# audeering/opensmile

Hardware: AMD Instinct MI355X
Metric: MFCC frames/sec (16kHz, 25ms/10ms) (higher is better)
Workload: dtype f32

## Files before the change

### include/smilehip.h

```cpp
#ifndef SMILEHIP_H
#define SMILEHIP_H

#include <stdint.h>

#ifdef __cplusplus
extern "C" {
#endif

#define SMILEHIP_VERSION 0x000100

typedef enum smilehip_status {
  SMILEHIP_OK = 0,
  SMILEHIP_ERR_INVALID = -1,
  SMILEHIP_ERR_NO_DEVICE = -2,
  SMILEHIP_ERR_HIP = -3,
  SMILEHIP_ERR_NOMEM = -4
} smilehip_status;

typedef enum smilehip_winfunc {
  SMILEHIP_WIN_RECT = 0, SMILEHIP_WIN_HANN = 1, SMILEHIP_WIN_HAMM = 2,
  SMILEHIP_WIN_GAUSS = 3, SMILEHIP_WIN_SINE = 4, SMILEHIP_WIN_TRI = 5,
  SMILEHIP_WIN_BARTLETT = 6, SMILEHIP_WIN_LANCZOS = 7
} smilehip_winfunc;

typedef struct smilehip_lld_config {
  uint32_t struct_size;
  double sample_rate;
  double frame_size_sec;
  double frame_step_sec;
  int32_t preemph;
  float   preemph_k;
  int32_t preemph_de;
  int32_t win_func;
  double  win_sigma;
  double  win_gain;
  double  win_offset;
  int32_t zero_pad_symmetric;
  int32_t n_bands;
  float   lofreq;
  float   hifreq;
  int32_t use_power;
  int32_t mel_htk_compatible;
  int32_t first_mfcc;
  int32_t last_mfcc;
  float   cep_lifter;
  int32_t mfcc_htk_compatible;
  float   melfloor;
  int32_t n_delta;
  int32_t delta_win;
  int32_t  chain_kind;
  int32_t  plp_lp_order;
  float    plp_compression;
  double   pitch_max;
  double   voicing_cutoff;
  int32_t  sma_win;
  int64_t  force_frame_size;
  double   force_fft_frame_size_sec;
  uint32_t stage_mask;
  double   pitch_min;
  int32_t  shs_n_harmonics;
  float    shs_compression;
  float    f0_min_energy;
  int32_t  append_log_energy;
  int32_t  cms;
  int32_t  jitter_broken_thresh;
  int32_t  vit_buffer_len;
  double   jitter_search_range;
  double   formant_max_freq;
  double   specscale_min_f;
  int32_t  shs_n_candidates;
  int32_t  shs_old_peak_algo;
  int32_t  spectral_band_lo[2], spectral_band_hi[2];
  int32_t  specscale_off;
} smilehip_lld_config;

#define SMILEHIP_CHAIN_MFCC 0
#define SMILEHIP_CHAIN_IS09 1
#define SMILEHIP_CHAIN_COMPARE_AB 2
#define SMILEHIP_CHAIN_PLP 3
#define SMILEHIP_CHAIN_COMPARE_F0 4
#define SMILEHIP_CHAIN_COMPARE 5
#define SMILEHIP_CHAIN_EGEMAPS 6

#define SMILEHIP_STAGE_WINDOW 1u
#define SMILEHIP_STAGE_FFT    2u
#define SMILEHIP_STAGE_MEL    4u
#define SMILEHIP_STAGE_MFCC   8u
#define SMILEHIP_STAGE_ALL    15u
#define SMILEHIP_STAGE_SPECTRAL 16u

typedef struct smilehip_geometry {
  int64_t frame_size;
  int64_t frame_step;
  int64_t fft_size;
  int64_t n_bins;
  int32_t n_static;
  int32_t n_out;
  double  frame_period;
  double  fft_frame_size_sec;
} smilehip_geometry;

typedef struct smilehip_context smilehip_context;
typedef struct smilehip_plan smilehip_plan;
typedef struct smilehip_batch smilehip_batch;

int  smilehip_version(void);
const char *smilehip_last_error(void);
int  smilehip_init(int device, smilehip_context **ctx);
void smilehip_shutdown(smilehip_context *ctx);
int  smilehip_device_name(smilehip_context *ctx, char *buf, int buflen);

void smilehip_config_is09_lld(smilehip_lld_config *c);

void smilehip_config_plp_0_d_a(smilehip_lld_config *c);
void smilehip_config_compare16_ab(smilehip_lld_config *c);
int smilehip_config_htk_variant(smilehip_lld_config *c, const char *name);
void smilehip_config_compare16_f0(smilehip_lld_config *c);
void smilehip_config_compare16(smilehip_lld_config *c);
void smilehip_config_is13_compare(smilehip_lld_config *c);

void smilehip_config_egemapsv02(smilehip_lld_config *c);
void smilehip_config_egemapsv01a(smilehip_lld_config *c);

int smilehip_specscale_frames(smilehip_plan *plan, const float *d_mag, int64_t ld_src, float *d_dst, int64_t ld_dst,
                              int64_t n_frames, void *stream);
int smilehip_pitchshs_frames(smilehip_plan *plan, const float *d_hps, int64_t ld_src, float *d_dst, int64_t ld_dst,
                             int64_t n_frames, void *stream);

int smilehip_batch_f0_taps(smilehip_batch *b, float *d_hps_dst, const float **d_shs, const float **d_e60);
int smilehip_batch_f0_pending(smilehip_batch *b, const int32_t **d_pending);

#define SMILEHIP_FUNC_MAX          (1u << 0)
#define SMILEHIP_FUNC_MIN          (1u << 1)
#define SMILEHIP_FUNC_RANGE        (1u << 2)
#define SMILEHIP_FUNC_MAXPOS       (1u << 3)
#define SMILEHIP_FUNC_MINPOS       (1u << 4)
#define SMILEHIP_FUNC_AMEAN        (1u << 5)
#define SMILEHIP_FUNC_MAXAMEANDIST (1u << 6)
#define SMILEHIP_FUNC_MINAMEANDIST (1u << 7)
#define SMILEHIP_FUNC_LINREGC1     (1u << 8)
#define SMILEHIP_FUNC_LINREGC2     (1u << 9)
#define SMILEHIP_FUNC_LINREGERRA   (1u << 10)
#define SMILEHIP_FUNC_LINREGERRQ   (1u << 11)
#define SMILEHIP_FUNC_VARIANCE     (1u << 12)
#define SMILEHIP_FUNC_STDDEV       (1u << 13)
#define SMILEHIP_FUNC_SKEWNESS     (1u << 14)
#define SMILEHIP_FUNC_KURTOSIS     (1u << 15)
#define SMILEHIP_FUNC_AMEAN_M      (1u << 16)
#define SMILEHIP_FUNC_ALL          0x1ffffu
uint32_t smilehip_functionals_is09_mask(void);
int smilehip_functionals_count(uint32_t mask);
int smilehip_batch_func_rows(const smilehip_batch *batch, int64_t *rows);
int smilehip_batch_functionals(smilehip_plan *plan, smilehip_batch *batch, const float *d_lld, int64_t ld_lld,
                               uint32_t mask, float *d_func, int64_t ld_func, void *stream);

int smilehip_functionals_matrix(smilehip_context *ctx, const float *d_x, int64_t ld_x, int64_t rows, int32_t cols,
                                uint32_t mask, float *d_out, void *stream);

enum {
  SMILEHIP_FAM_EXTREMES = 0, SMILEHIP_FAM_MEANS, SMILEHIP_FAM_MOMENTS, SMILEHIP_FAM_REGRESSION, SMILEHIP_FAM_PERCENTILES,
  SMILEHIP_FAM_TIMES, SMILEHIP_FAM_SEGMENTS, SMILEHIP_FAM_LPC, SMILEHIP_FAM_PEAKS2, SMILEHIP_FAM_ONSET, SMILEHIP_FAM_PEAKS, SMILEHIP_FAM_CROSSINGS, SMILEHIP_FAM_DCT,
  SMILEHIP_FAM_SAMPLES, SMILEHIP_FAM_MODULATION, SMILEHIP_FAM_COUNT
};
enum { SMILEHIP_NORM_SEGMENT = 0, SMILEHIP_NORM_SECOND = 1, SMILEHIP_NORM_FRAME = 2 };
enum { SMILEHIP_SEG_RELTH = 0, SMILEHIP_SEG_NONX = 1, SMILEHIP_SEG_EQX = 2, SMILEHIP_SEG_MRELTH = 3, SMILEHIP_SEG_ABSTH = 4,
       SMILEHIP_SEG_NARELTH = 5, SMILEHIP_SEG_NAMRELTH = 6, SMILEHIP_SEG_NAABSTH = 7, SMILEHIP_SEG_DELTA = 8,
       SMILEHIP_SEG_DELTA2 = 9, SMILEHIP_SEG_CHX = 10 };

typedef struct smilehip_func_spec {
  int32_t n_fam;
  int32_t fam[12];
  int32_t non_zero_functs;
  int32_t reserved0;
  double period;
  uint32_t ext_mask; int32_t ext_norm;
  uint32_t means_mask; int32_t means_norm;
  uint32_t mom_mask; int32_t mom_stddev_norm; int32_t mom_ratio_limit; int32_t reserved1;
  uint32_t reg_mask; int32_t reg_centroid_norm, reg_norm_coeff, reg_norm_inputs, reg_centroid_abs,
      reg_centroid_limit, reg_ratio_limit, reg_old_buggy_qerr;
  uint32_t pct_mask; int32_t pct_interp, n_pctl, n_range;
  double pctl[8]; int32_t range_a[8], range_b[8];
  uint32_t times_mask; int32_t times_norm, times_buggy_sec_norm, reserved2;
  uint32_t seg_mask; int32_t seg_norm, seg_algo, seg_max_num, seg_min_lng, seg_auto_min_lng, seg_pause_min_lng,
      seg_x_is_rel, seg_n_thresholds, seg_ravg_lng;
  float seg_x; float seg_thresholds[8]; float seg_range_rel_threshold;
  int32_t lpc_gain, lpc_coeffs, lpc_first, lpc_order;
  uint32_t pk_mask; int32_t pk_norm, pk_ratio_limit, pk_dyn_rel, pk_use_abs, reserved5;
  float pk_rel_thresh, pk_abs_thresh;
  uint32_t ons_mask; int32_t ons_norm, ons_use_abs, reserved6;
  float ons_thr_on, ons_thr_off;
  uint32_t pko_mask; int32_t pko_norm;
  uint32_t crs_mask; int32_t dct_first, dct_last, n_samples;
  double sample_pos[8];
  int32_t n_quot, quot_a[8], quot_b[8];
  int32_t n_ul, n_dl, reserved7;
  double ul[8], dl[8];
  int32_t mod_win_frames, mod_step_frames, mod_n_bins, mod_win_func, mod_remove_nz_mean, reserved8;
  double mod_min_freq, mod_max_freq;
} smilehip_func_spec;

int smilehip_funcspec_count(const smilehip_func_spec *spec);
int smilehip_funcspec_compare16(const char *instance, smilehip_func_spec *spec);
int smilehip_funcspec_is13_compare(const char *instance, smilehip_func_spec *spec);
int smilehip_funcspec_matrix(smilehip_context *ctx, const smilehip_func_spec *spec, const float *d_x, int64_t ld_x,
                             int64_t rows, int32_t cols, float *d_out, void *stream);
int smilehip_batch_funcspec(smilehip_plan *plan, smilehip_batch *batch, const smilehip_func_spec *spec,
                            const float *d_lld, int64_t ld_lld, int32_t col_first, int32_t n_cols, int32_t rows_cut,
                            const float *d_extra, int64_t ld_extra, float *d_func, int64_t ld_func, void *stream);

int smilehip_functionals_compare16_count(void);
int smilehip_batch_functionals_compare16(smilehip_plan *plan, smilehip_batch *batch, const float *d_lld, int64_t ld_lld,
                                         float *d_func, int64_t ld_func, void *stream);
int smilehip_batch_functionals_is13_compare(smilehip_plan *plan, smilehip_batch *batch, const float *d_lld, int64_t ld_lld,
                                            float *d_func, int64_t ld_func, void *stream);
int smilehip_batch_compare_b_extra(smilehip_batch *batch, const float **d_extra);

int smilehip_funcspec_egemaps(const char *instance, smilehip_func_spec *spec);
int smilehip_functionals_egemaps_count(void);
int smilehip_batch_functionals_egemaps(smilehip_plan *plan, smilehip_batch *batch, float *d_func, int64_t ld_func, void *stream);
int smilehip_batch_egemaps_taps(smilehip_batch *batch, const float **d_raw20, const float **d_lpc, const float **d_formants,
                                const float **d_pitch3, const float **d_jit4, const float **d_shim_db, const float **d_harm6,
                                const float **d_func_in, const int32_t **d_pending, int64_t *h_frame_off60);

int  smilehip_alloc(smilehip_context *ctx, uint64_t bytes, void **d_ptr);
int  smilehip_free(smilehip_context *ctx, void *d_ptr);
int  smilehip_copy_to_device(smilehip_context *ctx, void *d_dst, const void *h_src, uint64_t bytes, void *stream);
int  smilehip_copy_to_host(smilehip_context *ctx, void *h_dst, const void *d_src, uint64_t bytes, void *stream);
int  smilehip_stream_synchronize(smilehip_context *ctx, void *stream);
int  smilehip_alloc_cache(smilehip_context *ctx, uint64_t bytes);
int  smilehip_stream_create(smilehip_context *ctx, void **stream);
int  smilehip_stream_destroy(smilehip_context *ctx, void *stream);
int  smilehip_event_create(smilehip_context *ctx, void **event);
int  smilehip_event_destroy(smilehip_context *ctx, void *event);
int  smilehip_event_record(smilehip_context *ctx, void *event, void *stream);
int  smilehip_stream_wait_event(smilehip_context *ctx, void *stream, void *event);
int  smilehip_copy_to_device_2d(smilehip_context *ctx, void *d_dst, uint64_t d_pitch, const void *h_src, uint64_t h_pitch,
                                uint64_t width_bytes, uint64_t rows, void *stream);
int  smilehip_copy_to_host_2d(smilehip_context *ctx, void *h_dst, uint64_t h_pitch, const void *d_src, uint64_t d_pitch,
                              uint64_t width_bytes, uint64_t rows, void *stream);
int  smilehip_alloc_host(smilehip_context *ctx, uint64_t bytes, void **h_ptr);
int  smilehip_free_host(smilehip_context *ctx, void *h_ptr);
int  smilehip_host_register(smilehip_context *ctx, void *h_ptr, uint64_t bytes);
int  smilehip_host_unregister(smilehip_context *ctx, void *h_ptr);
int  smilehip_htk_rows_be(smilehip_context *ctx, const float *d_src, int64_t n, void *d_dst, void *stream);

void smilehip_config_mfcc12_0_d_a(smilehip_lld_config *c);

int  smilehip_plan_create(smilehip_context *ctx, const smilehip_lld_config *cfg, smilehip_plan **plan);
int  smilehip_plan_create_host_only(const smilehip_lld_config *cfg, smilehip_plan **plan);
void smilehip_plan_destroy(smilehip_plan *plan);
int  smilehip_plan_geometry(const smilehip_plan *plan, smilehip_geometry *g);
int64_t smilehip_num_frames(const smilehip_plan *plan, int64_t n_samples);
double  smilehip_frame_time(const smilehip_plan *plan, int64_t t);
double  smilehip_row_time(const smilehip_plan *plan, int64_t n_frames, int64_t row);
int64_t smilehip_plan_get_window(const smilehip_plan *plan, float *out, int64_t cap);
int64_t smilehip_plan_get_mel_weights(const smilehip_plan *plan, float *out, int64_t cap);
int64_t smilehip_plan_get_mel_chanmap(const smilehip_plan *plan, int32_t *out, int64_t cap);
int64_t smilehip_plan_get_dct(const smilehip_plan *plan, float *out, int64_t cap);
int64_t smilehip_plan_get_lifter(const smilehip_plan *plan, float *out, int64_t cap);

int  smilehip_batch_create(smilehip_plan *plan, const int64_t *h_sample_offsets, int32_t n_utt,
                           smilehip_batch **batch);
void smilehip_batch_destroy(smilehip_batch *batch);
int64_t smilehip_batch_total_frames(const smilehip_batch *batch);
int64_t smilehip_batch_total_rows(const smilehip_batch *batch);
int  smilehip_batch_delta_fused(const smilehip_batch *batch);
int  smilehip_batch_frame_offsets(const smilehip_batch *batch, int64_t *h_row_offsets);

int  smilehip_mfcc_run(smilehip_plan *plan, smilehip_batch *batch, const int16_t *d_pcm,
                       float *d_out, int64_t ld_out, void *stream);

int  smilehip_lld_run(smilehip_plan *plan, smilehip_batch *batch, const int16_t *d_pcm,
                      float *d_out, int64_t ld_out, void *stream);
int  smilehip_lld_run_f32(smilehip_plan *plan, smilehip_batch *batch, const float *d_pcm_f32,
                          float *d_out, int64_t ld_out, void *stream);
int  smilehip_lld_run_host(smilehip_plan *plan, smilehip_batch *batch, const int16_t *h_pcm,
                           int64_t n_samples, float *h_out);

int  smilehip_mfcc_run_host(smilehip_plan *plan, smilehip_batch *batch, const int16_t *h_pcm,
                            int64_t n_samples, float *h_out);

int  smilehip_plan_set_timing(smilehip_plan *plan, int enable);
int  smilehip_plan_last_timing(smilehip_plan *plan, float *ms_main, float *ms_delta);
int  smilehip_kernel_timing(int enable);
int64_t smilehip_kernel_timing_report(char *buf, int64_t buflen);


int smilehip_pcm16_to_float(smilehip_context *ctx, const int16_t *d_pcm, int64_t n, float *d_out, void *stream);
int smilehip_pcm_convert(smilehip_context *ctx, const void *d_raw, int n_bps, int n_bits, int n_chan, int mono_mixdown,
                         int64_t n, float *d_out, void *stream);
int smilehip_pcm_convert_float(smilehip_context *ctx, const float *d_raw, int n_chan, int mono_mixdown, int64_t n, float *d_out,
                               void *stream);
int smilehip_irfft_frames(smilehip_plan *plan, const float *d_src, int64_t ld_src, float *d_dst, int64_t ld_dst, int64_t n_frames,
                          void *stream);
#define SMILEHIP_MAGPHASE_MAGNITUDE 1
#define SMILEHIP_MAGPHASE_PHASE 2
#define SMILEHIP_MAGPHASE_NORMALISE 4
#define SMILEHIP_MAGPHASE_POWER 8
#define SMILEHIP_MAGPHASE_DBPSD 16
int smilehip_fftmagphase_frames(smilehip_context *ctx, const float *d_src, int64_t ld_src, int64_t nfft, int32_t flags, float dbp_norm,
                                float min_dbp, float *d_dst, int64_t ld_dst, int64_t n_frames, void *stream);
int smilehip_melspec_table_frames(smilehip_context *ctx, const float *d_src, int64_t ld_src, int64_t K, int32_t n_bands, int32_t dense,
                                  const float *d_coef, const int32_t *d_chanmap, int32_t n_lo, int32_t n_hi, int32_t use_power,
                                  float htk_scale, float *d_dst, int64_t ld_dst, int64_t n_frames, void *stream);
int smilehip_melspec_inverse_table_frames(smilehip_context *ctx, const float *d_src, int64_t ld_src, int32_t n_src, int64_t K,
                                          const float *d_coef, const int32_t *d_chanmap, int32_t n_lo, int32_t n_hi, int32_t use_power,
                                          float htk_div, float *d_dst, int64_t ld_dst, int64_t n_frames, void *stream);
int smilehip_pitchacf_zcr_frames(smilehip_context *ctx, const float *d_src, int64_t ld_src, int64_t n, int64_t n_frames, double fs_sec,
                                 double max_pitch, double *d_zcr, void *stream);
#define SMILEHIP_MZCR_ZCR 1
#define SMILEHIP_MZCR_MCR 2
#define SMILEHIP_MZCR_AMAX 4
#define SMILEHIP_MZCR_MAXMIN 8
#define SMILEHIP_MZCR_DC 16
int smilehip_mzcr_frames(smilehip_context *ctx, const float *d_src, int64_t ld_src, int64_t N, int64_t n_frames, int32_t flags,
                         float *d_dst, int64_t ld_dst, void *stream);
int smilehip_frame_rows(smilehip_context *ctx, const float *d_samples, int64_t frame_size, int64_t frame_step, int64_t n_frames,
                        float *d_dst, int64_t ld_dst, void *stream);
int smilehip_preemphasis_frames(smilehip_context *ctx, const float *d_src, int64_t ld_src, float *d_dst,
                                int64_t ld_dst, int64_t n_frames, int64_t N, float k, int de, void *stream);
int smilehip_window_frames(smilehip_plan *plan, const float *d_src, int64_t ld_src, float *d_dst,
                           int64_t ld_dst, int64_t n_frames, void *stream);
int smilehip_rfft_frames(smilehip_plan *plan, const float *d_src, int64_t ld_src, float *d_dst,
                         int64_t ld_dst, int64_t n_frames, void *stream);
int smilehip_fftmag_frames(smilehip_plan *plan, const float *d_src, int64_t ld_src, float *d_dst,
                           int64_t ld_dst, int64_t n_frames, void *stream);
int smilehip_melspec_frames(smilehip_plan *plan, const float *d_src, int64_t ld_src, float *d_dst,
                            int64_t ld_dst, int64_t n_frames, void *stream);
int smilehip_mfcc_frames(smilehip_plan *plan, const float *d_src, int64_t ld_src, float *d_dst,
                         int64_t ld_dst, int64_t n_frames, void *stream);
int  smilehip_mfcc_inverse_frames(smilehip_plan *plan, const float *d_src, int64_t ld_src, float *d_dst, int64_t ld_dst,
                                  int64_t n_frames, int do_log, void *stream);
int smilehip_sumsq_frames(smilehip_context *ctx, const float *d_src, int64_t ld_src, int64_t N, int64_t n_frames,
                          double *d_out, void *stream);
int smilehip_zcr_count_frames(smilehip_context *ctx, const float *d_src, int64_t ld_src, int64_t N, int64_t n_frames,
                              int32_t *d_out, void *stream);
int smilehip_acf_frames(smilehip_plan *plan, const float *d_src, int64_t ld_src, float *d_dst, int64_t ld_dst, int64_t n_out,
                        int64_t n_frames, int use_power, int cepstrum, int norm_output, int abs_cepstrum, void *stream);
int smilehip_pitchacf_frames(smilehip_context *ctx, const float *d_src, int64_t ld_src, int64_t n, int64_t n_frames,
                             double fs_sec, double max_pitch, double *d_voicing, int32_t *d_max_idx, void *stream);
int smilehip_pitchacf_contour_step(smilehip_context *ctx, const double *d_voicing, const int32_t *d_max_idx, double t_samp,
                                   double voicing_cutoff, float *d_state, float *d_out4, void *stream);
int smilehip_pitchacf_contour_frames(smilehip_context *ctx, const double *d_voicing, const int32_t *d_max_idx, double t_samp,
                                     double voicing_cutoff, float *d_state, float *d_out4, int64_t n_frames, void *stream);
int smilehip_spectral_frames(smilehip_plan *plan, const float *d_mag, int64_t ld_src, float *d_state, int first,
                             float *d_dst, int64_t ld_dst, int64_t n_frames, void *stream);
typedef struct smilehip_spectral_opts {
  int32_t n_bands;
  int32_t band_lo[16], band_hi[16];
  int32_t n_rolloff;
  double  rolloff[16];
  int32_t flux, centroid, max_pos, min_pos, entropy, variance, skewness, kurtosis, slope, sharpness, harmonicity;
  int32_t flatness, log_flatness;
  int32_t spec_diff, spec_pos_diff, flux_centroid, flux_at_flux_centroid, standard_deviation;
  int32_t n_slopes;
  int32_t slope_lo[16], slope_hi[16];
} smilehip_spectral_opts;
typedef struct smilehip_spectral_op smilehip_spectral_op;
int smilehip_spectral_opts_count(const smilehip_spectral_opts *opts);
int smilehip_spectral_op_create(smilehip_context *ctx, const smilehip_spectral_opts *opts, int64_t K, double frame_size_sec,
                                smilehip_spectral_op **op);
int smilehip_spectral_op_n_out(const smilehip_spectral_op *op);
int smilehip_spectral_op_frames(smilehip_spectral_op *op, const float *d_mag, int64_t ld_src, float *d_state, int first,
                                float *d_dst, int64_t ld_dst, int64_t n_frames, void *stream);
int smilehip_spectral_op_destroy(smilehip_spectral_op *op);
int smilehip_plp_audspec_frames(smilehip_context *ctx, const float *d_mel, int64_t ld_src, int n_bands, const float *d_eql,
                                float melfloor, float compression, int new_rasta, const float *rasta_coef, float *d_state,
                                float *d_dst, int64_t ld_dst, int64_t n_frames, void *stream);
int smilehip_plp_cc_frames(smilehip_context *ctx, const float *d_mel, int64_t ld_src, int n_bands, const float *d_eql,
                           float melfloor, float compression, int lp_order, const float *d_cos, const float *d_sin,
                           float *d_dst, int64_t ld_dst, int64_t n_frames, void *stream);
int smilehip_plp_stage_frames(smilehip_context *ctx, const float *d_mel, int64_t ld_src, int n_bands, const float *d_eql,
                              float melfloor, float compression, int lp_order, const float *d_cos, int out_stage,
                              float *d_dst, int64_t ld_dst, int64_t n_frames, void *stream);
int smilehip_window_op_row(smilehip_context *ctx, const float *d_x, float *d_y, int64_t n_t, int kind, int W, void *stream);
int smilehip_window_op_row_ex(smilehip_context *ctx, const float *d_x, float *d_y, int64_t n_t, int kind, int W, float *d_norm_io,
                              void *stream);
#define SMILEHIP_DELTA_RELATIVE 1
#define SMILEHIP_DELTA_HALFWAVE 2
#define SMILEHIP_DELTA_ABS 4
#define SMILEHIP_DELTA_SEGMENTS 8
int smilehip_delta_op_row(smilehip_context *ctx, const float *d_x, float *d_y, int64_t n_t, int W, int flags, float *d_norm_io,
                          void *stream);
int smilehip_window_op_block(smilehip_context *ctx, const float *d_x, int64_t ld_x, float *d_y, int64_t ld_y, int64_t n_t,
                             int32_t n_cols, int op, int W, int delta_flags, void *stream);
int smilehip_delta_segments_block(smilehip_context *ctx, const float *d_x, int64_t ld_x, float *d_y, int64_t ld_y, int64_t n_ticks,
                                  int32_t tick_frames, int32_t n_cols, int W, int delta_flags, float *d_norm_io, void *stream);
int smilehip_spectral_gemaps_frames(smilehip_plan *plan, const float *d_mag, int64_t ld_src, float *d_state, int first,
                                    float *d_dst, int64_t ld_dst, int64_t n_frames, void *stream);
int smilehip_specresample_frames(smilehip_plan *plan, const float *d_spec, int64_t ld_src, float *d_dst, int64_t ld_dst,
                                 int64_t n_frames, void *stream);
int smilehip_lpc_frames(smilehip_plan *plan, const float *d_x, int64_t ld_src, float *d_lpc, int64_t ld_dst, int64_t n_frames,
                        void *stream);
int smilehip_specresample_geometry(int64_t n_in, double fs_sec, double last_fs_sec, double base_period, double target_fs,
                                   int64_t *n_out, int64_t *k_max, double *nd);
int smilehip_specresample_tables(int64_t n_in, int64_t n_out, int64_t k_max, double nd, float *cos_table, float *sin_table);
int smilehip_specresample_table_frames(smilehip_context *ctx, const float *d_src, int64_t ld_src, int64_t n_in, int64_t n_out,
                                       int64_t k_max, const float *d_cos, const float *d_sin, float *d_dst, int64_t ld_dst,
                                       int64_t n_frames, void *stream);
int smilehip_lpc_acf_frames(smilehip_context *ctx, const float *d_x, int64_t ld_src, int64_t n, int32_t p, float *d_lpc,
                            int64_t ld_dst, int64_t n_frames, void *stream);
int smilehip_lsp_frames(smilehip_context *ctx, const float *d_lpc, int64_t ld_src, int32_t p, float *d_dst, int64_t ld_dst,
                        int64_t n_frames, void *stream);
int smilehip_intensity_frames(smilehip_context *ctx, const float *d_src, int64_t ld_src, int64_t N, int32_t flags, float *d_dst,
                              int64_t ld_dst, int64_t n_frames, void *stream);
enum { SMILEHIP_VOP_ADD = 0, SMILEHIP_VOP_MUL, SMILEHIP_VOP_LOG, SMILEHIP_VOP_LOGA, SMILEHIP_VOP_SQRT, SMILEHIP_VOP_E, SMILEHIP_VOP_ABS,
       SMILEHIP_VOP_DB_POW, SMILEHIP_VOP_DB_MAG, SMILEHIP_VOP_X_SUM, SMILEHIP_VOP_X_SUMSQ, SMILEHIP_VOP_X_L1, SMILEHIP_VOP_X_L2 };
int smilehip_vecop_frames(smilehip_context *ctx, int32_t op, float param1, float logfloor, const float *d_src, int64_t ld_src,
                          int32_t n_cols, float *d_dst, int64_t ld_dst, int64_t n_frames, void *stream);
int smilehip_pitch_smoother_rows(smilehip_context *ctx, int32_t n_cand, float voicing_cutoff, int32_t octave_correction,
                                 int32_t post_simple, int32_t flags, const float *d_src, int64_t ld_src, const int64_t *d_row_off,
                                 int32_t n_streams, int64_t n_rows_single, void *d_state, int32_t resume, float *d_dst, int64_t ld_dst,
                                 int64_t *d_written, void *stream);
int smilehip_formantlpc_frames(smilehip_plan *plan, const float *d_lpc, int64_t ld_src, float *d_dst, int64_t ld_dst,
                               int64_t n_frames, void *stream);
#define SMILEHIP_FORMANT_STATE_BYTES 176
int smilehip_formantlpc_rows(smilehip_plan *plan, const float *d_lpc, int64_t ld_src, float *d_dst, int64_t ld_dst,
                             int64_t n_frames, void *d_state, int32_t resume, void *stream);
int smilehip_harmonics_frames(smilehip_plan *plan, const float *d_f0, const float *d_formants, int64_t ld_formants,
                              const float *d_mag, int64_t ld_mag, float *d_dst, int64_t ld_dst, int64_t n_frames, void *stream);

int smilehip_delta_chain(smilehip_plan *plan, smilehip_batch *batch, float *d_io, int64_t ld,
                         int32_t D, int32_t W, int32_t n_orders, void *stream);

int smilehip_valbased_select_frames(smilehip_context *ctx, const float *d_src, int64_t ld_src, int64_t N, int64_t n_frames,
                                    int32_t idx, float threshold, int32_t invert, int32_t allow_equal, int32_t zero_vec,
                                    int32_t remove_idx, float output_val, float *d_dst, int64_t ld_dst, int32_t *d_keep, void *stream);

typedef struct smilehip_viterbi_stream smilehip_viterbi_stream;
int smilehip_viterbi_stream_create(smilehip_context *ctx, int32_t buffer_len, float voicing_cutoff, const double *weights6,
                                   smilehip_viterbi_stream **out);
int smilehip_viterbi_stream_set_candidates(smilehip_viterbi_stream *s, int32_t n_candidates);
int smilehip_viterbi_stream_push(smilehip_viterbi_stream *s, const float *cand_f0, const float *cand_voicing,
                                 int32_t *n_decided, int32_t *frames, int32_t *states, int32_t cap);
int smilehip_viterbi_stream_push_frames(smilehip_viterbi_stream *s, const float *cand_f0, const float *cand_voicing, int64_t ld,
                                        int32_t n_frames, int32_t *n_decided, int32_t *frames, int32_t *states, int32_t cap);
int smilehip_viterbi_stream_flush(smilehip_viterbi_stream *s, int32_t *n_decided, int32_t *frames, int32_t *states, int32_t cap);
int smilehip_viterbi_stream_destroy(smilehip_viterbi_stream *s);

typedef struct smilehip_jitter_stream smilehip_jitter_stream;
int smilehip_jitter_stream_create(smilehip_context *ctx, double sample_period, int64_t frame_size, int64_t frame_step,
                                  double frame_step_sec, double search_range_rel, int32_t broken_jitter_thresh,
                                  smilehip_jitter_stream **out);
int smilehip_jitter_stream_set_time_offset(smilehip_jitter_stream *s, int64_t frames);
int smilehip_jitter_stream_push(smilehip_jitter_stream *s, float f0, const int16_t *h_pcm, int64_t pcm_start, int64_t n_pcm,
                                float *out5, int64_t *last_idx, int64_t *last_mis);
int smilehip_jitter_stream_push_frames(smilehip_jitter_stream *s, const float *f0, int32_t n_frames, const int16_t *h_pcm,
                                       int64_t pcm_start, int64_t n_pcm, float *out5, int64_t *last_idx, int64_t *last_mis);
int smilehip_jitter_stream_destroy(smilehip_jitter_stream *s);

#define SMILEHIP_SPECSCALE_LINEAR 0
#define SMILEHIP_SPECSCALE_LOG 1
#define SMILEHIP_SPECSCALE_BARK 2
#define SMILEHIP_SPECSCALE_MEL 3
#define SMILEHIP_SPECSCALE_SEMITONE 4
#define SMILEHIP_SPECSCALE_BARK_OLD 7
typedef struct smilehip_specscale_opts {
  int32_t scale;
  double  param;
  double  min_f, max_f;
  int32_t n_points_target;
  int32_t spec_enhance, spec_smooth, auditory_weighting;
} smilehip_specscale_opts;
typedef struct smilehip_specscale_op smilehip_specscale_op;
int smilehip_specscale_op_create(smilehip_context *ctx, const smilehip_specscale_opts *opts, int64_t n_src, double frame_size_sec,
                                 smilehip_specscale_op **out);
int smilehip_specscale_op_n_out(const smilehip_specscale_op *op);
int smilehip_specscale_op_frames(smilehip_specscale_op *op, const float *d_src, int64_t ld_src, float *d_dst, int64_t ld_dst,
                                 int64_t n_frames, void *stream);
int smilehip_specscale_op_destroy(smilehip_specscale_op *op);
int smilehip_specscale_tables(const smilehip_specscale_opts *opts, int64_t n_src, double frame_size_sec, double *f_t, double *spline,
                              int32_t *k, double *rec);

#ifdef __cplusplus
}
#endif
#endif
```

### opensmile_amd/capi.py

```python
import ctypes as C
import os

import numpy as np

HERE = os.path.dirname(os.path.abspath(__file__))
LIB_PATH = os.path.join(HERE, "libsmilehip.so")

WINFUNC = {"rec": 0, "rect": 0, "han": 1, "hann": 1, "ham": 2, "hamming": 2, "gau": 3,
           "gauss": 3, "sin": 4, "sine": 4, "tri": 5, "bar": 6, "bartlett": 6, "lac": 7}


class SmileHipError(RuntimeError):
    pass


class LldConfig(C.Structure):
    _fields_ = [
        ("struct_size", C.c_uint32),
        ("sample_rate", C.c_double), ("frame_size_sec", C.c_double), ("frame_step_sec", C.c_double),
        ("preemph", C.c_int32), ("preemph_k", C.c_float), ("preemph_de", C.c_int32),
        ("win_func", C.c_int32), ("win_sigma", C.c_double), ("win_gain", C.c_double),
        ("win_offset", C.c_double),
        ("zero_pad_symmetric", C.c_int32),
        ("n_bands", C.c_int32), ("lofreq", C.c_float), ("hifreq", C.c_float),
        ("use_power", C.c_int32), ("mel_htk_compatible", C.c_int32),
        ("first_mfcc", C.c_int32), ("last_mfcc", C.c_int32), ("cep_lifter", C.c_float),
        ("mfcc_htk_compatible", C.c_int32), ("melfloor", C.c_float),
        ("n_delta", C.c_int32), ("delta_win", C.c_int32),
        ("chain_kind", C.c_int32), ("plp_lp_order", C.c_int32), ("plp_compression", C.c_float), ("pitch_max", C.c_double), ("voicing_cutoff", C.c_double),
        ("sma_win", C.c_int32),
        ("force_frame_size", C.c_int64), ("force_fft_frame_size_sec", C.c_double),
        ("stage_mask", C.c_uint32),
        ("pitch_min", C.c_double), ("shs_n_harmonics", C.c_int32), ("shs_compression", C.c_float),
        ("f0_min_energy", C.c_float), ("append_log_energy", C.c_int32), ("cms", C.c_int32), ("jitter_broken_thresh", C.c_int32),
        ("vit_buffer_len", C.c_int32), ("jitter_search_range", C.c_double), ("formant_max_freq", C.c_double), ("specscale_min_f", C.c_double), ("shs_n_candidates", C.c_int32), ("shs_old_peak_algo", C.c_int32),
        ("spectral_band_lo", C.c_int32 * 2), ("spectral_band_hi", C.c_int32 * 2), ("specscale_off", C.c_int32),
    ]


STAGE_WINDOW, STAGE_FFT, STAGE_MEL, STAGE_MFCC, STAGE_ALL = 1, 2, 4, 8, 15


class FuncSpec(C.Structure):
    _fields_ = [
        ("n_fam", C.c_int32), ("fam", C.c_int32 * 12), ("non_zero_functs", C.c_int32), ("reserved0", C.c_int32),
        ("period", C.c_double),
        ("ext_mask", C.c_uint32), ("ext_norm", C.c_int32),
        ("means_mask", C.c_uint32), ("means_norm", C.c_int32),
        ("mom_mask", C.c_uint32), ("mom_stddev_norm", C.c_int32), ("mom_ratio_limit", C.c_int32), ("reserved1", C.c_int32),
        ("reg_mask", C.c_uint32), ("reg_centroid_norm", C.c_int32), ("reg_norm_coeff", C.c_int32),
        ("reg_norm_inputs", C.c_int32), ("reg_centroid_abs", C.c_int32), ("reg_centroid_limit", C.c_int32),
        ("reg_ratio_limit", C.c_int32), ("reg_old_buggy_qerr", C.c_int32),
        ("pct_mask", C.c_uint32), ("pct_interp", C.c_int32), ("n_pctl", C.c_int32), ("n_range", C.c_int32),
        ("pctl", C.c_double * 8), ("range_a", C.c_int32 * 8), ("range_b", C.c_int32 * 8),
        ("times_mask", C.c_uint32), ("times_norm", C.c_int32), ("times_buggy_sec_norm", C.c_int32), ("reserved2", C.c_int32),
        ("seg_mask", C.c_uint32), ("seg_norm", C.c_int32), ("seg_algo", C.c_int32), ("seg_max_num", C.c_int32),
        ("seg_min_lng", C.c_int32), ("seg_auto_min_lng", C.c_int32), ("seg_pause_min_lng", C.c_int32),
        ("seg_x_is_rel", C.c_int32), ("seg_n_thresholds", C.c_int32), ("seg_ravg_lng", C.c_int32),
        ("seg_x", C.c_float), ("seg_thresholds", C.c_float * 8), ("seg_range_rel_threshold", C.c_float),
        ("lpc_gain", C.c_int32), ("lpc_coeffs", C.c_int32), ("lpc_first", C.c_int32), ("lpc_order", C.c_int32),
        ("pk_mask", C.c_uint32), ("pk_norm", C.c_int32), ("pk_ratio_limit", C.c_int32), ("pk_dyn_rel", C.c_int32),
        ("pk_use_abs", C.c_int32), ("reserved5", C.c_int32),
        ("pk_rel_thresh", C.c_float), ("pk_abs_thresh", C.c_float),
        ("ons_mask", C.c_uint32), ("ons_norm", C.c_int32), ("ons_use_abs", C.c_int32), ("reserved6", C.c_int32),
        ("ons_thr_on", C.c_float), ("ons_thr_off", C.c_float),
        ("pko_mask", C.c_uint32), ("pko_norm", C.c_int32),
        ("crs_mask", C.c_uint32), ("dct_first", C.c_int32), ("dct_last", C.c_int32), ("n_samples", C.c_int32),
        ("sample_pos", C.c_double * 8),
        ("n_quot", C.c_int32), ("quot_a", C.c_int32 * 8), ("quot_b", C.c_int32 * 8),
        ("n_ul", C.c_int32), ("n_dl", C.c_int32), ("reserved7", C.c_int32),
        ("ul", C.c_double * 8), ("dl", C.c_double * 8),
        ("mod_win_frames", C.c_int32), ("mod_step_frames", C.c_int32), ("mod_n_bins", C.c_int32), ("mod_win_func", C.c_int32),
        ("mod_remove_nz_mean", C.c_int32), ("reserved8", C.c_int32),
        ("mod_min_freq", C.c_double), ("mod_max_freq", C.c_double),
    ]


class SpectralOpts(C.Structure):
    _fields_ = [("n_bands", C.c_int32), ("band_lo", C.c_int32 * 16), ("band_hi", C.c_int32 * 16), ("n_rolloff", C.c_int32),
                ("rolloff", C.c_double * 16)] + [(k, C.c_int32) for k in ("flux", "centroid", "max_pos", "min_pos", "entropy", "variance",
                                                                          "skewness", "kurtosis", "slope", "sharpness", "harmonicity", "flatness",
                                                                          "log_flatness", "spec_diff", "spec_pos_diff", "flux_centroid",
                                                                          "flux_at_flux_centroid", "standard_deviation", "n_slopes")] + [
                   ("slope_lo", C.c_int32 * 16), ("slope_hi", C.c_int32 * 16)]


def spectral_opts(bands, rolloff=(0.25, 0.5, 0.75, 0.9), slopes=(), **flags):
    o = SpectralOpts()
    o.n_slopes = len(slopes)
    for i, (a, b) in enumerate(slopes):
        o.slope_lo[i], o.slope_hi[i] = a, b
    o.n_bands = len(bands)
    for i, (a, b) in enumerate(bands):
        o.band_lo[i], o.band_hi[i] = a, b
    o.n_rolloff = len(rolloff)
    for i, r in enumerate(rolloff):
        o.rolloff[i] = r
    for k, v in flags.items():
        setattr(o, k, int(v))
    return o


class SpecScaleOpts(C.Structure):
    _fields_ = [("scale", C.c_int32), ("param", C.c_double), ("min_f", C.c_double), ("max_f", C.c_double), ("n_points_target", C.c_int32),
                ("spec_enhance", C.c_int32), ("spec_smooth", C.c_int32), ("auditory_weighting", C.c_int32)]


SPECSCALE = {"lin": 0, "log": 1, "bark": 2, "mel": 3, "sem": 4, "bao": 7}


def specscale_opts(scale, param=0.0, min_f=25.0, max_f=-1.0, n_points_target=0, spec_enhance=0, spec_smooth=0, auditory_weighting=0):
    o = SpecScaleOpts()
    o.scale = SPECSCALE[scale] if isinstance(scale, str) else int(scale)
    o.param, o.min_f, o.max_f, o.n_points_target = float(param), float(min_f), float(max_f), int(n_points_target)
    o.spec_enhance, o.spec_smooth, o.auditory_weighting = int(spec_enhance), int(spec_smooth), int(auditory_weighting)
    return o


class Geometry(C.Structure):
    _fields_ = [("frame_size", C.c_int64), ("frame_step", C.c_int64), ("fft_size", C.c_int64),
                ("n_bins", C.c_int64), ("n_static", C.c_int32), ("n_out", C.c_int32),
                ("frame_period", C.c_double), ("fft_frame_size_sec", C.c_double)]


_vp, _i32, _i64, _f32, _dbl = C.c_void_p, C.c_int32, C.c_int64, C.c_float, C.c_double
SYMBOLS = {
    "smilehip_version": (C.c_int, []),
    "smilehip_last_error": (C.c_char_p, []),
    "smilehip_init": (C.c_int, [C.c_int, C.POINTER(_vp)]),
    "smilehip_shutdown": (None, [_vp]),
    "smilehip_device_name": (C.c_int, [_vp, C.c_char_p, C.c_int]),
    "smilehip_config_is09_lld": (None, [C.POINTER(LldConfig)]),
    "smilehip_config_compare16_ab": (None, [C.POINTER(LldConfig)]),
    "smilehip_config_compare16_f0": (None, [C.POINTER(LldConfig)]),
    "smilehip_config_htk_variant": (C.c_int, [C.POINTER(LldConfig), C.c_char_p]),
    "smilehip_config_compare16": (None, [C.POINTER(LldConfig)]),
    "smilehip_specscale_frames": (C.c_int, [_vp, _vp, _i64, _vp, _i64, _i64, _vp]),
    "smilehip_pitchshs_frames": (C.c_int, [_vp, _vp, _i64, _vp, _i64, _i64, _vp]),
    "smilehip_batch_f0_taps": (C.c_int, [_vp, _vp, C.POINTER(_vp), C.POINTER(_vp)]),
    "smilehip_config_plp_0_d_a": (None, [C.POINTER(LldConfig)]),
    "smilehip_batch_total_rows": (_i64, [_vp]),
    "smilehip_batch_delta_fused": (C.c_int, [_vp]),
    "smilehip_functionals_is09_mask": (C.c_uint32, []),
    "smilehip_functionals_count": (C.c_int, [C.c_uint32]),
    "smilehip_functionals_matrix": (C.c_int, [_vp, _vp, _i64, _i64, C.c_int32, C.c_uint32, _vp, _vp]),
    "smilehip_batch_func_rows": (C.c_int, [_vp, _vp]),
    "smilehip_batch_functionals": (C.c_int, [_vp, _vp, _vp, _i64, C.c_uint32, _vp, _i64, _vp]),
    "smilehip_functionals_compare16_count": (C.c_int, []),
    "smilehip_batch_functionals_compare16": (C.c_int, [_vp, _vp, _vp, _i64, _vp, _i64, _vp]),
    "smilehip_batch_compare_b_extra": (C.c_int, [_vp, _vp]),
    "smilehip_funcspec_count": (C.c_int, [_vp]),
    "smilehip_funcspec_compare16": (C.c_int, [C.c_char_p, _vp]),
    "smilehip_funcspec_is13_compare": (C.c_int, [C.c_char_p, _vp]),
    "smilehip_batch_functionals_is13_compare": (C.c_int, [_vp, _vp, _vp, _i64, _vp, _i64, _vp]),
    "smilehip_config_is13_compare": (None, [_vp]),
    "smilehip_config_egemapsv02": (None, [C.POINTER(LldConfig)]),
    "smilehip_config_egemapsv01a": (None, [C.POINTER(LldConfig)]),
    "smilehip_funcspec_egemaps": (C.c_int, [C.c_char_p, _vp]),
    "smilehip_functionals_egemaps_count": (C.c_int, []),
    "smilehip_batch_functionals_egemaps": (C.c_int, [_vp, _vp, _vp, _i64, _vp]),
    "smilehip_batch_egemaps_taps": (C.c_int, [_vp] + [C.POINTER(_vp)] * 9 + [_vp]),
    "smilehip_spectral_gemaps_frames": (C.c_int, [_vp, _vp, _i64, _vp, C.c_int, _vp, _i64, _i64, _vp]),
    "smilehip_specresample_frames": (C.c_int, [_vp, _vp, _i64, _vp, _i64, _i64, _vp]),
    "smilehip_lpc_frames": (C.c_int, [_vp, _vp, _i64, _vp, _i64, _i64, _vp]),
    "smilehip_formantlpc_frames": (C.c_int, [_vp, _vp, _i64, _vp, _i64, _i64, _vp]),
    "smilehip_formantlpc_rows": (C.c_int, [_vp, _vp, _i64, _vp, _i64, _i64, _vp, _i32, _vp]),
    "smilehip_harmonics_frames": (C.c_int, [_vp, _vp, _vp, _i64, _vp, _i64, _vp, _i64, _i64, _vp]),
    "smilehip_valbased_select_frames": (C.c_int, [_vp, _vp, _i64, _i64, _i64, _i32, _f32, _i32, _i32, _i32, _i32, _f32, _vp, _i64, _vp, _vp]),
    "smilehip_jitter_stream_create": (C.c_int, [_vp, _dbl, _i64, _i64, _dbl, _dbl, _i32, C.POINTER(_vp)]),
    "smilehip_jitter_stream_push": (C.c_int, [_vp, _f32, _vp, _i64, _i64, _vp, _vp, _vp]),
    "smilehip_jitter_stream_set_time_offset": (C.c_int, [_vp, _i64]),
    "smilehip_jitter_stream_destroy": (C.c_int, [_vp]),
    "smilehip_viterbi_stream_create": (C.c_int, [_vp, _i32, _f32, _vp, C.POINTER(_vp)]),
    "smilehip_viterbi_stream_push": (C.c_int, [_vp, _vp, _vp, _vp, _vp, _vp, _i32]),
    "smilehip_viterbi_stream_set_candidates": (C.c_int, [_vp, _i32]),
    "smilehip_viterbi_stream_flush": (C.c_int, [_vp, _vp, _vp, _vp, _i32]),
    "smilehip_viterbi_stream_destroy": (C.c_int, [_vp]),
    "smilehip_funcspec_matrix": (C.c_int, [_vp, _vp, _vp, _i64, _i64, C.c_int32, _vp, _vp]),
    "smilehip_batch_funcspec": (C.c_int, [_vp, _vp, _vp, _vp, _i64, C.c_int32, C.c_int32, C.c_int32, _vp, _i64, _vp, _i64, _vp]),
    "smilehip_lld_run": (C.c_int, [_vp, _vp, _vp, _vp, _i64, _vp]),
    "smilehip_lld_run_f32": (C.c_int, [_vp, _vp, _vp, _vp, _i64, _vp]),
    "smilehip_lld_run_host": (C.c_int, [_vp, _vp, _vp, _i64, _vp]),
    "smilehip_alloc": (C.c_int, [_vp, C.c_uint64, C.POINTER(_vp)]),
    "smilehip_free": (C.c_int, [_vp, _vp]),
    "smilehip_alloc_host": (C.c_int, [_vp, C.c_uint64, C.POINTER(_vp)]),
    "smilehip_free_host": (C.c_int, [_vp, _vp]),
    "smilehip_htk_rows_be": (C.c_int, [_vp, _vp, _i64, _vp, _vp]),
    "smilehip_copy_to_device": (C.c_int, [_vp, _vp, _vp, C.c_uint64, _vp]),
    "smilehip_copy_to_host": (C.c_int, [_vp, _vp, _vp, C.c_uint64, _vp]),
    "smilehip_alloc_cache": (C.c_int, [_vp, C.c_uint64]),
    "smilehip_stream_create": (C.c_int, [_vp, C.POINTER(_vp)]),
    "smilehip_stream_destroy": (C.c_int, [_vp, _vp]),
    "smilehip_event_create": (C.c_int, [_vp, C.POINTER(_vp)]),
    "smilehip_event_destroy": (C.c_int, [_vp, _vp]),
    "smilehip_event_record": (C.c_int, [_vp, _vp, _vp]),
    "smilehip_stream_wait_event": (C.c_int, [_vp, _vp, _vp]),
    "smilehip_kernel_timing": (C.c_int, [C.c_int]),
    "smilehip_kernel_timing_report": (C.c_int64, [_vp, _i64]),
    "smilehip_copy_to_device_2d": (C.c_int, [_vp, _vp, C.c_uint64, _vp, C.c_uint64, C.c_uint64, C.c_uint64, _vp]),
    "smilehip_copy_to_host_2d": (C.c_int, [_vp, _vp, C.c_uint64, _vp, C.c_uint64, C.c_uint64, C.c_uint64, _vp]),
    "smilehip_host_register": (C.c_int, [_vp, _vp, C.c_uint64]),
    "smilehip_host_unregister": (C.c_int, [_vp, _vp]),
    "smilehip_frame_rows": (C.c_int, [_vp, _vp, _i64, _i64, _i64, _vp, _i64, _vp]),
    "smilehip_window_op_block": (C.c_int, [_vp, _vp, _i64, _vp, _i64, _i64, _i32, C.c_int, C.c_int, C.c_int, _vp]),
    "smilehip_delta_segments_block": (C.c_int, [_vp, _vp, _i64, _vp, _i64, _i64, _i32, _i32, C.c_int, C.c_int, _vp, _vp]),
    "smilehip_pitchacf_contour_frames": (C.c_int, [_vp, _vp, _vp, _dbl, _dbl, _vp, _vp, _i64, _vp]),
    "smilehip_viterbi_stream_push_frames": (C.c_int, [_vp, _vp, _vp, _i64, _i32, _vp, _vp, _vp, _i32]),
    "smilehip_jitter_stream_push_frames": (C.c_int, [_vp, _vp, _i32, _vp, _i64, _i64, _vp, _vp, _vp]),
    "smilehip_stream_synchronize": (C.c_int, [_vp, _vp]),
    "smilehip_config_mfcc12_0_d_a": (None, [C.POINTER(LldConfig)]),
    "smilehip_plan_create": (C.c_int, [_vp, C.POINTER(LldConfig), C.POINTER(_vp)]),
    "smilehip_plan_create_host_only": (C.c_int, [C.POINTER(LldConfig), C.POINTER(_vp)]),
    "smilehip_plan_destroy": (None, [_vp]),
    "smilehip_plan_geometry": (C.c_int, [_vp, C.POINTER(Geometry)]),
    "smilehip_num_frames": (_i64, [_vp, _i64]),
    "smilehip_frame_time": (_dbl, [_vp, _i64]),
    "smilehip_row_time": (_dbl, [_vp, _i64, _i64]),
    "smilehip_plan_get_window": (_i64, [_vp, _vp, _i64]),
    "smilehip_plan_get_mel_weights": (_i64, [_vp, _vp, _i64]),
    "smilehip_plan_get_mel_chanmap": (_i64, [_vp, _vp, _i64]),
    "smilehip_plan_get_dct": (_i64, [_vp, _vp, _i64]),
    "smilehip_plan_get_lifter": (_i64, [_vp, _vp, _i64]),
    "smilehip_batch_f0_pending": (C.c_int, [_vp, _vp]),
    "smilehip_batch_create": (C.c_int, [_vp, _vp, _i32, C.POINTER(_vp)]),
    "smilehip_batch_destroy": (None, [_vp]),
    "smilehip_batch_total_frames": (_i64, [_vp]),
    "smilehip_batch_frame_offsets": (C.c_int, [_vp, _vp]),
    "smilehip_mfcc_run": (C.c_int, [_vp, _vp, _vp, _vp, _i64, _vp]),
    "smilehip_mfcc_run_host": (C.c_int, [_vp, _vp, _vp, _i64, _vp]),
    "smilehip_plan_set_timing": (C.c_int, [_vp, C.c_int]),
    "smilehip_plan_last_timing": (C.c_int, [_vp, C.POINTER(_f32), C.POINTER(_f32)]),
    "smilehip_sumsq_frames": (C.c_int, [_vp, _vp, _i64, _i64, _i64, _vp, _vp]),
    "smilehip_zcr_count_frames": (C.c_int, [_vp, _vp, _i64, _i64, _i64, _vp, _vp]),
    "smilehip_acf_frames": (C.c_int, [_vp, _vp, _i64, _vp, _i64, _i64, _i64, C.c_int, C.c_int, C.c_int, C.c_int, _vp]),
    "smilehip_pitchacf_frames": (C.c_int, [_vp, _vp, _i64, _i64, _i64, _dbl, _dbl, _vp, _vp, _vp]),
    "smilehip_pitchacf_contour_step": (C.c_int, [_vp, _vp, _vp, _dbl, _dbl, _vp, _vp, _vp]),
    "smilehip_spectral_frames": (C.c_int, [_vp, _vp, _i64, _vp, C.c_int, _vp, _i64, _i64, _vp]),
    "smilehip_spectral_opts_count": (C.c_int, [_vp]),
    "smilehip_spectral_op_create": (C.c_int, [_vp, _vp, _i64, C.c_double, _vp]),
    "smilehip_spectral_op_n_out": (C.c_int, [_vp]),
    "smilehip_spectral_op_frames": (C.c_int, [_vp, _vp, _i64, _vp, C.c_int, _vp, _i64, _i64, _vp]),
    "smilehip_spectral_op_destroy": (C.c_int, [_vp]),
    "smilehip_plp_audspec_frames": (C.c_int, [_vp, _vp, _i64, C.c_int, _vp, C.c_float, C.c_float, C.c_int, _vp, _vp, _vp, _i64,
                                             _i64, _vp]),
    "smilehip_plp_cc_frames": (C.c_int, [_vp, _vp, _i64, C.c_int, _vp, C.c_float, C.c_float, C.c_int, _vp, _vp, _vp, _i64, _i64,
                                        _vp]),
    "smilehip_mfcc_inverse_frames": (C.c_int, [_vp, _vp, _i64, _vp, _i64, _i64, C.c_int, _vp]),
    "smilehip_plp_stage_frames": (C.c_int, [_vp, _vp, _i64, C.c_int, _vp, C.c_float, C.c_float, C.c_int, _vp, C.c_int, _vp, _i64, _i64,
                                           _vp]),
    "smilehip_window_op_row": (C.c_int, [_vp, _vp, _vp, _i64, C.c_int, C.c_int, _vp]),
    "smilehip_window_op_row_ex": (C.c_int, [_vp, _vp, _vp, _i64, C.c_int, C.c_int, _vp, _vp]),
    "smilehip_delta_op_row": (C.c_int, [_vp, _vp, _vp, _i64, C.c_int, C.c_int, _vp, _vp]),
    "smilehip_pcm_convert": (C.c_int, [_vp, _vp, C.c_int, C.c_int, C.c_int, C.c_int, _i64, _vp, _vp]),
    "smilehip_pcm_convert_float": (C.c_int, [_vp, _vp, C.c_int, C.c_int, _i64, _vp, _vp]),
    "smilehip_pcm16_to_float": (C.c_int, [_vp, _vp, _i64, _vp, _vp]),
    "smilehip_preemphasis_frames": (C.c_int, [_vp, _vp, _i64, _vp, _i64, _i64, _i64, _f32, C.c_int, _vp]),
    "smilehip_window_frames": (C.c_int, [_vp, _vp, _i64, _vp, _i64, _i64, _vp]),
    "smilehip_rfft_frames": (C.c_int, [_vp, _vp, _i64, _vp, _i64, _i64, _vp]),
    "smilehip_fftmag_frames": (C.c_int, [_vp, _vp, _i64, _vp, _i64, _i64, _vp]),
    "smilehip_irfft_frames": (C.c_int, [_vp, _vp, _i64, _vp, _i64, _i64, _vp]),
    "smilehip_fftmagphase_frames": (C.c_int, [_vp, _vp, _i64, _i64, _i32, _f32, _f32, _vp, _i64, _i64, _vp]),
    "smilehip_melspec_table_frames": (C.c_int, [_vp, _vp, _i64, _i64, _i32, _i32, _vp, _vp, _i32, _i32, _i32, _f32, _vp, _i64, _i64, _vp]),
    "smilehip_melspec_inverse_table_frames": (C.c_int, [_vp, _vp, _i64, _i32, _i64, _vp, _vp, _i32, _i32, _i32, _f32, _vp, _i64, _i64, _vp]),
    "smilehip_pitchacf_zcr_frames": (C.c_int, [_vp, _vp, _i64, _i64, _i64, _dbl, _dbl, _vp, _vp]),
    "smilehip_mzcr_frames": (C.c_int, [_vp, _vp, _i64, _i64, _i64, _i32, _vp, _i64, _vp]),
    "smilehip_melspec_frames": (C.c_int, [_vp, _vp, _i64, _vp, _i64, _i64, _vp]),
    "smilehip_mfcc_frames": (C.c_int, [_vp, _vp, _i64, _vp, _i64, _i64, _vp]),
    "smilehip_delta_chain": (C.c_int, [_vp, _vp, _vp, _i64, _i32, _i32, _i32, _vp]),
    "smilehip_specresample_geometry": (C.c_int, [_i64, _dbl, _dbl, _dbl, _dbl, _vp, _vp, _vp]),
    "smilehip_specresample_tables": (C.c_int, [_i64, _i64, _i64, _dbl, _vp, _vp]),
    "smilehip_specresample_table_frames": (C.c_int, [_vp, _vp, _i64, _i64, _i64, _i64, _vp, _vp, _vp, _i64, _i64, _vp]),
    "smilehip_lpc_acf_frames": (C.c_int, [_vp, _vp, _i64, _i64, _i32, _vp, _i64, _i64, _vp]),
    "smilehip_lsp_frames": (C.c_int, [_vp, _vp, _i64, _i32, _vp, _i64, _i64, _vp]),
    "smilehip_intensity_frames": (C.c_int, [_vp, _vp, _i64, _i64, _i32, _vp, _i64, _i64, _vp]),
    "smilehip_vecop_frames": (C.c_int, [_vp, _i32, _f32, _f32, _vp, _i64, _i32, _vp, _i64, _i64, _vp]),
    "smilehip_pitch_smoother_rows": (C.c_int, [_vp, _i32, _f32, _i32, _i32, _i32, _vp, _i64, _vp, _i32, _i64, _vp, _i32, _vp, _i64, _vp, _vp]),
    "smilehip_specscale_op_create": (C.c_int, [_vp, _vp, _i64, _dbl, _vp]),
    "smilehip_specscale_op_n_out": (C.c_int, [_vp]),
    "smilehip_specscale_op_frames": (C.c_int, [_vp, _vp, _i64, _vp, _i64, _i64, _vp]),
    "smilehip_specscale_op_destroy": (C.c_int, [_vp]),
    "smilehip_specscale_tables": (C.c_int, [_vp, _i64, _dbl, _vp, _vp, _vp, _vp]),
}

_lib = None


def load():
    global _lib
    if _lib is None:
        path = os.environ.get("SMILEHIP_LIB", LIB_PATH)
        if not os.path.exists(path):
            raise SmileHipError(
                f"{LIB_PATH} not found: build it with `python -c 'import __graft_entry__ as g; g.build()'` "
                "(make -C opensmile_amd/csrc). libsmilehip has no CPU fallback.")
        L = C.CDLL(path)
        for name, (res, args) in SYMBOLS.items():
            fn = getattr(L, name)
            fn.restype = res
            fn.argtypes = args
        _lib = L
    return _lib


def _check(rc):
    if rc != 0:
        raise SmileHipError(f"smilehip error {rc}: {load().smilehip_last_error().decode()}")


def plp_0_d_a_config():
    c = LldConfig()
    load().smilehip_config_plp_0_d_a(C.byref(c))
    return c


def compare16_ab_config():
    c = LldConfig()
    load().smilehip_config_compare16_ab(C.byref(c))
    return c


def htk_variant_config(name):
    c = LldConfig()
    _check(load().smilehip_config_htk_variant(C.byref(c), name.encode()))
    return c


def compare16_config():
    c = LldConfig()
    load().smilehip_config_compare16(C.byref(c))
    return c


def is13_compare_config():
    c = LldConfig()
    load().smilehip_config_is13_compare(C.byref(c))
    return c


def egemapsv02_config():
    c = LldConfig()
    load().smilehip_config_egemapsv02(C.byref(c))
    return c


def egemapsv01a_config():
    c = LldConfig()
    load().smilehip_config_egemapsv01a(C.byref(c))
    return c


def funcspec_egemaps(instance):
    s = FuncSpec()
    _check(load().smilehip_funcspec_egemaps(instance.encode(), C.byref(s)))
    return s


def rows_op_host(ctx, fn, handle, inputs, out_cols, pre=(), post=()):
    L = load()
    inputs = [np.ascontiguousarray(a, dtype=np.float32) for a in inputs]
    n = inputs[0].shape[0]
    out = np.zeros((n, out_cols), np.float32)
    ptrs = []
    d_out = _vp()
    try:
        for a in inputs:
            d = _vp()
            _check(L.smilehip_alloc(ctx._h, max(a.nbytes, 4), C.byref(d)))
            ptrs.append(d)
            if a.nbytes:
                _check(L.smilehip_copy_to_device(ctx._h, d, a.ctypes.data, a.nbytes, None))
        _check(L.smilehip_alloc(ctx._h, max(out.nbytes, 4), C.byref(d_out)))
        args = [handle] + list(pre)
        for a, d in zip(inputs, ptrs):
            args += [d] + ([a.shape[1]] if a.ndim == 2 else [])
        args += [d_out, out_cols, n] + list(post) + [None]
        _check(fn(*args))
        _check(L.smilehip_stream_synchronize(ctx._h, None))
        if out.nbytes:
            _check(L.smilehip_copy_to_host(ctx._h, out.ctypes.data, d_out, out.nbytes, None))
    finally:
        for d in ptrs:
            L.smilehip_free(ctx._h, d)
        L.smilehip_free(ctx._h, d_out)
    return out


def specresample_host(plan, spec):
    return rows_op_host(plan.ctx, load().smilehip_specresample_frames, plan._h, [spec], 220)


def lpc_host(plan, x):
    return rows_op_host(plan.ctx, load().smilehip_lpc_frames, plan._h, [x], 11)


FORMANT_STATE_BYTES = 176


def formantlpc_host(plan, lpc, cuts=None):
    if cuts is None:
        return rows_op_host(plan.ctx, load().smilehip_formantlpc_frames, plan._h, [lpc], 10)
    L = load()
    ctx = plan.ctx
    lpc = np.ascontiguousarray(lpc, dtype=np.float32)
    n = lpc.shape[0]
    out = np.zeros((n, 10), np.float32)
    bounds = [0] + sorted(int(c) for c in cuts) + [n]
    d_in, d_out, d_st = _vp(), _vp(), _vp()
    _check(L.smilehip_alloc(ctx._h, max(lpc.nbytes, 4), C.byref(d_in)))
    _check(L.smilehip_alloc(ctx._h, max(out.nbytes, 4), C.byref(d_out)))
    _check(L.smilehip_alloc(ctx._h, FORMANT_STATE_BYTES, C.byref(d_st)))
    try:
        if lpc.nbytes:
            _check(L.smilehip_copy_to_device(ctx._h, d_in, lpc.ctypes.data, lpc.nbytes, None))
        for k in range(len(bounds) - 1):
            a, b = bounds[k], bounds[k + 1]
            _check(L.smilehip_formantlpc_rows(plan._h, d_in.value + a * lpc.shape[1] * 4, lpc.shape[1], d_out.value + a * 40, 10,
                                              b - a, d_st, 1 if a > 0 else 0, None))
        _check(L.smilehip_stream_synchronize(ctx._h, None))
        if out.nbytes:
            _check(L.smilehip_copy_to_host(ctx._h, out.ctypes.data, d_out, out.nbytes, None))
    finally:
        for d in (d_in, d_out, d_st):
            L.smilehip_free(ctx._h, d)
    return out


def harmonics_host(plan, f0, formants, mag):
    f0 = np.ascontiguousarray(f0, dtype=np.float32).reshape(-1)
    return rows_op_host(plan.ctx, load().smilehip_harmonics_frames, plan._h, [f0, formants, mag], 6)


def spectral_gemaps_host(plan, mag):
    L = load()
    mag = np.ascontiguousarray(mag, dtype=np.float32)
    n, K = mag.shape
    out = np.zeros((n, 5), np.float32)
    d_in, d_out, d_st = _vp(), _vp(), _vp()
    ctx = plan.ctx
    _check(L.smilehip_alloc(ctx._h, max(mag.nbytes, 4), C.byref(d_in)))
    _check(L.smilehip_alloc(ctx._h, max(out.nbytes, 4), C.byref(d_out)))
    _check(L.smilehip_alloc(ctx._h, K * 4, C.byref(d_st)))
    try:
        if mag.nbytes:
            _check(L.smilehip_copy_to_device(ctx._h, d_in, mag.ctypes.data, mag.nbytes, None))
        half = n // 2
        _check(L.smilehip_spectral_gemaps_frames(plan._h, d_in, K, d_st, 1, d_out, 5, half, None))
        _check(L.smilehip_spectral_gemaps_frames(plan._h, d_in.value + half * K * 4, K, d_st, 1 if half == 0 else 0,
                                                 d_out.value + half * 5 * 4, 5, n - half, None))
        _check(L.smilehip_stream_synchronize(ctx._h, None))
        if out.nbytes:
            _check(L.smilehip_copy_to_host(ctx._h, out.ctypes.data, d_out, out.nbytes, None))
    finally:
        L.smilehip_free(ctx._h, d_in)
        L.smilehip_free(ctx._h, d_out)
        L.smilehip_free(ctx._h, d_st)
    return out


def funcspec_is13_compare(instance):
    s = FuncSpec()
    _check(load().smilehip_funcspec_is13_compare(instance.encode(), C.byref(s)))
    return s


def compare16_f0_config():
    c = LldConfig()
    load().smilehip_config_compare16_f0(C.byref(c))
    return c


def funcspec_compare16(instance):
    s = FuncSpec()
    _check(load().smilehip_funcspec_compare16(instance.encode(), C.byref(s)))
    return s


def funcspec_count(spec):
    n = load().smilehip_funcspec_count(C.byref(spec))
    if n < 0:
        _check(n)
    return n


def funcspec_matrix_host(ctx, spec, x):
    L = load()
    x = np.ascontiguousarray(x, dtype=np.float32)
    rows, cols = x.shape
    per = funcspec_count(spec)
    out = np.zeros((cols, per), np.float32)
    d_x, d_out = _vp(), _vp()
    _check(L.smilehip_alloc(ctx._h, max(x.nbytes, 4), C.byref(d_x)))
    _check(L.smilehip_alloc(ctx._h, max(out.nbytes, 4), C.byref(d_out)))
    try:
        _check(L.smilehip_copy_to_device(ctx._h, d_x, x.ctypes.data, x.nbytes, None))
        _check(L.smilehip_funcspec_matrix(ctx._h, C.byref(spec), d_x, cols, rows, cols, d_out, None))
        _check(L.smilehip_stream_synchronize(ctx._h, None))
        _check(L.smilehip_copy_to_host(ctx._h, out.ctypes.data, d_out, out.nbytes, None))
    finally:
        L.smilehip_free(ctx._h, d_x)
        L.smilehip_free(ctx._h, d_out)
    return out


def is09_lld_config():
    c = LldConfig()
    load().smilehip_config_is09_lld(C.byref(c))
    return c


def mfcc12_0_d_a_config():
    c = LldConfig()
    load().smilehip_config_mfcc12_0_d_a(C.byref(c))
    return c


class Context:
    def __init__(self, device=0):
        self._h = _vp()
        _check(load().smilehip_init(device, C.byref(self._h)))

    def name(self):
        buf = C.create_string_buffer(256)
        _check(load().smilehip_device_name(self._h, buf, 256))
        return buf.value.decode()

    def close(self):
        if self._h:
            load().smilehip_shutdown(self._h)
            self._h = _vp()

    def __del__(self):
        try:
            self.close()
        except Exception:
            pass


class Plan:

    def __init__(self, ctx, cfg=None):
        self.ctx = ctx
        self.cfg = cfg if cfg is not None else mfcc12_0_d_a_config()
        self._h = _vp()
        if ctx is None:
            _check(load().smilehip_plan_create_host_only(C.byref(self.cfg), C.byref(self._h)))
        else:
            _check(load().smilehip_plan_create(ctx._h, C.byref(self.cfg), C.byref(self._h)))
        g = Geometry()
        _check(load().smilehip_plan_geometry(self._h, C.byref(g)))
        self.geometry = g

    def num_frames(self, n_samples):
        return int(load().smilehip_num_frames(self._h, n_samples))

    def frame_time(self, t):
        return float(load().smilehip_frame_time(self._h, t))

    def _table(self, fn, dtype):
        n = fn(self._h, None, 0)
        a = np.zeros(n, dtype)
        fn(self._h, a.ctypes.data, n)
        return a

    def window(self):
        return self._table(load().smilehip_plan_get_window, np.float32)

    def mel_weights(self):
        return self._table(load().smilehip_plan_get_mel_weights, np.float32)

    def mel_chanmap(self):
        return self._table(load().smilehip_plan_get_mel_chanmap, np.int32)

    def dct(self):
        g = self.geometry
        return self._table(load().smilehip_plan_get_dct, np.float32).reshape(g.n_static, self.cfg.n_bands)

    def lifter(self):
        return self._table(load().smilehip_plan_get_lifter, np.float32)

    def set_timing(self, on=True):
        _check(load().smilehip_plan_set_timing(self._h, 1 if on else 0))

    def last_timing(self):
        a, b = _f32(), _f32()
        _check(load().smilehip_plan_last_timing(self._h, C.byref(a), C.byref(b)))
        return a.value, b.value

    def close(self):
        if self._h:
            load().smilehip_plan_destroy(self._h)
            self._h = _vp()

    def __del__(self):
        try:
            self.close()
        except Exception:
            pass


class Batch:

    def __init__(self, plan, sample_offsets):
        self.plan = plan
        off = np.ascontiguousarray(sample_offsets, dtype=np.int64)
        assert off.ndim == 1 and len(off) >= 1
        self.n_utt = len(off) - 1
        self.sample_offsets = off
        self._h = _vp()
        _check(load().smilehip_batch_create(plan._h, off.ctypes.data, self.n_utt, C.byref(self._h)))
        self.total_frames = int(load().smilehip_batch_total_frames(self._h))
        self.total_rows = int(load().smilehip_batch_total_rows(self._h))
        self.delta_fused = bool(load().smilehip_batch_delta_fused(self._h))
        fo = np.zeros(self.n_utt + 1, np.int64)
        _check(load().smilehip_batch_frame_offsets(self._h, fo.ctypes.data))
        self.frame_offsets = fo

    def run_device(self, d_pcm_ptr, d_out_ptr, ld_out, stream=None):
        _check(load().smilehip_lld_run(self.plan._h, self._h, d_pcm_ptr, d_out_ptr, ld_out, stream))

    def run_device_f32(self, d_pcm_f32_ptr, d_out_ptr, ld_out, stream=None):
        _check(load().smilehip_lld_run_f32(self.plan._h, self._h, d_pcm_f32_ptr, d_out_ptr, ld_out, stream))

    def run_host(self, pcm):
        pcm = np.ascontiguousarray(pcm, dtype=np.int16)
        out = np.zeros((self.total_rows, self.plan.geometry.n_out), np.float32)
        _check(load().smilehip_lld_run_host(self.plan._h, self._h, pcm.ctypes.data, len(pcm),
                                            out.ctypes.data))
        return out

    def f0_run_host_taps(self, pcm):
        L = load()
        ctx = self.plan.ctx._h
        pcm = np.ascontiguousarray(pcm, dtype=np.int16)
        K = self.plan.geometry.n_bins
        nf = self.total_frames
        out = np.zeros((self.total_rows, self.plan.geometry.n_out), np.float32)
        taps = {"hps": np.zeros((nf, K), np.float32), "shs": np.zeros((nf, 21), np.float32), "e60": np.zeros((nf, 1), np.float32)}
        d_pcm, d_out, d_hps = _vp(), _vp(), _vp()
        _check(L.smilehip_alloc(ctx, max(pcm.nbytes, 4), C.byref(d_pcm)))
        _check(L.smilehip_alloc(ctx, max(out.nbytes, 4), C.byref(d_out)))
        _check(L.smilehip_alloc(ctx, max(taps["hps"].nbytes, 4), C.byref(d_hps)))
        try:
            if pcm.nbytes:
                _check(L.smilehip_copy_to_device(ctx, d_pcm, pcm.ctypes.data, pcm.nbytes, None))
            d_shs, d_e60 = _vp(), _vp()
            _check(L.smilehip_batch_f0_taps(self._h, d_hps, C.byref(d_shs), C.byref(d_e60)))
            _check(L.smilehip_lld_run(self.plan._h, self._h, d_pcm, d_out, self.plan.geometry.n_out, None))
            _check(L.smilehip_stream_synchronize(ctx, None))
            if out.nbytes:
                _check(L.smilehip_copy_to_host(ctx, out.ctypes.data, d_out, out.nbytes, None))
            if nf:
                _check(L.smilehip_copy_to_host(ctx, taps["hps"].ctypes.data, d_hps, taps["hps"].nbytes, None))
                _check(L.smilehip_copy_to_host(ctx, taps["shs"].ctypes.data, d_shs, taps["shs"].nbytes, None))
                _check(L.smilehip_copy_to_host(ctx, taps["e60"].ctypes.data, d_e60, taps["e60"].nbytes, None))
            _check(L.smilehip_batch_f0_taps(self._h, None, None, None))
        finally:
            L.smilehip_free(ctx, d_pcm)
            L.smilehip_free(ctx, d_out)
            L.smilehip_free(ctx, d_hps)
        return out, taps

    def func_rows(self):
        r = np.zeros(self.n_utt, np.int64)
        _check(load().smilehip_batch_func_rows(self._h, r.ctypes.data))
        return r

    def functionals_device(self, d_lld_ptr, ld_lld, d_func_ptr, ld_func, mask=None, stream=None):
        L = load()
        mask = L.smilehip_functionals_is09_mask() if mask is None else mask
        _check(L.smilehip_batch_functionals(self.plan._h, self._h, d_lld_ptr, ld_lld, mask, d_func_ptr, ld_func, stream))

    def functionals_host(self, lld, mask=None):
        L = load()
        mask = L.smilehip_functionals_is09_mask() if mask is None else mask
        per = L.smilehip_functionals_count(mask)
        n_out = self.plan.geometry.n_out
        lld = np.ascontiguousarray(lld, dtype=np.float32)
        assert lld.shape == (self.total_rows, n_out)
        out = np.zeros((self.n_utt, n_out * per), np.float32)
        ctx = self.plan.ctx._h
        d_lld, d_out = _vp(), _vp()
        _check(L.smilehip_alloc(ctx, max(lld.nbytes, 4), C.byref(d_lld)))
        _check(L.smilehip_alloc(ctx, max(out.nbytes, 4), C.byref(d_out)))
        try:
            if lld.nbytes:
                _check(L.smilehip_copy_to_device(ctx, d_lld, lld.ctypes.data, lld.nbytes, None))
            _check(L.smilehip_batch_functionals(self.plan._h, self._h, d_lld, n_out, mask, d_out, n_out * per, None))
            _check(L.smilehip_stream_synchronize(ctx, None))
            if out.nbytes:
                _check(L.smilehip_copy_to_host(ctx, out.ctypes.data, d_out, out.nbytes, None))
        finally:
            L.smilehip_free(ctx, d_lld)
            L.smilehip_free(ctx, d_out)
        return out

    def run_host_with_functionals16(self, pcm):
        L = load()
        pcm = np.ascontiguousarray(pcm, dtype=np.int16)
        n_out = self.plan.geometry.n_out
        nf = L.smilehip_functionals_compare16_count()
        lld = np.zeros((self.total_rows, n_out), np.float32)
        func = np.zeros((self.n_utt, nf), np.float32)
        ex = np.zeros((self.n_utt, 110), np.float32)
        ctx = self.plan.ctx._h
        d_pcm, d_lld, d_func = _vp(), _vp(), _vp()
        _check(L.smilehip_alloc(ctx, max(pcm.nbytes, 4), C.byref(d_pcm)))
        _check(L.smilehip_alloc(ctx, max(lld.nbytes, 4), C.byref(d_lld)))
        _check(L.smilehip_alloc(ctx, max(func.nbytes, 4), C.byref(d_func)))
        try:
            if pcm.nbytes:
                _check(L.smilehip_copy_to_device(ctx, d_pcm, pcm.ctypes.data, pcm.nbytes, None))
            _check(L.smilehip_lld_run(self.plan._h, self._h, d_pcm, d_lld, n_out, None))
            fn = L.smilehip_batch_functionals_is13_compare if self.plan.cfg.jitter_broken_thresh else L.smilehip_batch_functionals_compare16
            _check(fn(self.plan._h, self._h, d_lld, n_out, d_func, nf, None))
            _check(L.smilehip_stream_synchronize(ctx, None))
            if lld.nbytes:
                _check(L.smilehip_copy_to_host(ctx, lld.ctypes.data, d_lld, lld.nbytes, None))
            if func.nbytes:
                _check(L.smilehip_copy_to_host(ctx, func.ctypes.data, d_func, func.nbytes, None))
            d_ex = _vp()
            _check(L.smilehip_batch_compare_b_extra(self._h, C.byref(d_ex)))
            if ex.nbytes:
                _check(L.smilehip_copy_to_host(ctx, ex.ctypes.data, d_ex, ex.nbytes, None))
        finally:
            L.smilehip_free(ctx, d_pcm)
            L.smilehip_free(ctx, d_lld)
            L.smilehip_free(ctx, d_func)
        return lld, func, ex

    def run_host_egemaps(self, pcm, functionals=True, taps=False):
        L = load()
        pcm = np.ascontiguousarray(pcm, dtype=np.int16)
        n_out = self.plan.geometry.n_out
        lld = np.zeros((self.total_rows, n_out), np.float32)
        func = np.zeros((self.n_utt, 88), np.float32) if functionals else None
        ctx = self.plan.ctx._h
        d_pcm, d_lld, d_func = _vp(), _vp(), _vp()
        _check(L.smilehip_alloc(ctx, max(pcm.nbytes, 4), C.byref(d_pcm)))
        _check(L.smilehip_alloc(ctx, max(lld.nbytes, 4), C.byref(d_lld)))
        _check(L.smilehip_alloc(ctx, max(self.n_utt * 88 * 4, 4), C.byref(d_func)))
        out_taps = {}
        try:
            if pcm.nbytes:
                _check(L.smilehip_copy_to_device(ctx, d_pcm, pcm.ctypes.data, pcm.nbytes, None))
            _check(L.smilehip_lld_run(self.plan._h, self._h, d_pcm, d_lld, n_out, None))
            if functionals:
                _check(L.smilehip_batch_functionals_egemaps(self.plan._h, self._h, d_func, 88, None))
            _check(L.smilehip_stream_synchronize(ctx, None))
            if lld.nbytes:
                _check(L.smilehip_copy_to_host(ctx, lld.ctypes.data, d_lld, lld.nbytes, None))
            if functionals and func.nbytes:
                _check(L.smilehip_copy_to_host(ctx, func.ctypes.data, d_func, func.nbytes, None))
            if taps:
                ptrs = [_vp() for _ in range(9)]
                fo60 = np.zeros(self.n_utt + 1, np.int64)
                _check(L.smilehip_batch_egemaps_taps(self._h, *[C.byref(q) for q in ptrs], fo60.ctypes.data))
                nf, nf60 = self.total_frames, int(fo60[-1])
                T20 = np.diff(self.frame_offsets_frames())
                T60 = np.diff(fo60)
                nfin = int(np.where(T60 >= 1, T20 + 1, 0).sum())
                shapes = [("raw20", (nf, 12)), ("lpc", (nf, 12)), ("formants", (nf, 10)), ("pitch3", (nf60, 3)), ("jit4", (nf60, 4)),
                          ("shim_db", (nf60, 1)), ("harm6", (nf60, 6)), ("func_in", (nfin, 36))]
                for (name, shp), q in zip(shapes, ptrs):
                    a = np.zeros(shp, np.float32)
                    if a.nbytes:
                        _check(L.smilehip_copy_to_host(ctx, a.ctypes.data, q, a.nbytes, None))
                    out_taps[name] = a
                pend = np.zeros(self.n_utt, np.int32)
                if pend.nbytes:
                    _check(L.smilehip_copy_to_host(ctx, pend.ctypes.data, ptrs[8], pend.nbytes, None))
                out_taps["pending"] = pend
                out_taps["frame_off60"] = fo60
                out_taps["fin_off"] = np.concatenate([[0], np.cumsum(np.where(T60 >= 1, T20 + 1, 0))]).astype(np.int64)
        finally:
            L.smilehip_free(ctx, d_pcm)
            L.smilehip_free(ctx, d_lld)
            L.smilehip_free(ctx, d_func)
        return (lld, func, out_taps) if taps else (lld, func)

    def frame_offsets_frames(self):
        T = [self.plan.num_frames(int(self.sample_offsets[u + 1] - self.sample_offsets[u])) for u in range(self.n_utt)]
        return np.concatenate([[0], np.cumsum(T)]).astype(np.int64)

    def funcspec_host(self, lld, spec, col_first, n_cols, rows_cut, extra=None):
        L = load()
        per = funcspec_count(spec)
        lld = np.ascontiguousarray(lld, dtype=np.float32)
        ld = lld.shape[1]
        assert lld.shape[0] == self.total_rows
        out = np.zeros((self.n_utt, n_cols * per), np.float32)
        ctx = self.plan.ctx._h
        d_lld, d_out, d_ex = _vp(), _vp(), _vp()
        _check(L.smilehip_alloc(ctx, max(lld.nbytes, 4), C.byref(d_lld)))
        _check(L.smilehip_alloc(ctx, max(out.nbytes, 4), C.byref(d_out)))
        try:
            if extra is not None:
                extra = np.ascontiguousarray(extra, dtype=np.float32)
                assert extra.shape == (self.n_utt, n_cols)
                _check(L.smilehip_alloc(ctx, max(extra.nbytes, 4), C.byref(d_ex)))
                _check(L.smilehip_copy_to_device(ctx, d_ex, extra.ctypes.data, extra.nbytes, None))
            if lld.nbytes:
                _check(L.smilehip_copy_to_device(ctx, d_lld, lld.ctypes.data, lld.nbytes, None))
            _check(L.smilehip_batch_funcspec(self.plan._h, self._h, C.byref(spec), d_lld, ld, col_first, n_cols, rows_cut,
                                             d_ex if extra is not None else None, n_cols, d_out, n_cols * per, None))
            _check(L.smilehip_stream_synchronize(ctx, None))
            if out.nbytes:
                _check(L.smilehip_copy_to_host(ctx, out.ctypes.data, d_out, out.nbytes, None))
        finally:
            L.smilehip_free(ctx, d_lld)
            L.smilehip_free(ctx, d_out)
            if extra is not None:
                L.smilehip_free(ctx, d_ex)
        return out

    def close(self):
        if self._h:
            load().smilehip_batch_destroy(self._h)
            self._h = _vp()

    def __del__(self):
        try:
            self.close()
        except Exception:
            pass


def extract_mfcc(pcm_list, cfg=None, device=0):
    ctx = Context(device)
    plan = Plan(ctx, cfg)
    lens = [len(p) for p in pcm_list]
    off = np.concatenate([[0], np.cumsum(lens)]).astype(np.int64)
    pcm = np.concatenate([np.asarray(p, np.int16) for p in pcm_list]) if pcm_list else np.zeros(0, np.int16)
    b = Batch(plan, off)
    out = b.run_host(pcm)
    res = [out[b.frame_offsets[i]:b.frame_offsets[i + 1]] for i in range(len(pcm_list))]
    b.close()
    plan.close()
    ctx.close()
    return res


def pcm_convert_host(ctx, raw, n_bps, n_bits, n_chan, mixdown=True):
    L = load()
    raw = np.ascontiguousarray(np.frombuffer(bytes(raw), dtype=np.uint8))
    n = len(raw) // (n_bps * n_chan)
    out = np.zeros(n if mixdown else (n, n_chan), np.float32)
    d_in, d_out = _vp(), _vp()
    _check(L.smilehip_alloc(ctx._h, max(raw.nbytes, 4), C.byref(d_in)))
    _check(L.smilehip_alloc(ctx._h, max(out.nbytes, 4), C.byref(d_out)))
    try:
        if raw.nbytes:
            _check(L.smilehip_copy_to_device(ctx._h, d_in, raw.ctypes.data, raw.nbytes, None))
        _check(L.smilehip_pcm_convert(ctx._h, d_in, n_bps, n_bits, n_chan, int(mixdown), n, d_out, None))
        _check(L.smilehip_stream_synchronize(ctx._h, None))
        if out.nbytes:
            _check(L.smilehip_copy_to_host(ctx._h, out.ctypes.data, d_out, out.nbytes, None))
    finally:
        L.smilehip_free(ctx._h, d_in)
        L.smilehip_free(ctx._h, d_out)
    return out


def kernel_timing(enable=True):
    _check(load().smilehip_kernel_timing(1 if enable else 0))


def kernel_timing_report():
    L = load()
    n = 1 << 16
    while True:
        buf = C.create_string_buffer(n)
        got = L.smilehip_kernel_timing_report(buf, n)
        if got >= 0:
            break
        n = -got + 1
    out = {}
    for line in buf.value.decode().splitlines():
        name, launches, ms = line.split("\t")
        name = name.split("<")[0].strip()
        a = out.get(name, (0, 0.0))
        out[name] = (a[0] + int(launches), a[1] + float(ms))
    return out


def pcm16_to_float(ctx, d_pcm, n, d_out, stream=None):
    _check(load().smilehip_pcm16_to_float(ctx._h, d_pcm, n, d_out, stream))


def preemphasis_frames(ctx, d_src, ld_src, d_dst, ld_dst, n_frames, N, k, de=0, stream=None):
    _check(load().smilehip_preemphasis_frames(ctx._h, d_src, ld_src, d_dst, ld_dst, n_frames, N, k, de, stream))


def window_frames(plan, d_src, ld_src, d_dst, ld_dst, n_frames, stream=None):
    _check(load().smilehip_window_frames(plan._h, d_src, ld_src, d_dst, ld_dst, n_frames, stream))


def rfft_frames(plan, d_src, ld_src, d_dst, ld_dst, n_frames, stream=None):
    _check(load().smilehip_rfft_frames(plan._h, d_src, ld_src, d_dst, ld_dst, n_frames, stream))


def fftmag_frames(plan, d_src, ld_src, d_dst, ld_dst, n_frames, stream=None):
    _check(load().smilehip_fftmag_frames(plan._h, d_src, ld_src, d_dst, ld_dst, n_frames, stream))


def melspec_frames(plan, d_src, ld_src, d_dst, ld_dst, n_frames, stream=None):
    _check(load().smilehip_melspec_frames(plan._h, d_src, ld_src, d_dst, ld_dst, n_frames, stream))


def mfcc_frames(plan, d_src, ld_src, d_dst, ld_dst, n_frames, stream=None):
    _check(load().smilehip_mfcc_frames(plan._h, d_src, ld_src, d_dst, ld_dst, n_frames, stream))


# ... 32 lines not shown
```

### opensmile_amd/csrc/batch_layout.hpp

```cpp
#pragma once
#include <algorithm>
#include <cmath>
#include <cstdint>
#include <map>
#include <vector>

#include "../../include/smilehip.h"
#include "lld_tile_rec.hpp"

namespace smilehip {

struct BatchLayoutSpec {
  int chain_kind = SMILEHIP_CHAIN_MFCC;
  int64_t N = 0, H = 0;
  double period = 0.0;
  int row_extra = 0;
  bool fused_delta_eligible = false;
  int64_t fast_slots = 8;
  int64_t tile_frames = 0;
  int64_t dtile_rows = 0;
  int short_T = 0;
  int jitter_chunk = 0;
  int run_frames_override = 0;
};

struct BatchLayout {
  std::vector<int64_t> samp_off, frame_off, row_off;
  std::vector<int64_t> fin_off;
  std::vector<int32_t> short_utts;
  bool all_even = true;
  int64_t total_frames = 0, total_rows = 0;
  std::vector<int32_t> tile_utt, tile_t0, dtile_utt, dtile_t0;
  std::vector<TileRec> tile_rec;
  std::vector<int32_t> run_utt, run_t0;
  int32_t run_frames = 8;
  std::vector<FTileRec> ftiles;
  std::vector<int32_t> jit_utt, jit_t0;
  std::vector<int32_t> frame_utt;
};

constexpr int kRunFramesMin = 8;

inline int compare_run_frames(int64_t total_frames) {
  int L = kRunFramesMin;
  while (L < 64 && total_frames / (2 * L) >= 65536) L *= 2;
  return L;
}

inline int64_t layout_num_frames(int64_t len, int64_t N, int64_t H) { return len < N ? 0 : (len - N) / H + 1; }
inline int64_t samples_60ms(double period) { return std::lround(0.060 / period); }

inline int64_t layout_rows(const BatchLayoutSpec &s, int64_t len, int64_t T) {
  const bool compare = s.chain_kind == SMILEHIP_CHAIN_COMPARE_AB || s.chain_kind == SMILEHIP_CHAIN_COMPARE;
  if (!compare && s.chain_kind != SMILEHIP_CHAIN_EGEMAPS) return T > 0 ? T + s.row_extra : 0;
  const int64_t T60 = layout_num_frames(len, samples_60ms(s.period), s.H);
  return T60 >= (compare ? 4 : 1) ? T60 + 1 : 0;
}

inline void layout_fused_tiles(const BatchLayoutSpec &s, const int64_t *h_off, int32_t n_utt, BatchLayout &out) {
  const auto parts_of = [&](int64_t T, int64_t L) { return (T + L - 1) / L; };
  int64_t bestL = 32;
  double best = 1e300;
  std::map<int64_t, int64_t> hist;
  for (int32_t u = 0; u < n_utt; ++u) {
    const int64_t T = out.frame_off[u + 1] - out.frame_off[u];
    if (T > 0) hist[T]++;
  }
  for (int64_t L = 32; L <= 2048; L += 4) {
    int64_t n = 0;
    for (const auto &h : hist) n += h.second * ((h.first <= s.short_T) ? 1 : parts_of(h.first, L));
    const double cost = double((n + s.fast_slots - 1) / s.fast_slots) * double(L / 4 + 2);
    if (cost <= best) { best = cost; bestL = L; }
  }
  for (int32_t u = 0; u < n_utt; ++u) {
    const int64_t T = out.frame_off[u + 1] - out.frame_off[u];
    if (T <= 0) continue;
    const int64_t parts = (T <= s.short_T) ? 1 : parts_of(T, bestL);
    const int64_t len = (((T + parts - 1) / parts) + 3) & ~int64_t(3);
    for (int64_t t0 = 0; t0 < T; t0 += len) {
      const int64_t t1 = std::min<int64_t>(T, t0 + len), p0 = t0 > 0 ? t0 - 4 : 0;
      FTileRec r;
      r.samp0 = h_off[u] + p0 * s.H;
      r.row0 = out.frame_off[u] + p0;
      const int64_t last = (t1 + 3) & ~int64_t(3);
      r.n_frames = (int32_t)(last - p0 + 4);
      r.live_n = (int32_t)(T - p0);
      r.e0 = (int32_t)(t0 - p0);
      r.e1 = (int32_t)(t1 - p0);
      r.lo = (int32_t)(-p0);
      r.delta_on = T > s.short_T;
      out.ftiles.push_back(r);
    }
  }
  std::stable_sort(out.ftiles.begin(), out.ftiles.end(), [](const FTileRec &a, const FTileRec &c) { return a.n_frames > c.n_frames; });
}

inline int batch_layout(const BatchLayoutSpec &s, const int64_t *h_off, int32_t n_utt, BatchLayout &out) {
  out = BatchLayout();
  out.samp_off.assign(h_off, h_off + (n_utt ? n_utt + 1 : 0));
  if (n_utt == 0) out.samp_off.assign(1, 0);
  out.frame_off.assign(size_t(n_utt) + 1, 0);
  out.row_off.assign(size_t(n_utt) + 1, 0);
  const bool compare = s.chain_kind == SMILEHIP_CHAIN_COMPARE_AB || s.chain_kind == SMILEHIP_CHAIN_COMPARE;
  const bool egemaps = s.chain_kind == SMILEHIP_CHAIN_EGEMAPS;
  if (egemaps) out.fin_off.assign(size_t(n_utt) + 1, 0);
  {
    int64_t total_T = 0;
    for (int32_t u = 0; u < n_utt; ++u) total_T += layout_num_frames(h_off[u + 1] - h_off[u], s.N, s.H);
    out.run_frames = s.run_frames_override >= 1 ? s.run_frames_override : compare_run_frames(total_T);
  }
  for (int32_t u = 0; u < n_utt; ++u) {
    const int64_t len = h_off[u + 1] - h_off[u];
    if (len < 0) return u + 1;
    const int64_t T = layout_num_frames(len, s.N, s.H);
    const int64_t rows = layout_rows(s, len, T);
    if (compare || egemaps)
      for (int64_t t0 = 0; t0 < T; t0 += out.run_frames) {
        out.run_utt.push_back(u);
        out.run_t0.push_back((int32_t)t0);
      }
    if (egemaps) out.fin_off[u + 1] = out.fin_off[u] + (rows > 0 ? T + 1 : 0);
    out.frame_off[u + 1] = out.frame_off[u] + T;
    out.row_off[u + 1] = out.row_off[u] + rows;
    if (T > 0 && T <= s.short_T) out.short_utts.push_back(u);
    if (T > 0 && (h_off[u] & 1)) out.all_even = false;
    for (int64_t t0 = 0; t0 < T; t0 += s.tile_frames) {
      out.tile_utt.push_back(u);
      out.tile_t0.push_back((int32_t)t0);
      TileRec r;
      r.samp0 = h_off[u] + t0 * s.H;
      r.row0 = out.frame_off[u] + t0;
      r.n_frames = (int32_t)std::min<int64_t>(s.tile_frames, T - t0);
      r.pad = 0;
      out.tile_rec.push_back(r);
    }
    for (int64_t t0 = 0; t0 < rows; t0 += s.dtile_rows) {
      out.dtile_utt.push_back(u);
      out.dtile_t0.push_back((int32_t)t0);
    }
  }
  out.total_frames = out.frame_off[n_utt];
  out.total_rows = out.row_off[n_utt];
  if (s.chain_kind == SMILEHIP_CHAIN_IS09 && out.total_frames > 0) {
    out.frame_utt.resize((size_t)out.total_frames);
    for (int32_t u = 0; u < n_utt; ++u) std::fill(out.frame_utt.begin() + out.frame_off[u], out.frame_utt.begin() + out.frame_off[u + 1], u);
  }
  if (s.fused_delta_eligible && out.total_frames > 0 && out.all_even)
    layout_fused_tiles(s, h_off, n_utt, out);
  if (s.chain_kind == SMILEHIP_CHAIN_COMPARE_F0) {
    int64_t maxT = 0;
    for (int32_t u = 0; u < n_utt; ++u) maxT = std::max(maxT, out.frame_off[u + 1] - out.frame_off[u]);
    for (int64_t t0 = 0; t0 < maxT; t0 += s.jitter_chunk)
      for (int32_t u = 0; u < n_utt; ++u)
        if (t0 < out.frame_off[u + 1] - out.frame_off[u]) { out.jit_utt.push_back(u); out.jit_t0.push_back((int32_t)t0); }
  }
  return 0;
}

}
```

### opensmile_amd/csrc/lld_mfcc512.hip

```cpp
#include <hip/hip_runtime.h>
#include "kernel_timing.hpp"

#include <algorithm>
#include <cmath>
#include <cstdio>
#include <cstdlib>
#include <cstring>
#include <type_traits>
#include <vector>

#include "lld_device.hpp"
#include "lld_launch.hpp"
#include "lld_params.hpp"
#include "tables.hpp"

namespace smilehip {

namespace {

constexpr int kWavesPerBlock = 8;
constexpr int kTileFrames = 32;
constexpr int kTB2Row = 65;
constexpr int kTB2Floats = 2 * (15 * kTB2Row + 3 * 16 + 16);
constexpr int kLmelFloats = 64;
constexpr int kOctetFloats = 12;
constexpr int kPbFloats = 448;
constexpr int kWaveFloats = 2080;

static_assert(kWaveFloats >= kTB2Floats && kWaveFloats >= 4 * (kLmelFloats + kPbFloats) && kWaveFloats % 4 == 0, "per-wave LDS region");
static_assert(kPbFloats % 64 == 0 && kPbFloats >= 33 * kOctetFloats, "power buffer");

constexpr float C1 = 0.92387953251128673848f;
constexpr float S1 = 0.38268343236508978178f;
constexpr float R2 = 0.70710678118654752440f;

__device__ __forceinline__ void wave_lds_fence() {
  __builtin_amdgcn_fence(__ATOMIC_ACQ_REL, "wavefront");
  __builtin_amdgcn_wave_barrier();
}

__host__ __device__ constexpr int pb_pos(int k) { return k + (kOctetFloats - 8) * (k >> 3); }

__device__ __forceinline__ void dft4(float &r0, float &i0, float &r1, float &i1, float &r2, float &i2,
                                     float &r3, float &i3) {
  const float t0r = r0 + r2, t0i = i0 + i2;
  const float t1r = r0 - r2, t1i = i0 - i2;
  const float t2r = r1 + r3, t2i = i1 + i3;
  const float t3r = r1 - r3, t3i = i1 - i3;
  r0 = t0r + t2r; i0 = t0i + t2i;
  r2 = t0r - t2r; i2 = t0i - t2i;
  r1 = t1r + t3i; i1 = t1i - t3r;
  r3 = t1r - t3i; i3 = t1i + t3r;
}

__device__ __forceinline__ void cmul(float &r, float &i, float c, float s) {
  const float nr = fmaf(r, c, -i * s);
  const float ni = fmaf(r, s, i * c);
  r = nr; i = ni;
}
__device__ __forceinline__ void cmul_ns(float &r, float &i, float c, float s, float ns) {
  const float nr = fmaf(r, c, i * ns);
  const float ni = fmaf(r, s, i * c);
  r = nr; i = ni;
}

struct Dft16K {
  float c1, s1, r2, nc1, ns1, nr2;
  __device__ __forceinline__ Dft16K() : c1(C1), s1(S1), r2(R2), nc1(-C1), ns1(-S1), nr2(-R2) {
    asm volatile("" : "+s"(c1), "+s"(s1), "+s"(r2), "+s"(nc1), "+s"(ns1), "+s"(nr2));
  }
};

__device__ __forceinline__ void dft16_first(float (&re)[16], float (&im)[16], int m0) {
  dft4(re[m0], im[m0], re[m0 + 4], im[m0 + 4], re[m0 + 8], im[m0 + 8], re[m0 + 12], im[m0 + 12]);
}
__device__ __forceinline__ void dft16_twiddles(float (&re)[16], float (&im)[16], const Dft16K &K) {
  cmul_ns(re[1 + 4], im[1 + 4], K.c1, K.ns1, K.s1);
  { const float a = re[1 + 8], b = im[1 + 8]; re[1 + 8] = K.r2 * (a + b); im[1 + 8] = K.r2 * (b - a); }
  cmul_ns(re[1 + 12], im[1 + 12], K.s1, K.nc1, K.c1);
  { const float a = re[2 + 4], b = im[2 + 4]; re[2 + 4] = K.r2 * (a + b); im[2 + 4] = K.r2 * (b - a); }
  { const float a = re[2 + 8], b = im[2 + 8]; re[2 + 8] = b; im[2 + 8] = -a; }
  { const float a = re[2 + 12], b = im[2 + 12]; re[2 + 12] = K.r2 * (b - a); im[2 + 12] = K.nr2 * (a + b); }
  cmul_ns(re[3 + 4], im[3 + 4], K.s1, K.nc1, K.c1);
  { const float a = re[3 + 8], b = im[3 + 8]; re[3 + 8] = K.r2 * (b - a); im[3 + 8] = K.nr2 * (a + b); }
  cmul_ns(re[3 + 12], im[3 + 12], K.nc1, K.s1, K.ns1);
}
__device__ __forceinline__ void dft16_last(float (&re)[16], float (&im)[16], int q) {
  dft4(re[4 * q], im[4 * q], re[4 * q + 1], im[4 * q + 1], re[4 * q + 2], im[4 * q + 2], re[4 * q + 3], im[4 * q + 3]);
}
__device__ __forceinline__ void dft16_rename(float (&re)[16], float (&im)[16]) {
  float tr[16], ti[16];
#pragma unroll
  for (int q = 0; q < 4; ++q)
#pragma unroll
    for (int p = 0; p < 4; ++p) { tr[q + 4 * p] = re[4 * q + p]; ti[q + 4 * p] = im[4 * q + p]; }
#pragma unroll
  for (int k = 0; k < 16; ++k) { re[k] = tr[k]; im[k] = ti[k]; }
}
__device__ __forceinline__ void dft16(float (&re)[16], float (&im)[16], const Dft16K &K) {
#pragma unroll
  for (int m0 = 0; m0 < 4; ++m0) dft16_first(re, im, m0);
  dft16_twiddles(re, im, K);
#pragma unroll
  for (int q = 0; q < 4; ++q) dft16_last(re, im, q);
  dft16_rename(re, im);
}

template <int CTRL>
__device__ __forceinline__ float dpp_f(float v) {
  return __int_as_float(__builtin_amdgcn_update_dpp(0, __float_as_int(v), CTRL, 0xf, 0xf, true));
}

}

#ifdef SMILEHIP_MFCC512_PRED_LOADS
#ifdef SMILEHIP_MFCC512_GLOBAL_LOADS
#error "SMILEHIP_MFCC512_GLOBAL_LOADS loads no predecessor samples"
#endif
constexpr bool kPredLoads = true;
#else
constexpr bool kPredLoads = false;
#endif
#ifdef SMILEHIP_MFCC512_B16_SAMPLES
#ifdef SMILEHIP_MFCC512_GLOBAL_LOADS
#error "SMILEHIP_MFCC512_GLOBAL_LOADS loads dwords for aligned input: it cannot be combined with SMILEHIP_MFCC512_B16_SAMPLES"
#endif
constexpr bool kB16Samples = true;
#else
constexpr bool kB16Samples = false;
#endif
#ifdef SMILEHIP_MFCC512_WRITES_IN_ONE_BLOCK
constexpr bool kWritesEarly = false;
#else
constexpr bool kWritesEarly = true;
#endif
#ifdef SMILEHIP_MFCC512_READS_IN_DFT_ORDER
constexpr bool kReadsInDftOrder = true;
#else
constexpr bool kReadsInDftOrder = false;
#endif
#ifdef SMILEHIP_MFCC512_MIRROR_OPERAND
constexpr bool kMirrorOperand = true;
#else
constexpr bool kMirrorOperand = false;
#endif
#ifdef SMILEHIP_MFCC512_BPERMUTE_PARTNER
constexpr bool kMirrorAtUse = false;
#else
constexpr bool kMirrorAtUse = kMirrorOperand;
#endif
template <int MP, bool ALIGNED, bool PREEMPH>
struct FrameRegs {
  uint32_t v[ALIGNED && !kB16Samples ? MP : 2 * MP];
  uint32_t p[PREEMPH && kPredLoads ? MP : 1];
};

template <int MP, bool ALIGNED, bool PREEMPH>
__device__ __forceinline__ void pcm_prefetch(const int16_t *pcm, int64_t pcm_total, int64_t base, int H, int lane,
                                             FrameRegs<MP, ALIGNED, PREEMPH> &R) {
#ifndef SMILEHIP_MFCC512_GLOBAL_LOADS
  const int64_t b0 = base < 0 ? 0 : base;
  int64_t left = (pcm_total - b0) * 2;
  left = left < 0 ? 0 : (left > 0xfffffffcLL ? 0xfffffffcLL : left);
  const __amdgpu_buffer_rsrc_t rsrc = __builtin_amdgcn_make_buffer_rsrc(const_cast<int16_t *>(pcm + b0), 0, (int)(uint32_t)left, 0x00020000);
  uint32_t lo = ((uint32_t)(lane >> 4) * (uint32_t)H + 2u * (uint32_t)(lane & 15)) * 2u + (uint32_t)((base - b0) * 2);
  asm volatile("" : "+v"(lo));
  uint32_t lo_p = lo - 2u;
  if (PREEMPH && kPredLoads) asm volatile("" : "+v"(lo_p));
#pragma unroll
  for (int m = 0; m < MP; ++m) {
    if (PREEMPH && kPredLoads)
      R.p[m] = (uint32_t)(int32_t)(int16_t)__builtin_amdgcn_raw_buffer_load_b16(rsrc, m == 0 ? (int)lo_p : (int)lo + 64 * m - 2, 0, 0);
    if (ALIGNED && !kB16Samples) {
      R.v[m] = (uint32_t)__builtin_amdgcn_raw_buffer_load_b32(rsrc, (int)lo + 64 * m, 0, 0);
    } else {
      R.v[2 * m] = (uint32_t)(int32_t)(int16_t)__builtin_amdgcn_raw_buffer_load_b16(rsrc, (int)lo + 64 * m, 0, 0);
      R.v[2 * m + 1] = (uint32_t)(int32_t)(int16_t)__builtin_amdgcn_raw_buffer_load_b16(rsrc, (int)lo + 64 * m + 2, 0, 0);
    }
  }
#else
#ifdef SMILEHIP_DEBUG_SAME_SPAN
  base &= 0xfffff;
#endif
  uint32_t lo = ((uint32_t)(lane >> 4) * (uint32_t)H + 2u * (uint32_t)(lane & 15)) * 2u;
  asm volatile("" : "+v"(lo));
#ifdef SMILEHIP_DEBUG_NO_LOADS
  for (int m = 0; m < (ALIGNED ? MP : 2 * MP); ++m) R.v[m] = lo * (m + 3);
  return;
#endif
  const unsigned char *span = reinterpret_cast<const unsigned char *>(pcm + base);
  const int64_t room = pcm_total - base;
  if (base >= 0 && room >= (int64_t)(3 * H + 32 * MP)) {
#pragma unroll
    for (int m = 0; m < MP; ++m) {
      const unsigned char *q = span + 64 * m + lo;
      if (ALIGNED) {
        R.v[m] = *reinterpret_cast<const uint32_t *>(q);
      } else {
        R.v[2 * m] = (uint32_t)(int32_t) reinterpret_cast<const int16_t *>(q)[0];
        R.v[2 * m + 1] = (uint32_t)(int32_t) reinterpret_cast<const int16_t *>(q)[1];
      }
    }
  } else {
    const int64_t last = ALIGNED ? ((pcm_total >> 1) - 1) * 2 : pcm_total - 2;
    const int32_t lim_lo = base < 0 ? (int32_t)(-base) * 2 : 0;
    int64_t hi64 = (last - base) * 2;
    hi64 = hi64 > (1 << 24) ? (1 << 24) : hi64;
    const int32_t lim_hi = hi64 < lim_lo ? lim_lo : (int32_t)hi64;
#pragma unroll
    for (int m = 0; m < MP; ++m) {
      int32_t off = (int32_t)lo + 64 * m;
      off = off < lim_lo ? lim_lo : (off > lim_hi ? lim_hi : off);
      const unsigned char *q = span + off;
      if (ALIGNED) {
        R.v[m] = *reinterpret_cast<const uint32_t *>(q);
      } else {
        R.v[2 * m] = (uint32_t)(int32_t) reinterpret_cast<const int16_t *>(q)[0];
        R.v[2 * m + 1] = (uint32_t)(int32_t) reinterpret_cast<const int16_t *>(q)[1];
      }
    }
  }
#endif
}

#ifdef SMILEHIP_PHASE_TIMING
__device__ unsigned long long g_phase[16];
#define PHASE_DECL unsigned long long ph_acc[12] = {0}; unsigned long long ph_last = __builtin_amdgcn_s_memtime();
#define PHASE(i) do { const unsigned long long t_ = __builtin_amdgcn_s_memtime(); ph_acc[i] += t_ - ph_last; ph_last = t_; } while (0)
#define PHASE_FLUSH do { if (lane == 0) for (int i_ = 0; i_ < 12; ++i_) atomicAdd(&g_phase[i_], ph_acc[i_]); } while (0)
#else
#define PHASE_DECL
#define PHASE(i)
#define PHASE_FLUSH
#endif

template <int MP, bool PREEMPH, bool USE_POWER, bool ALIGNED, bool PLP, int UC, bool DELTA, bool PAD0>
__device__ __forceinline__ void lld_mfcc512_body(const LldParams &P, const Fast512Tables &F) {
  extern __shared__ __attribute__((aligned(16))) float smem[];
  const int lane = threadIdx.x & 63;
  const int wave = __builtin_amdgcn_readfirstlane(threadIdx.x >> 6);
  const int g = lane >> 4;
  const int j = lane & 15;

  float2 *s_tw512 = reinterpret_cast<float2 *>(smem);
  float2 *s_win = s_tw512 + 256;
  float2 *s_tw256 = s_win + MP * 16;
  float4 *s_melw0 = reinterpret_cast<float4 *>(s_tw256 + 256);
  float4 *s_melw1 = s_melw0 + UC * 16;
  float *s_dct = reinterpret_cast<float *>(s_melw1 + UC * 16);
  float *s_plp = s_dct + 16 * 28;
  constexpr int shared_floats = 256 * 2 + MP * 16 * 2 + 256 * 2 + UC * 16 * 8 + 16 * 28 + 48;
  float *wbase = smem + shared_floats + wave * kWaveFloats;
  float *s_lmel = wbase + g * kLmelFloats;
  float *s_cep = s_lmel + 48;
  float *s_pb = wbase + 4 * kLmelFloats + g * kPbFloats;

  for (int i = threadIdx.x; i < 256; i += blockDim.x) { s_tw512[i] = F.tw512[i]; s_tw256[i] = F.tw256[i]; }
  for (int i = threadIdx.x; i < MP * 16; i += blockDim.x) s_win[i] = F.win[i];
  for (int i = threadIdx.x; i < UC * 16; i += blockDim.x) { s_melw0[i] = F.melw[2 * i]; s_melw1[i] = F.melw[2 * i + 1]; }
  for (int i = threadIdx.x; i < 16 * 28; i += blockDim.x) s_dct[i] = F.dct28[i];
  if (PLP) {
    for (int i = threadIdx.x; i < 32; i += blockDim.x) s_plp[i] = F.plp_eql[i];
    for (int i = threadIdx.x; i < 16; i += blockDim.x) s_plp[32 + i] = F.plp_sin[i];
  }
  __syncthreads();

  uint32_t mo[UC];
#pragma unroll
  for (int i = 0; i < UC; ++i) mo[i] = F.melo[i * 16 + j];
  const uint32_t lane_bands = (uint32_t)F.lane_bands[j];
  const int band0 = (int)((lane_bands >> 8) & 0xffu), band1 = (int)((lane_bands >> 16) & 0xffu);
  float uf0[UC], uf1[UC];
#pragma unroll
  for (int i = 0; i < UC; ++i) { uf0[i] = ((lane_bands >> i) & 1u) ? 1.0f : 0.0f; uf1[i] = 1.0f - uf0[i]; }
  const uint32_t out_off = (uint32_t)(g * (int)P.ld_out + j) * 4u;
  const uint32_t out_off_d = out_off + (uint32_t)P.n_mfcc * 4u;
  const uint32_t out_off_dd = out_off + (uint32_t)P.n_mfcc * 8u;
  const float nkpre = P.de ? P.k : -P.k;
  const int m0 = P.pad_left >> 5, j0 = (P.pad_left >> 1) & 15;
  float *pb_k = s_pb + pb_pos(j);
  float *pb_m = s_pb + pb_pos(256 - j);

  const Dft16K dk;
  PHASE_DECL
  const int tile_stride = __builtin_amdgcn_readfirstlane((int)gridDim.x) * kWavesPerBlock;
  int tile = blockIdx.x * kWavesPerBlock + wave;
  const int n_tiles = DELTA ? P.n_ftiles : P.n_tiles;
  if (tile >= n_tiles) return;
  typedef typename std::conditional<DELTA, FTileRec, TileRec>::type Rec;
  typedef const __attribute__((address_space(4))) Rec *ConstRecPtr;
  const ConstRecPtr recs = DELTA ? (ConstRecPtr)(uintptr_t)P.ftile_rec : (ConstRecPtr)(uintptr_t)P.tile_rec;
  int64_t cur_samp0 = recs[tile].samp0, cur_row0 = recs[tile].row0;
  int cur_n = recs[tile].n_frames;
  int cur_live = 0, cur_e0 = 0, cur_e1 = 0, cur_lo = 0, cur_don = 0;
  if constexpr (DELTA) {
    cur_live = recs[tile].live_n; cur_e0 = recs[tile].e0; cur_e1 = recs[tile].e1; cur_lo = recs[tile].lo; cur_don = recs[tile].delta_on;
  }
  bool has_next = tile + tile_stride < n_tiles;
  int64_t nxt_samp0 = cur_samp0;
  if (has_next) nxt_samp0 = recs[tile + tile_stride].samp0;
  int tp = 0;
  FrameRegs<MP, ALIGNED, PREEMPH> R;
  pcm_prefetch<MP, ALIGNED, PREEMPH>(P.pcm, P.pcm_total, cur_samp0 - P.pad_left, P.H, lane, R);
  unsigned char *pend_row = nullptr;
  float pend_val = 0.0f;
  bool pend_live = false;
  float s_prev = 0.0f, d_cur = 0.0f;
  int b_tp = 0, b_lo = 0, b_live = 0, b_e0 = 0, b_e1 = 0, b_don = 0;
  const auto from_group = [&](int grp, float v) {
    return __int_as_float(__builtin_amdgcn_ds_bpermute(4 * ((grp << 4) | j), __float_as_int(v)));
  };
  const auto regress = [](float vm2, float vm1, float vp1, float vp2) {
    float num = 0.0f;
    num += 1.0f * (vp1 - vm1);
    num += 2.0f * (vp2 - vm2);
    return num;
  };
  const auto div10 = [](float a, bool &plain) {
    const float y = 0.1f, b = 10.0f;
    plain |= div_needs_division(a);
    return div_markstein(a, b, y);
  };
  const auto delta_fast = [&](float s_cur, float dp, float &dn, float &ddn, float &drow, bool &plain) {
    const float s1 = from_group((g + 1) & 3, g == 0 ? s_cur : s_prev);
    const float s3 = from_group((g + 3) & 3, g == 3 ? s_prev : s_cur);
    dn = div10(regress(s_prev, s1, s3, s_cur), plain);
    const float d1 = from_group((g + 1) & 3, g == 0 ? dn : dp);
    const float d3 = from_group((g + 3) & 3, g == 3 ? dp : dn);
    ddn = div10(regress(dp, d1, d3, dn), plain);
    drow = from_group((g + 2) & 3, g >= 2 ? dp : dn);
  };
  const auto delta_exact = [&](float s_cur, float dp, int btp, int lo, int live_n, float &dn, float &ddn, float &drow) {
    const auto fetch = [&](int x, int hi_c, int base, float cur, float prev) {
      x = x < lo ? lo : (x > hi_c ? hi_c : x);
      const int dd = x - base;
      const float c = from_group(dd & 3, cur), p = from_group(dd & 3, prev);
      return dd >= 0 ? c : p;
    };
    const float norm = 10.0f;
    const int fd = btp - 2 + g, fdd = btp - 4 + g, hi0 = live_n - 1, hi1 = live_n + 1;
    dn = regress(fetch(fd - 2, hi0, btp, s_cur, s_prev), fetch(fd - 1, hi0, btp, s_cur, s_prev), fetch(fd + 1, hi0, btp, s_cur, s_prev),
                 fetch(fd + 2, hi0, btp, s_cur, s_prev)) / norm;
    ddn = regress(fetch(fdd - 2, hi1, btp - 2, dn, dp), fetch(fdd - 1, hi1, btp - 2, dn, dp), fetch(fdd + 1, hi1, btp - 2, dn, dp),
                  fetch(fdd + 2, hi1, btp - 2, dn, dp)) / norm;
    drow = from_group((g + 2) & 3, g >= 2 ? dp : dn);
  };

  for (;;) {
    const bool live = tp + g < (DELTA ? cur_live : cur_n);
    PHASE(0);
    if constexpr (!DELTA) {
      if (pend_row != nullptr && pend_live) {
        uint32_t oo = out_off;
        asm volatile("" : "+v"(oo));
        *reinterpret_cast<float *>(pend_row + oo) = pend_val;
      }
    }
    float st_dn = 0.0f, st_ddn = 0.0f, st_drow = 0.0f;
    bool st_plain = false;
    if constexpr (DELTA) delta_fast(pend_val, d_cur, st_dn, st_ddn, st_drow, st_plain);
    float re[16], im[16];
    {
      float tprev = 0.0f;
      (void)tprev;
#pragma unroll
      for (int m = 0; m < 16; ++m) {
        if (m < MP) {
          float a, b;
          if constexpr (ALIGNED && !kB16Samples) {
            a = (float)(int16_t)(R.v[m] & 0xffffu);
            b = (float)(int16_t)(R.v[m] >> 16);
          } else {
            a = (float)(int32_t)R.v[2 * m];
            b = (float)(int32_t)R.v[2 * m + 1];
          }
          float ya = a, yb = b;
          if (PREEMPH) {
            float pa;
            if constexpr (kPredLoads) {
              pa = (float)(int32_t)R.p[m];
            } else {
              const float t = dpp_f<0x121>(b);
              pa = (j == 0) ? tprev : t;
              tprev = t;
            }
#ifndef SMILEHIP_MFCC512_PREEMPH_TWO_ROUNDINGS
            yb = fmaf(nkpre, a, b);
            ya = fmaf(nkpre, pa, a);
#else
            yb = b + nkpre * a;
            ya = a + nkpre * pa;
#endif
            if (PAD0 ? (m == 0 && j == 0) : (m == m0 && j == j0)) ya = P.one_minus_k * a;
          }
          const float2 w = s_win[m * 16 + j];
          re[m] = ya * w.x;
          im[m] = yb * w.y;
        } else {
          re[m] = 0.0f; im[m] = 0.0f;
        }
      }
    }
    PHASE(1);
    if constexpr (DELTA) {
      const bool clamped = !(b_tp - 6 >= b_lo && b_tp + 3 <= b_live - 1);
      if (clamped || __builtin_amdgcn_ballot_w64(st_plain && j < P.n_mfcc) != 0) delta_exact(pend_val, d_cur, b_tp, b_lo, b_live, st_dn, st_ddn, st_drow);
      const int fdd = b_tp - 4 + g;
      const bool row_live = pend_row != nullptr && j < P.n_mfcc && fdd >= b_e0 && fdd < b_e1;
      if (row_live) {
        uint32_t oo = out_off;
        asm volatile("" : "+v"(oo));
        *reinterpret_cast<float *>(pend_row + oo) = s_prev;
      }
      if (row_live && b_don) {
        uint32_t oo = out_off_d;
        asm volatile("" : "+v"(oo));
        *reinterpret_cast<float *>(pend_row + oo) = st_drow;
        oo = out_off_dd;
        asm volatile("" : "+v"(oo));
        *reinterpret_cast<float *>(pend_row + oo) = st_ddn;
      }
      s_prev = pend_val;
      d_cur = st_dn;
    }

    float2 *tbw = reinterpret_cast<float2 *>(wbase) + g * 16 + j;
    const float2 *tbr = reinterpret_cast<const float2 *>(wbase) + g * 16 + j * kTB2Row;
    if constexpr (kWritesEarly) {
      float2 w[4], wn[4];
#pragma unroll
      for (int p = 1; p < 4; ++p) w[p] = s_tw256[(4 * p) * 16 + j];
      w[0] = make_float2(1.0f, 0.0f);
#pragma unroll
      for (int m0 = 0; m0 < 4; ++m0) dft16_first(re, im, m0);
      dft16_twiddles(re, im, dk);
#pragma unroll
      for (int q = 0; q < 4; ++q) {
        if (q < 3) {
#pragma unroll
          for (int p = 0; p < 4; ++p) wn[p] = s_tw256[(q + 1 + 4 * p) * 16 + j];
        }
        dft16_last(re, im, q);
#pragma unroll
        for (int p = 0; p < 4; ++p) {
          const int k1 = q + 4 * p;
          if (k1 > 0) cmul(re[4 * q + p], im[4 * q + p], w[p].x, w[p].y);
          tbw[k1 * kTB2Row] = make_float2(re[4 * q + p], im[4 * q + p]);
        }
#pragma unroll
        for (int p = 0; p < 4; ++p) w[p] = wn[p];
      }
    } else {
      dft16(re, im, dk);
#pragma unroll
      for (int k1 = 1; k1 < 16; ++k1) {
        const float2 w = s_tw256[k1 * 16 + j];
        cmul(re[k1], im[k1], w.x, w.y);
      }
#pragma unroll
      for (int k1 = 0; k1 < 16; ++k1) tbw[k1 * kTB2Row] = make_float2(re[k1], im[k1]);
    }
    PHASE(3);
    {
      wave_lds_fence();
#pragma unroll
      for (int i = 0; i < 16; ++i) {
        const int jj = kReadsInDftOrder ? (i >> 2) + 4 * (i & 3) : i;
        typedef const volatile __attribute__((address_space(3))) unsigned long long *LdsU64;
        const unsigned long long v = ((LdsU64)tbr)[jj];
        re[jj] = __int_as_float((int)(uint32_t)v); im[jj] = __int_as_float((int)(uint32_t)(v >> 32));
      }
      wave_lds_fence();
    }
    PHASE(4);
#ifndef SMILEHIP_DEBUG_SKIP_DFT2
    dft16(re, im, dk);
#endif
    PHASE(5);

    float zr[8], zi[8];
#ifdef SMILEHIP_MFCC512_BPERMUTE_PARTNER
    {
      const int paddr = 4 * ((lane & 48) | ((16 - j) & 15));
#pragma unroll
      for (int q = 0; q < 8; ++q) {
        float c = __int_as_float(__builtin_amdgcn_ds_bpermute(paddr, __float_as_int(re[15 - q])));
        float d = __int_as_float(__builtin_amdgcn_ds_bpermute(paddr, __float_as_int(im[15 - q])));
        if (q > 0) { c = (j == 0) ? re[16 - q] : c; d = (j == 0) ? im[16 - q] : d; }
        zr[q] = c; zi[q] = d;
      }
    }
#else
#pragma unroll
    for (int q = 0; q < 8; ++q) {
      const float pr = q > 0 ? dpp_f<0x12f>(re[(16 - q) & 15]) : re[15];
      const float pi = q > 0 ? dpp_f<0x12f>(im[(16 - q) & 15]) : im[15];
      const float tr = __int_as_float(__builtin_amdgcn_update_dpp(__float_as_int(pr), __float_as_int(re[15 - q]), 0x101, 0xf, 0xf, false));
      const float ti = __int_as_float(__builtin_amdgcn_update_dpp(__float_as_int(pi), __float_as_int(im[15 - q]), 0x101, 0xf, 0xf, false));
      zr[q] = kMirrorOperand ? tr : dpp_f<0x140>(tr);
      zi[q] = kMirrorOperand ? ti : dpp_f<0x140>(ti);
    }
#endif
    float2 tw5[8];
#pragma unroll
    for (int q = 0; q < 8; ++q) tw5[q] = s_tw512[j + 16 * q];
#pragma unroll
    for (int q = 0; q < 8; ++q) {
      const float2 w = tw5[q];
      const float a = re[q], b = im[q];
      const float c = kMirrorAtUse ? dpp_f<0x140>(zr[q]) : zr[q], d = kMirrorAtUse ? dpp_f<0x140>(zi[q]) : zi[q];
      const float sr = a + c, si = b - d, dr = a - c, di = b + d;
      const float ur = fmaf(w.x, dr, -w.y * di);
      const float ui = fmaf(w.x, di, w.y * dr);
      const float xr = sr + ui, xi = si - ur;
      const float yr = sr - ui, yi = si + ur;
      float pk = fmaf(xi, xi, xr * xr);
      float pm = fmaf(yi, yi, yr * yr);
      if (q == 0 && j == 0) {
        const float v0 = 2.0f * (a + b), v1 = 2.0f * (a - b);
        pk = v0 * v0; pm = v1 * v1;
      }
      if (!USE_POWER) { pk = sqrtf(pk); pm = sqrtf(pm); }
      pb_k[(2 * kOctetFloats) * q] = pk;
      pb_m[-(2 * kOctetFloats) * q] = pm;
    }
    if (j == 0) {
      const float a = re[8], b = im[8];
      const float s = 4.0f * fmaf(b, b, a * a);
      s_pb[pb_pos(128)] = USE_POWER ? s : sqrtf(s);
    } else if (j < 8) {
      s_pb[pb_pos(256) + j] = 0.0f;
    }
    wave_lds_fence();

    PHASE(6);
    int ntp = tp + 4;
    const bool advance = ntp >= cur_n;
    const bool more = !advance || has_next;
    if (advance) ntp = 0;
    if (more)
      pcm_prefetch<MP, ALIGNED, PREEMPH>(P.pcm, P.pcm_total, (advance ? nxt_samp0 : cur_samp0) + (int64_t)ntp * P.H - P.pad_left, P.H, lane, R);

    PHASE(7);
    {
      float a0 = 0.0f, a1 = 0.0f;
#pragma unroll
      for (int i = 0; i < UC; ++i) {
        const float4 *pp = reinterpret_cast<const float4 *>(reinterpret_cast<const unsigned char *>(s_pb) + mo[i]);
        const float4 p0 = pp[0], p1 = pp[1];
        const float4 w0 = s_melw0[i * 16 + j], w1 = s_melw1[i * 16 + j];
        float acc = p0.x * w0.x;
        acc = fmaf(p0.y, w0.y, acc); acc = fmaf(p0.z, w0.z, acc); acc = fmaf(p0.w, w0.w, acc);
        acc = fmaf(p1.x, w1.x, acc); acc = fmaf(p1.y, w1.y, acc); acc = fmaf(p1.z, w1.z, acc); acc = fmaf(p1.w, w1.w, acc);
        a0 = fmaf(acc, uf0[i], a0);
        a1 = fmaf(acc, uf1[i], a1);
      }
      PHASE(8);
#pragma unroll
      for (int h = 0; h < 2; ++h) {
        const int b = h ? band1 : band0;
        const float acc = h ? a1 : a0;
        if (b != 0xff) {
          if (PLP) {
            float v = acc * F.mel_scale;
            v = v < P.melfloor ? P.melfloor : v;
            s_lmel[b] = __expf(P.plp_compression * __logf(v * s_plp[b]));
          } else {
            s_lmel[b] = log_mel_fast(acc * F.mel_scale, P.melfloor, P.log_floor);
          }
        }
      }
      if (j + 16 >= P.n_bands) s_lmel[j + 16] = 0.0f;
      if (j >= P.n_bands) s_lmel[j] = 0.0f;
    }
    wave_lds_fence();

    PHASE(9);
    if (PLP) {
      float *s_acf = s_lmel + 32;
      if (j <= P.plp_order) s_acf[j] = plp_acf_lag(s_lmel, s_dct + j * 28, P.n_bands);
      wave_lds_fence();
      if (j == 0) plp_cc_serial(s_acf, P.plp_order, s_plp + 32, s_cep);
      wave_lds_fence();
      if (j < P.n_mfcc) pend_val = s_cep[j];
    } else
    if (j < P.n_mfcc) {
      const float4 *row_c = reinterpret_cast<const float4 *>(s_dct + j * 28);
      const float4 *lm = reinterpret_cast<const float4 *>(s_lmel);
      float acc = 0.0f, dgain = 0.0f;
#pragma unroll
      for (int q = 0; q < 7; ++q) {
        const float4 l = lm[q], c = row_c[q];
        acc = fmaf(l.x, c.x, acc); acc = fmaf(l.y, c.y, acc); acc = fmaf(l.z, c.z, acc);
        if (q < 6) acc = fmaf(l.w, c.w, acc); else dgain = c.w;
      }
      pend_val = acc * dgain;
    }
    pend_live = live && j < P.n_mfcc;
    pend_row = reinterpret_cast<unsigned char *>(P.out + (cur_row0 + tp - (DELTA ? 4 : 0)) * P.ld_out);
    if constexpr (DELTA) { b_tp = tp; b_lo = cur_lo; b_live = cur_live; b_e0 = cur_e0; b_e1 = cur_e1; b_don = cur_don; }
    wave_lds_fence();
    PHASE(10);
    if (!more) break;
    if (advance) {
      tile += tile_stride;
      cur_samp0 = nxt_samp0; cur_row0 = recs[tile].row0; cur_n = recs[tile].n_frames;
      if constexpr (DELTA) {
        cur_live = recs[tile].live_n; cur_e0 = recs[tile].e0; cur_e1 = recs[tile].e1; cur_lo = recs[tile].lo; cur_don = recs[tile].delta_on;
      }
      has_next = tile + tile_stride < n_tiles;
      if (has_next) nxt_samp0 = recs[tile + tile_stride].samp0;
    }
    tp = ntp;
  }
  if constexpr (DELTA) {
    float dn, ddn, drow;
    delta_exact(pend_val, d_cur, b_tp, b_lo, b_live, dn, ddn, drow);
    const int fdd = b_tp - 4 + g;
    if (j < P.n_mfcc && fdd >= b_e0 && fdd < b_e1) {
      *reinterpret_cast<float *>(pend_row + out_off) = s_prev;
      if (b_don) {
        *reinterpret_cast<float *>(pend_row + out_off_d) = drow;
        *reinterpret_cast<float *>(pend_row + out_off_dd) = ddn;
      }
    }
  } else if (pend_live) {
    uint32_t oo = out_off;
    asm volatile("" : "+v"(oo));
    *reinterpret_cast<float *>(pend_row + oo) = pend_val;
  }
  PHASE_FLUSH;
}

template <int MP, bool PREEMPH, bool USE_POWER, bool ALIGNED, bool PLP, int UC, bool DELTA = false>
__global__ void __launch_bounds__(kWavesPerBlock * 64, 4) lld_mfcc512(LldParams P, Fast512Tables F) {
  lld_mfcc512_body<MP, PREEMPH, USE_POWER, ALIGNED, PLP, UC, DELTA, true>(P, F);
}
template <int MP, bool PREEMPH, bool USE_POWER, bool ALIGNED, bool PLP, int UC, bool DELTA = false>
__global__ void __launch_bounds__(kWavesPerBlock * 64, 4) lld_mfcc512_padded(LldParams P, Fast512Tables F) {
  lld_mfcc512_body<MP, PREEMPH, USE_POWER, ALIGNED, PLP, UC, DELTA, false>(P, F);
}

#ifdef SMILEHIP_PHASE_TIMING
extern "C" int smilehip_debug_phase(unsigned long long *out16, int reset) {
  if (out16 && hipMemcpyFromSymbol(out16, HIP_SYMBOL(g_phase), sizeof(unsigned long long) * 16) != hipSuccess) return -1;
  if (reset) {
    unsigned long long z[16] = {0};
    if (hipMemcpyToSymbol(HIP_SYMBOL(g_phase), z, sizeof(z)) != hipSuccess) return -1;
  }
  return 0;
}
#endif

bool fast512_applicable(int Nfft, int N) { return Nfft == 512 && N <= 512 && N >= 2; }

int fast512_tile_frames() { return kTileFrames; }

int fast512_build_host(const smilehip_lld_config &cfg, const Geometry &geo, const std::vector<float> &window,
                       const MelBank &mel, const DctTables &dct, Fast512Host &h) {
  const int pad_left = cfg.zero_pad_symmetric ? (int)((geo.Nfft - geo.N) / 2) : 0;
  const int H = (int)geo.H, N = (int)geo.N;
  if (mel.n_bands > 27 || dct.n_mfcc > 16 || cfg.win_offset != 0.0 || (pad_left & 1) || (H & 1) || H < 2) return -1;
  h.mp = (pad_left + N) <= 13 * 32 ? 13 : 16;
  const char *fp = getenv("SMILEHIP_MFCC512_FORCE_PADDED");
  h.force_padded = fp != nullptr && fp[0] == '1';
  h.tw256.resize(256);
  for (int k1 = 0; k1 < 16; ++k1)
    for (int j = 0; j < 16; ++j) {
      const double a = -2.0 * M_PI * double(j * k1) / 256.0;
      h.tw256[k1 * 16 + j] = make_float2(float(cos(a)), float(sin(a)));
    }
  h.tw512.resize(256);
  for (int k = 0; k < 256; ++k) {
    const double a = -2.0 * M_PI * double(k) / 512.0;
    h.tw512[k] = make_float2(float(cos(a)), float(sin(a)));
  }
  h.win.assign(size_t(h.mp) * 16, make_float2(0.f, 0.f));
  for (int m = 0; m < h.mp; ++m)
    for (int j = 0; j < 16; ++j) {
      const int n = 2 * (j + 16 * m) - pad_left;
      float a = 0.f, b = 0.f;
      if (n >= 0 && n < N) a = float(double(window[n]) / 32767.0);
      if (n + 1 >= 0 && n + 1 < N) b = float(double(window[n + 1]) / 32767.0);
      h.win[size_t(m) * 16 + j] = make_float2(a, b);
    }
  struct Unit { int octet; float w[8]; };
  std::vector<Unit> units;
  const int nb = mel.n_bands;
  std::vector<int> first_unit(nb + 1, 0);
  for (int b = 0; b < nb; ++b) {
    int lo = -1, hi = -1;
    if (mel.rise_hi[b] > mel.rise_lo[b]) { lo = mel.rise_lo[b]; hi = mel.rise_hi[b]; }
    if (mel.fall_hi[b] > mel.fall_lo[b]) { if (lo < 0) lo = mel.fall_lo[b]; hi = mel.fall_hi[b]; }
    first_unit[b] = int(units.size());
    if (lo >= 0) {
      for (int o = lo / 8; o <= (hi - 1) / 8; ++o) {
        Unit un;
        un.octet = o;
        for (int e = 0; e < 8; ++e) {
          const int n = 8 * o + e;
          float w = 0.0f;
          if (n >= mel.rise_lo[b] && n < mel.rise_hi[b]) w = 1.0f - mel.coef[n];
          else if (n >= mel.fall_lo[b] && n < mel.fall_hi[b]) w = mel.coef[n];
          un.w[e] = w;
        }
        units.push_back(un);
      }
    }
  }
  first_unit[nb] = int(units.size());
  h.n_slots = int(units.size());
  std::vector<int> size(nb), order(nb);
  for (int b = 0; b < nb; ++b) { size[b] = first_unit[b + 1] - first_unit[b]; order[b] = b; }
  std::stable_sort(order.begin(), order.end(), [&](int x, int y) { return size[x] > size[y]; });
  int cap = 0;
  std::vector<std::pair<int, int>> lanes;
  for (int c : {6, 8}) {
    lanes.clear();
    std::vector<char> used(nb, 0);
    bool ok = true;
    for (int oi = 0; oi < nb && ok; ++oi) {
      const int a = order[oi];
      if (used[a]) continue;
      used[a] = 1;
      if (size[a] > c) { ok = false; break; }
      int partner = -1;
      for (int oj = oi + 1; oj < nb; ++oj)
        if (!used[order[oj]] && size[a] + size[order[oj]] <= c) { partner = order[oj]; break; }
      if (partner >= 0) used[partner] = 1;
      lanes.push_back({a, partner});
    }
    if (ok && (int)lanes.size() <= 16) { cap = c; break; }
  }
  if (cap == 0) return -1;
  h.mel_units = cap;
  std::vector<std::vector<int>> slot(16, std::vector<int>(cap, -1));
  for (size_t l = 0; l < lanes.size(); ++l) {
    int pos = 0;
    for (int which = 0; which < 2; ++which) {
      const int b = which ? lanes[l].second : lanes[l].first;
      if (b < 0) continue;
      for (int c = first_unit[b]; c < first_unit[b + 1]; ++c) slot[l][pos++] = c;
    }
  }
  auto step_cost = [&](int i, int &worst, int &coll) {
    int cnt[16] = {0};
    for (int l = 0; l < 16; ++l)
      if (slot[l][i] >= 0) ++cnt[units[slot[l][i]].octet & 15];
    worst = 1; coll = 0;
    for (int r = 0; r < 16; ++r) { worst = std::max(worst, cnt[r]); coll += std::max(0, cnt[r] - 1); }
  };
  auto total_cost = [&](long &primary, long &secondary) {
    primary = secondary = 0;
    for (int i = 0; i < cap; ++i) { int w, c; step_cost(i, w, c); primary += w; secondary += c; }
  };
  long best_p, best_s;
  total_cost(best_p, best_s);
  for (bool improved = true; improved;) {
    improved = false;
    for (int l = 0; l < 16; ++l)
      for (int a = 0; a < cap; ++a)
        for (int b = a + 1; b < cap; ++b) {
          if (slot[l][a] == slot[l][b]) continue;
          std::swap(slot[l][a], slot[l][b]);
          long p, s2;
          total_cost(p, s2);
          if (p < best_p || (p == best_p && s2 < best_s)) { best_p = p; best_s = s2; improved = true; }
          else std::swap(slot[l][a], slot[l][b]);
        }
  }
  h.mel_conflict_steps = int(best_p - cap);
  if (getenv("SMILEHIP_DEBUG_TABLES"))
    fprintf(stderr, "fast512: %d mel units on %zu lanes, %d per lane, bank model: %ld extra cycles over %d steps (%ld colliding lanes)\n",
            h.n_slots, lanes.size(), cap, best_p - cap, cap, best_s);
  h.melw.assign(size_t(cap) * 16 * 2, make_float4(0.f, 0.f, 0.f, 0.f));
  h.melo.assign(size_t(cap) * 16, 0u);
  h.lane_bands.assign(16, int32_t(0xffff00));
  for (int i = 0; i < cap; ++i) {
    bool taken[16] = {false};
    for (int l = 0; l < 16; ++l)
      if (slot[l][i] >= 0) taken[units[slot[l][i]].octet & 15] = true;
    for (int l = 0; l < 16; ++l) {
      const size_t idx = size_t(i) * 16 + l;
      if (slot[l][i] >= 0) {
        const Unit &un = units[slot[l][i]];
        h.melw[2 * idx] = make_float4(un.w[0], un.w[1], un.w[2], un.w[3]);
        h.melw[2 * idx + 1] = make_float4(un.w[4], un.w[5], un.w[6], un.w[7]);
        h.melo[idx] = uint32_t(un.octet) * uint32_t(kOctetFloats * 4);
      } else {
        int o = 0;
        for (int r = 0; r < 16; ++r)
          if (!taken[r]) { o = r; taken[r] = true; break; }
        h.melo[idx] = uint32_t(o) * uint32_t(kOctetFloats * 4);
      }
    }
  }
  for (size_t l = 0; l < lanes.size(); ++l) {
    uint32_t mask = 0;
    const int b0 = lanes[l].first;
    for (int i = 0; i < cap; ++i)
      if (slot[l][i] >= first_unit[b0] && slot[l][i] < first_unit[b0 + 1]) mask |= 1u << i;
    h.lane_bands[l] = int32_t(mask | (uint32_t(b0) << 8) | (uint32_t(lanes[l].second < 0 ? 0xff : lanes[l].second) << 16));
  }
  h.mel_scale = mel.scale * (cfg.use_power ? 0.25f : 0.5f);
  h.dct28.assign(16 * 28, 0.0f);
  for (int r = 0; r < dct.n_mfcc; ++r)
    for (int m = 0; m < mel.n_bands; ++m) h.dct28[size_t(r) * 28 + m] = dct.cos_rows[size_t(r) * mel.n_bands + m];
  for (int r = 0; r < dct.n_mfcc; ++r) h.dct28[size_t(r) * 28 + 27] = dct.gain[r];
  return 0;
}

template <int MP, bool PREEMPH, bool USE_POWER, bool ALIGNED, bool PLP, int UC, bool DELTA = false>
static hipError_t launch_mfcc512_one(bool padded, unsigned grid, size_t lds, hipStream_t s, const LldParams &P, const Fast512Tables &F) {
  if constexpr (PREEMPH) {
    if (padded) {
      hipError_t e = hipFuncSetAttribute(reinterpret_cast<const void *>(&lld_mfcc512_padded<MP, PREEMPH, USE_POWER, ALIGNED, PLP, UC, DELTA>),
                                         hipFuncAttributeMaxDynamicSharedMemorySize, (int)lds);
      if (e != hipSuccess) return e;
      SMILEHIP_KLAUNCH((lld_mfcc512_padded<MP, PREEMPH, USE_POWER, ALIGNED, PLP, UC, DELTA>), dim3(grid), dim3(kWavesPerBlock * 64), lds, s, P, F);
      return hipSuccess;
    }
  }
  hipError_t e = hipFuncSetAttribute(reinterpret_cast<const void *>(&lld_mfcc512<MP, PREEMPH, USE_POWER, ALIGNED, PLP, UC, DELTA>),
                                     hipFuncAttributeMaxDynamicSharedMemorySize, (int)lds);
  if (e != hipSuccess) return e;
  SMILEHIP_KLAUNCH((lld_mfcc512<MP, PREEMPH, USE_POWER, ALIGNED, PLP, UC, DELTA>), dim3(grid), dim3(kWavesPerBlock * 64), lds, s, P, F);
  return hipSuccess;
}

hipError_t launch_mfcc512(const LldParams &P, const Fast512Tables &F, const Fast512Host &h, bool aligned, bool fused_delta, hipStream_t s) {
  const int shared_floats = 256 * 2 + h.mp * 16 * 2 + 256 * 2 + h.mel_units * 16 * 8 + 16 * 28 + 48;
  const size_t lds = sizeof(float) * (size_t(shared_floats) + size_t(kWavesPerBlock) * kWaveFloats);
  if (fused_delta && (!aligned || !P.ftile_rec || P.n_ftiles <= 0)) return hipErrorInvalidValue;
  unsigned grid = (unsigned)(((fused_delta ? P.n_ftiles : P.n_tiles) + kWavesPerBlock - 1) / kWavesPerBlock);
  if (grid > (unsigned)h.max_blocks) grid = (unsigned)h.max_blocks;
#ifdef SMILEHIP_DEBUG_KNOBS
  if (const char *e = getenv("SMILEHIP_DEBUG_GRID")) grid = (unsigned)atoi(e);
#endif
  bool launched = false;
  const bool padded = P.pad_left != 0 || h.force_padded;
#define SMILEHIP_LAUNCH(...)                                                                                    \
  {                                                                                                             \
    hipError_t e = launch_mfcc512_one<__VA_ARGS__>(padded, grid, lds, s, P, F);                                 \
    if (e != hipSuccess) return e;                                                                              \
    launched = true;                                                                                            \
  }
#define SMILEHIP_MATCH(MPV, PE, UP, AL, PL, UCV)                                                                \
  (!launched && h.mp == MPV && (P.preemph != 0) == PE && (P.use_power != 0) == UP && aligned == AL && (P.plp != 0) == PL && h.mel_units == UCV)
#define SMILEHIP_PICK_UD(MPV, PE, UP, PL, UCV) \
  if (fused_delta && SMILEHIP_MATCH(MPV, PE, UP, true, PL, UCV)) SMILEHIP_LAUNCH(MPV, PE, UP, true, PL, UCV, true)
#define SMILEHIP_PICK_U(MPV, PE, UP, AL, PL, UCV) \
  if (!fused_delta && SMILEHIP_MATCH(MPV, PE, UP, AL, PL, UCV)) SMILEHIP_LAUNCH(MPV, PE, UP, AL, PL, UCV)
#define SMILEHIP_PICK(MPV, PE, UP, AL, PL) SMILEHIP_PICK_U(MPV, PE, UP, AL, PL, 6) SMILEHIP_PICK_U(MPV, PE, UP, AL, PL, 8)
#define SMILEHIP_PICKD(MPV, PE, UP, PL) SMILEHIP_PICK_UD(MPV, PE, UP, PL, 6) SMILEHIP_PICK_UD(MPV, PE, UP, PL, 8)
#define SMILEHIP_PICK2(MPV, PE, UP) SMILEHIP_PICK(MPV, PE, UP, true, false) SMILEHIP_PICK(MPV, PE, UP, false, false) SMILEHIP_PICKD(MPV, PE, UP, false)
#define SMILEHIP_PICK4(MPV) SMILEHIP_PICK2(MPV, true, true) SMILEHIP_PICK2(MPV, true, false) \
                            SMILEHIP_PICK2(MPV, false, true) SMILEHIP_PICK2(MPV, false, false) \
                             \
                            SMILEHIP_PICK(MPV, true, true, true, true) SMILEHIP_PICK(MPV, true, true, false, true) \
                            SMILEHIP_PICK(MPV, false, true, true, true) SMILEHIP_PICK(MPV, false, true, false, true) \
                            SMILEHIP_PICKD(MPV, true, true, true) SMILEHIP_PICKD(MPV, false, true, true)
  SMILEHIP_PICK4(13)
  SMILEHIP_PICK4(16)
#undef SMILEHIP_PICK4
#undef SMILEHIP_PICK2
#undef SMILEHIP_PICKD
#undef SMILEHIP_PICK
#undef SMILEHIP_PICK_U
#undef SMILEHIP_PICK_UD
#undef SMILEHIP_MATCH
#undef SMILEHIP_LAUNCH
  if (!launched) return hipErrorInvalidConfiguration;
  return hipGetLastError();
}

}
```

### opensmile_amd/csrc/smilehip_batch.cpp

```cpp
#include "smilehip_internal.hpp"
#include "batch_layout.hpp"

smilehip_batch::~smilehip_batch() { delete f0_batch; }

static inline bool mfcc_like(const smilehip_plan *p) {
  return p->cfg.chain_kind == SMILEHIP_CHAIN_MFCC || p->cfg.chain_kind == SMILEHIP_CHAIN_PLP;
}

static BatchLayoutSpec layout_spec(const smilehip_plan *plan) {
  const smilehip_lld_config &c = plan->cfg;
  BatchLayoutSpec s;
  s.chain_kind = c.chain_kind;
  s.N = plan->geo.N; s.H = plan->geo.H; s.period = plan->geo.period;
  s.row_extra = plan_row_extra(plan);
  s.fused_delta_eligible = plan->use_fast && mfcc_like(plan) && c.n_delta == 2 && c.delta_win == 2 && !c.append_log_energy && !c.cms &&
                           !getenv("SMILEHIP_NO_FUSED_DELTA");
  s.fast_slots = std::max<int64_t>(1, plan->fast.max_blocks) * 8;
  s.tile_frames = plan->use_fast ? fast512_tile_frames() : (c.chain_kind == SMILEHIP_CHAIN_COMPARE_F0 ? f0_tile_frames() : (int64_t(1) << 40));
  s.dtile_rows = chain_tile_rows(); s.short_T = chain_short_max(); s.jitter_chunk = jitter_chunk_frames();
  if (const char *rf = getenv("SMILEHIP_RUN_FRAMES")) { const int v = atoi(rf); if (v >= 1 && v <= 4096) s.run_frames_override = v; }
  return s;
}

static inline size_t at_least_one(int64_t n) { return size_t(n ? n : 1); }

static int alloc_mfcc_scratch(const smilehip_plan *plan, smilehip_batch *b, const BatchLayout &L) {
  b->n_ftiles = (int32_t)L.ftiles.size();
  if (b->n_ftiles) return b->d_ftile_rec.upload(L.ftiles);
  if (plan->cfg.n_delta > 0 && b->total_frames > 0 && b->d_static.alloc(size_t(b->total_frames) * size_t(plan_n_static(plan))))
    return fail(SMILEHIP_ERR_HIP, "hipMalloc of the static-block scratch failed");
  return SMILEHIP_OK;
}

static int alloc_is09_scratch(smilehip_batch *b, const BatchLayout &L) {
  int rc;
  if (b->total_frames > 0 && (rc = b->d_frame_utt.upload(L.frame_utt))) return rc;
  if (b->d_raw16.alloc(size_t(b->total_frames) * 16)) return fail(SMILEHIP_ERR_HIP, "hipMalloc of the IS09 scratch matrix failed");
  return SMILEHIP_OK;
}

static int alloc_compare_ab_scratch(smilehip_batch *b, const BatchLayout &L) {
  int rc;
  b->n_runs = (int32_t)L.run_utt.size();
  if ((rc = b->d_run_utt.upload(L.run_utt)) || (rc = b->d_run_t0.upload(L.run_t0))) return rc;
  const size_t nf = at_least_one(b->total_frames);
  if (b->d_rawA.alloc(nf * 4) || b->d_rawB.alloc(nf * 55) || b->d_mel1.alloc(nf * 26) || b->d_b_extra.alloc(at_least_one(b->n_utt) * 110))
    return fail(SMILEHIP_ERR_HIP, "hipMalloc of the ComParE scratch matrices failed");
  (void)hipMemset(b->d_rawA.p, 0, nf * 4 * sizeof(float));
  return SMILEHIP_OK;
}

static int alloc_f0_scratch(const smilehip_plan *plan, smilehip_batch *b, const BatchLayout &L) {
  const size_t nf = at_least_one(b->total_frames);
  if (b->d_shs.alloc(nf * 21) || b->d_e60.alloc(nf)) return fail(SMILEHIP_ERR_HIP, "hipMalloc of the F0 scratch matrices failed");
  const size_t nab = (size_t)std::max<int64_t>(f0_scratch_doubles(b->n_tiles, (int)plan->geo.K), 1);
  if (b->d_f0_ab.alloc(nab)) return fail(SMILEHIP_ERR_HIP, "hipMalloc of the F0 row scratch (%zu MB) failed", nab * sizeof(double) >> 20);
  static const bool pipe_on = [] { const char *e = getenv("SMILEHIP_F0_PIPE"); return e && e[0] == '1'; }();
  if (pipe_on && b->n_tiles > f0_chunk_tiles()) {
    size_t free_b = 0, total_b = 0;
    if (hipMemGetInfo(&free_b, &total_b) != hipSuccess || free_b / 4 <= nab * sizeof(double) || b->d_f0_ab2.alloc(nab))
      (void)hipGetLastError();
  }
  int rc;
  const std::vector<int32_t> zp(at_least_one(b->n_utt), 0);
  if ((rc = b->d_pending.upload(zp)) || (rc = b->d_jit_redo.upload(zp)) || (rc = b->d_jit_utt.upload(L.jit_utt)) ||
      (rc = b->d_jit_t0.upload(L.jit_t0)) || (rc = b->d_jit_ctl.upload(std::vector<int32_t>(2, 0))))
    return rc;
  return SMILEHIP_OK;
}

static int alloc_compare_scratch(smilehip_plan *plan, smilehip_batch *b, const BatchLayout &L) {
  int rc;
  if ((rc = alloc_compare_ab_scratch(b, L)) || (rc = smilehip_batch_create(plan->f0_plan, b->h_samp_off.data(), b->n_utt, &b->f0_batch)))
    return rc;
  const size_t nf = at_least_one(b->f0_batch->total_frames);
  if (b->d_pitch2.alloc(nf * 2) || b->d_jit4.alloc(nf * 4)) return fail(SMILEHIP_ERR_HIP, "hipMalloc of the F0 group's scratch matrices failed");
  return SMILEHIP_OK;
}

static void try_keep_magnitudes(const smilehip_plan *f0_plan, smilehip_batch *fb) {
  if (fb->total_frames <= 0) return;
  const int64_t ld = (f0_plan->geo.K + 3) & ~int64_t(3);
  const size_t n = size_t(fb->total_frames) * size_t(ld);
  size_t free_b = 0, total_b = 0;
  const char *env = getenv("SMILEHIP_HARM_KEEP_MAG");
  bool keep = hipMemGetInfo(&free_b, &total_b) == hipSuccess && n * sizeof(float) <= free_b / 2;
  if (env && env[0] == '0') keep = false;
  if (env && env[0] == '1') keep = true;
  if (keep && fb->d_mag_keep.alloc(n) == SMILEHIP_OK)
    fb->mag_ld = ld;
  else
    (void)hipGetLastError();
}

static int alloc_egemaps_scratch(smilehip_plan *plan, smilehip_batch *b, const BatchLayout &L) {
  int rc;
  b->n_runs = (int32_t)L.run_utt.size();
  if ((rc = b->d_run_utt.upload(L.run_utt)) || (rc = b->d_run_t0.upload(L.run_t0)) || (rc = b->d_fin_off.upload(b->h_fin_off)) ||
      (rc = smilehip_batch_create(plan->f0_plan, b->h_samp_off.data(), b->n_utt, &b->f0_batch)))
    return rc;
  const size_t nf = at_least_one(b->total_frames), nf60 = at_least_one(b->f0_batch->total_frames), nfin = at_least_one(b->h_fin_off[b->n_utt]);
  if (b->d_raw20.alloc(nf * 12) || b->d_spec220.alloc(nf * 220) || b->d_lpc.alloc(nf * 12) || b->d_formants.alloc(nf * 10) ||
      b->d_pitch3.alloc(nf60 * 3) || b->d_jit4.alloc(nf60 * 4) || b->d_shim.alloc(nf60) || b->d_harm6.alloc(nf60 * 6) ||
      b->d_func_in.alloc(nfin * 36))
    return fail(SMILEHIP_ERR_HIP, "hipMalloc of the eGeMAPS scratch matrices failed (%.1f GB needed)",
                double(nf * 254 + nf60 * 14 + nfin * 36) * 4e-9);
  if ((rc = b->d_pending_j.upload(std::vector<int32_t>(at_least_one(b->n_utt), 0))) || (rc = b->d_harm_ctl.upload(std::vector<int32_t>(2, 0))) ||
      (rc = b->d_fm_flags.upload(std::vector<uint64_t>(2 * ((nf + 63) / 64), 0))))
    return rc;
  try_keep_magnitudes(plan->f0_plan, b->f0_batch);
  return SMILEHIP_OK;
}

extern "C" int smilehip_batch_create(smilehip_plan *plan, const int64_t *h_off, int32_t n_utt, smilehip_batch **out) {
  if (!plan || !out || n_utt < 0 || (n_utt > 0 && !h_off)) return fail(SMILEHIP_ERR_INVALID, "smilehip_batch_create: bad argument");
  *out = nullptr;
  if (!plan->ctx) return fail(SMILEHIP_ERR_NO_DEVICE, "host-only plan: no device attached (tables only)");
  if (plan->stage_mask != SMILEHIP_STAGE_ALL) return fail(SMILEHIP_ERR_INVALID, "single-component plan cannot run the fused chain");
  if (int rt = require_transform(plan, "smilehip_batch_create")) return rt;
  HIP_TRY(hipSetDevice(plan->ctx->device));
  std::unique_ptr<smilehip_batch> b(new (std::nothrow) smilehip_batch());
  if (!b) return fail(SMILEHIP_ERR_NOMEM, "out of host memory");
  BatchLayout L;
  if (const int bad = batch_layout(layout_spec(plan), h_off, n_utt, L))
    return fail(SMILEHIP_ERR_INVALID, "sample offsets must be non-decreasing (utterance %d)", bad - 1);
  b->plan = plan;
  b->n_utt = n_utt;
  b->total_frames = L.total_frames; b->total_rows = L.total_rows;
  b->n_tiles = (int32_t)L.tile_utt.size(); b->n_dtiles = (int32_t)L.dtile_utt.size();
  b->run_frames = L.run_frames; b->all_even = L.all_even;
  int rc;
  if ((rc = b->d_samp_off.upload(L.samp_off)) || (rc = b->d_frame_off.upload(L.frame_off)) || (rc = b->d_row_off.upload(L.row_off)) ||
      (rc = b->d_tile_utt.upload(L.tile_utt)) || (rc = b->d_tile_t0.upload(L.tile_t0)) || (rc = b->d_tile_rec.upload(L.tile_rec)) ||
      (rc = b->d_dtile_utt.upload(L.dtile_utt)) || (rc = b->d_dtile_t0.upload(L.dtile_t0)) || (rc = b->d_short.upload(L.short_utts)))
    return rc;
  b->h_samp_off = std::move(L.samp_off);
  b->h_frame_off = std::move(L.frame_off); b->h_row_off = std::move(L.row_off);
  b->h_fin_off = std::move(L.fin_off); b->h_short = std::move(L.short_utts);
  switch (plan->cfg.chain_kind) {
    case SMILEHIP_CHAIN_IS09: rc = alloc_is09_scratch(b.get(), L); break;
    case SMILEHIP_CHAIN_COMPARE_AB: rc = alloc_compare_ab_scratch(b.get(), L); break;
    case SMILEHIP_CHAIN_COMPARE_F0: rc = alloc_f0_scratch(plan, b.get(), L); break;
    case SMILEHIP_CHAIN_COMPARE: rc = alloc_compare_scratch(plan, b.get(), L); break;
    case SMILEHIP_CHAIN_EGEMAPS: rc = alloc_egemaps_scratch(plan, b.get(), L); break;
    case SMILEHIP_CHAIN_MFCC:
    case SMILEHIP_CHAIN_PLP: rc = alloc_mfcc_scratch(plan, b.get(), L); break;
  }
  if (rc) return rc;
  *out = b.release();
  return SMILEHIP_OK;
}

extern "C" void smilehip_batch_destroy(smilehip_batch *b) { delete b; }
extern "C" int64_t smilehip_batch_total_frames(const smilehip_batch *b) { return b ? b->total_frames : 0; }
extern "C" int64_t smilehip_batch_total_rows(const smilehip_batch *b) { return b ? b->total_rows : 0; }
extern "C" int smilehip_batch_delta_fused(const smilehip_batch *b) { return b && b->n_ftiles > 0 ? 1 : 0; }
extern "C" int smilehip_batch_frame_offsets(const smilehip_batch *b, int64_t *o) {
  if (!b || !o) return fail(SMILEHIP_ERR_INVALID, "smilehip_batch_frame_offsets: null argument");
  std::memcpy(o, b->h_row_off.data(), b->h_row_off.size() * sizeof(int64_t));
  return SMILEHIP_OK;
}

static bool serial_forced() {
  static const bool v = [] { const char *e = getenv("SMILEHIP_SERIAL"); return e && e[0] != '0'; }();
  return v;
}
static bool serial_streams(int64_t total_frames) {
  static const int forced = [] { const char *e = getenv("SMILEHIP_SERIAL"); return e ? (e[0] == '0' ? 0 : 1) : -1; }();
  return forced >= 0 ? forced != 0 : total_frames >= (int64_t)4000000;
}
static void fill_params(const smilehip_plan *p, const smilehip_batch *b, const int16_t *d_pcm, float *d_out,
                        int64_t ld, LldParams &P) {
  std::memset(&P, 0, sizeof(P));
  P.pcm = d_pcm;
  P.pcm_f32 = b->run_pcm_f32;
  P.pcm_total = b->h_samp_off.back();
  P.samp_off = b->d_samp_off.p;
  P.frame_off = b->d_frame_off.p;
  P.frame_utt = b->d_frame_utt.p;
  P.tile_utt = b->d_tile_utt.p;
  P.tile_t0 = b->d_tile_t0.p;
  P.tile_rec = b->d_tile_rec.p;
  P.ftile_rec = b->d_ftile_rec.p;
  P.n_ftiles = b->n_ftiles;
  P.n_utt = b->n_utt;
  P.n_tiles = b->n_tiles;
  P.total_frames = b->total_frames;
  P.out = d_out;
  P.ld_out = ld;
  P.N = (int32_t)p->geo.N;
  P.H = (int32_t)p->geo.H;
  P.Nfft = (int32_t)p->geo.Nfft;
  P.K = (int32_t)p->geo.K;
  P.pad_left = p->cfg.zero_pad_symmetric ? (int32_t)((p->geo.Nfft - p->geo.N) / 2) : 0;
  P.preemph = p->cfg.preemph;
  P.de = p->cfg.preemph_de;
  P.k = p->cfg.preemph_k;
  P.one_minus_k = 1 - p->cfg.preemph_k;
  P.win_offset = (float)p->cfg.win_offset;
  P.window = p->d_window.p;
  P.oo = p->oo.tab();
  P.mel_coef = p->d_mel_coef.p;
  P.mel_rng = p->d_mel_rng.p;
  P.mel_scale = p->mel.scale;
  P.use_power = p->cfg.use_power;
  P.n_bands = p->mel.n_bands;
  P.dct_rows = p->d_dct_rows.p;
  P.dct_gain = p->d_dct_gain.p;
  P.n_mfcc = p->dct.n_mfcc;
  P.melfloor = p->dct.melfloor;
  P.log_floor = p->dct.log_floor;
  P.plp = p->cfg.chain_kind == SMILEHIP_CHAIN_PLP;
  P.plp_order = p->cfg.plp_lp_order;
  P.plp_compression = p->cfg.plp_compression;
  P.plp_eql = p->d_plp_eql.p;
  P.plp_cos = p->d_plp_cos.p;
  P.plp_sin = p->d_plp_sin.p;
}

static ChainParams chain_params(const smilehip_batch *b, const float *x, int64_t ld_x, int32_t D, float *out, int64_t ld_out) {
  ChainParams Q;
  std::memset(&Q, 0, sizeof(Q));
  Q.frame_off = b->d_frame_off.p;
  Q.row_off = b->d_row_off.p;
  Q.tile_utt = b->d_dtile_utt.p;
  Q.tile_t0 = b->d_dtile_t0.p;
  Q.n_tiles = b->n_dtiles;
  Q.n_utt = b->n_utt;
  Q.x = x;
  Q.ld_x = ld_x;
  Q.out = out;
  Q.ld_out = ld_out;
  Q.D = D;
  Q.short_T = chain_short_max();
  Q.short_utts = b->d_short.p;
  Q.n_short = (int32_t)b->h_short.size();
  return Q;
}

static int delta_chain_from(smilehip_plan *plan, smilehip_batch *b, const float *d_x, int64_t ld_x, int copy_col, float *d_io,
                            int64_t ld, int32_t D, int32_t W, int32_t n_orders, void *stream) {
  if (!plan || !b || !d_io) return fail(SMILEHIP_ERR_INVALID, "smilehip_delta_chain: null argument");
  if (n_orders < 1 || n_orders > 2 || W < 1 || W > 4 || D < 1 || D > 64 || ld < (int64_t)D * (1 + n_orders))
    return fail(SMILEHIP_ERR_INVALID, "smilehip_delta_chain: unsupported D=%d W=%d orders=%d ld=%lld", D, W, n_orders, (long long)ld);
  if (b->total_frames == 0) return SMILEHIP_OK;
  if (b->total_rows != b->total_frames) return fail(SMILEHIP_ERR_INVALID, "smilehip_delta_chain: batch belongs to a chain with extra rows");
  ChainParams Q = chain_params(b, d_x, ld_x, D, d_io, ld);
  Q.copy_col = copy_col;
  Q.n_stages = n_orders;
  Q.kind[0] = Q.kind[1] = 0;
  Q.W[0] = Q.W[1] = W;
  Q.out_col[0] = D;
  Q.out_col[1] = 2 * D;
  hipError_t e = launch_chain(Q, (hipStream_t)stream);
  if (e != hipSuccess) return fail(SMILEHIP_ERR_HIP, "window-chain kernel launch failed: %s", hipGetErrorString(e));
  return SMILEHIP_OK;
}

extern "C" int smilehip_delta_chain(smilehip_plan *plan, smilehip_batch *b, float *d_io, int64_t ld, int32_t D,
                                    int32_t W, int32_t n_orders, void *stream) {
  return delta_chain_from(plan, b, d_io, ld, -1, d_io, ld, D, W, n_orders, stream);
}

extern "C" int smilehip_mfcc_run(smilehip_plan *plan, smilehip_batch *b, const int16_t *d_pcm, float *d_out,
                                 int64_t ld_out, void *stream) {
  if (!plan || !b || b->plan != plan) return fail(SMILEHIP_ERR_INVALID, "smilehip_mfcc_run: plan/batch mismatch");
  if (plan->cfg.chain_kind != SMILEHIP_CHAIN_MFCC && plan->cfg.chain_kind != SMILEHIP_CHAIN_PLP)
    return fail(SMILEHIP_ERR_INVALID, "smilehip_mfcc_run: plan is not an MFCC / PLP chain (use smilehip_lld_run)");
  const int n_static = plan_n_static(plan), n_cep = plan->dct.n_mfcc;
  const int n_out = n_static * (1 + plan->cfg.n_delta);
  if (ld_out < n_out) return fail(SMILEHIP_ERR_INVALID, "ld_out %lld < n_out %d", (long long)ld_out, n_out);
  if (b->total_frames == 0) return SMILEHIP_OK;
  if (!d_pcm || !d_out) return fail(SMILEHIP_ERR_INVALID, "smilehip_mfcc_run: null device pointer");
  hipStream_t s = (hipStream_t)stream;
  LldParams P;
  fill_params(plan, b, d_pcm, d_out, ld_out, P);
  const bool aligned_in = b->all_even && ((reinterpret_cast<uintptr_t>(d_pcm) & 3) == 0);
  const bool fused_delta = plan->use_fast && !b->run_pcm_f32 && b->n_ftiles > 0 && aligned_in;
  const bool compact = !fused_delta && plan->cfg.n_delta > 0 && b->d_static.p != nullptr;
  if (compact) {
    P.out = b->d_static.p;
    P.ld_out = n_static;
  }
  hipEvent_t *ev = plan->ev[plan->n_timed % smilehip_plan::kRing];
  if (plan->timing) {
    for (int i = 0; i < 3; ++i)
      if (!ev[i]) HIP_TRY(hipEventCreate(&ev[i]));
    HIP_TRY(hipEventRecord(ev[0], s));
  }
  hipError_t e;
  if (plan->use_fast && !b->run_pcm_f32) {
    Fast512Tables F;
    F.tw256 = plan->d_tw256.p;
    F.tw512 = plan->d_tw512.p;
    F.win = plan->d_fwin.p;
    F.melw = plan->d_melw.p;
    F.melo = plan->d_melo.p;
    F.dct28 = plan->d_dct28.p;
    F.lane_bands = plan->d_lane_bands.p;
    F.mel_units = plan->fast.mel_units;
    F.mel_scale = plan->fast.mel_scale;
    F.plp_eql = plan->d_plp_eql.p;
    F.plp_sin = plan->d_plp_sin.p;
    const bool aligned = aligned_in;
    e = launch_mfcc512(P, F, plan->fast, aligned, fused_delta, s);
  } else {
    e = launch_mfcc_generic(P, s);
  }
  if (e != hipSuccess) return fail(SMILEHIP_ERR_HIP, "mfcc kernel launch failed: %s", hipGetErrorString(e));
  if (plan->cfg.append_log_energy) {
    e = launch_log_energy(P, b->d_dtile_utt.p, b->d_dtile_t0.p, b->n_dtiles, P.out, P.ld_out, n_cep, s);
    if (e != hipSuccess) return fail(SMILEHIP_ERR_HIP, "log-energy kernel launch failed: %s", hipGetErrorString(e));
  }
  if (plan->timing) HIP_TRY(hipEventRecord(ev[1], s));
  if (fused_delta) {
    if (!b->h_short.empty()) {
      ChainParams Q = chain_params(b, d_out, ld_out, n_static, d_out, ld_out);
      Q.tile_utt = Q.tile_t0 = nullptr; Q.n_tiles = 0;
      Q.copy_col = -1;
      Q.n_stages = 2;
      Q.kind[0] = Q.kind[1] = 0;
      Q.W[0] = Q.W[1] = plan->cfg.delta_win;
      Q.out_col[0] = n_static;
      Q.out_col[1] = 2 * n_static;
      e = launch_chain(Q, s);
      if (e != hipSuccess) return fail(SMILEHIP_ERR_HIP, "window-chain kernel launch failed: %s", hipGetErrorString(e));
    }
  } else if (plan->cfg.n_delta > 0) {
    int rc = compact ? delta_chain_from(plan, b, b->d_static.p, n_static, 0, d_out, ld_out, n_static,
                                        plan->cfg.delta_win, plan->cfg.n_delta, stream)
                     : smilehip_delta_chain(plan, b, d_out, ld_out, n_static, plan->cfg.delta_win, plan->cfg.n_delta, stream);
    if (rc) return rc;
  }
  if (plan->cfg.cms) {
    e = launch_cms(b->d_frame_off.p, b->n_utt, P.out, P.ld_out, d_out, ld_out, n_cep, s);
    if (e != hipSuccess) return fail(SMILEHIP_ERR_HIP, "mean-subtraction kernel launch failed: %s", hipGetErrorString(e));
  }
  if (plan->timing) {
    HIP_TRY(hipEventRecord(ev[2], s));
    plan->n_timed++;
  }
  return SMILEHIP_OK;
}

static int timing_mark(smilehip_plan *plan, int which, hipStream_t s) {
  if (!plan->timing) return SMILEHIP_OK;
  hipEvent_t *ev = plan->ev[plan->n_timed % smilehip_plan::kRing];
  if (!ev[which]) HIP_TRY(hipEventCreate(&ev[which]));
  HIP_TRY(hipEventRecord(ev[which], s));
  if (which == 2) plan->n_timed++;
  return SMILEHIP_OK;
}

static int is09_run(smilehip_plan *plan, smilehip_batch *b, const int16_t *d_pcm, float *d_out, int64_t ld_out, void *stream) {
  const int n_out = plan_n_out(plan);
  if (ld_out < n_out) return fail(SMILEHIP_ERR_INVALID, "ld_out %lld < n_out %d", (long long)ld_out, n_out);
  if (b->total_frames == 0) return SMILEHIP_OK;
  if (!d_pcm || !d_out) return fail(SMILEHIP_ERR_INVALID, "smilehip_lld_run: null device pointer");
  hipStream_t s = (hipStream_t)stream;
  LldParams P;
  fill_params(plan, b, d_pcm, d_out, ld_out, P);
  Is09Params I;
  I.raw16 = b->d_raw16.p;
  I.fsSec = (float)plan->geo.fft_frame_size_sec;
  I.maxPitch = plan->cfg.pitch_max;
  I.voicingCutoff = plan->cfg.voicing_cutoff;
  if (I.voicingCutoff > 1.0) I.voicingCutoff = 1.0;
  if (I.voicingCutoff < 0.0) I.voicingCutoff = 0.0;
  if (I.maxPitch < 0.0) I.maxPitch = 0.0;
  int trc;
  if ((trc = timing_mark(plan, 0, s))) return trc;
  hipError_t e = launch_is09(P, I, s);
  if (e != hipSuccess) return fail(SMILEHIP_ERR_HIP, "IS09 kernel launch failed: %s", hipGetErrorString(e));
  if ((trc = timing_mark(plan, 1, s))) return trc;
  ChainParams Q = chain_params(b, b->d_raw16.p, 16, 16, d_out, ld_out);
  Q.copy_col = -1;
  Q.n_stages = 2;
  Q.kind[0] = 1; Q.W[0] = plan->cfg.sma_win / 2;
  Q.kind[1] = 0; Q.W[1] = plan->cfg.delta_win;
  Q.out_col[0] = 0;
  Q.out_col[1] = 16;
  e = launch_chain(Q, s);
  if (e != hipSuccess) return fail(SMILEHIP_ERR_HIP, "window-chain kernel launch failed: %s", hipGetErrorString(e));
  return timing_mark(plan, 2, s);
}

static int compare_run(smilehip_plan *plan, smilehip_batch *b, const int16_t *d_pcm, float *d_out, int64_t ld_out, void *stream,
                       int de_col = 59) {
  const int n_out = plan_n_out(plan);
  if (ld_out < n_out) return fail(SMILEHIP_ERR_INVALID, "ld_out %lld < n_out %d", (long long)ld_out, n_out);
  if (b->total_frames == 0 || b->total_rows == 0) return SMILEHIP_OK;
  if (!d_pcm || !d_out) return fail(SMILEHIP_ERR_INVALID, "smilehip_lld_run: null device pointer");
  hipStream_t s = (hipStream_t)stream;
  LldParams P;
  fill_params(plan, b, d_pcm, d_out, ld_out, P);
  CompareParams Q;
  std::memset(&Q, 0, sizeof(Q));
  Q.run_utt = b->d_run_utt.p;
  Q.run_t0 = b->d_run_t0.p;
  Q.run_frames = b->run_frames;
  Q.rawA = b->d_rawA.p;
  Q.rawB = b->d_rawB.p;
  Q.mel1 = b->d_mel1.p;
  Q.eql = plan->d_eql.p;
  Q.eql_log = plan->d_eql_log.p;
  Q.sharp_w = plan->d_sharp.p;
  Q.plp_melfloor = 0.00000000093f;
  Q.compression = 0.33f;
  Q.rasta_iir = plan->rasta_iir;
  for (int i = 0; i < 5; ++i) Q.rasta_fir[i] = plan->rasta_fir[i];
  Q.fsSec = plan->geo.fft_frame_size_sec;
  Q.N60 = (int32_t)samples_60ms(plan->geo.period);
  Q.max_utt_samples = 0;
  for (size_t u2 = 0; u2 + 1 < b->h_samp_off.size(); ++u2) Q.max_utt_samples = std::max<int64_t>(Q.max_utt_samples, b->h_samp_off[u2 + 1] - b->h_samp_off[u2]);
  for (int i = 0; i < 2; ++i) {
    Q.band_iL[i] = plan->band_iL[i]; Q.band_iR[i] = plan->band_iR[i];
    Q.band_wL[i] = plan->band_wL[i]; Q.band_wR[i] = plan->band_wR[i];
  }
  Q.slope_Sf = plan->slope_Sf;
  Q.slope_S2f = plan->slope_S2f;
  int trc;
  if ((trc = timing_mark(plan, 0, s))) return trc;
  hipError_t e = launch_compare(P, Q, b->n_runs, b->d_row_off.p, b->total_rows, d_out, ld_out, de_col, s);
  if (e != hipSuccess) return fail(SMILEHIP_ERR_HIP, "ComParE kernel launch failed: %s", hipGetErrorString(e));
  if ((trc = timing_mark(plan, 1, s))) return trc;
  ChainParams C = chain_params(b, b->d_rawB.p, 55, 55, d_out, ld_out);
  C.copy_col = -1;
// ... 381 lines not shown
```

Before: 2.862 billion.

## Skip dead delta-tail passes, prune first FFT layer, and rebalance fused tile split

Adds a fast path for trailing passes in delta mode where only delta outputs remain, skipping the FFT, mel and DCT work. Specialises the first radix-4 FFT layer when the fourth input group is zero, and adds an optional early mel-weight load. Rewrites the fused-tile layout cost model so that halo passes are counted and each utterance is split into balanced pass counts. It also exposes a user-selectable tile length through a new API. This mixes several ideas, and the layout change may alter how work is spread across slots.

```diff
diff --git a/include/smilehip.h b/include/smilehip.h
--- a/include/smilehip.h
+++ b/include/smilehip.h
@@ -261,6 +261,8 @@
 
 int  smilehip_batch_create(smilehip_plan *plan, const int64_t *h_sample_offsets, int32_t n_utt,
                            smilehip_batch **batch);
+int  smilehip_batch_create_tiled(smilehip_plan *plan, const int64_t *h_sample_offsets, int32_t n_utt,
+                                 int32_t fused_tile_frames, smilehip_batch **batch);
 void smilehip_batch_destroy(smilehip_batch *batch);
 int64_t smilehip_batch_total_frames(const smilehip_batch *batch);
 int64_t smilehip_batch_total_rows(const smilehip_batch *batch);
diff --git a/opensmile_amd/capi.py b/opensmile_amd/capi.py
--- a/opensmile_amd/capi.py
+++ b/opensmile_amd/capi.py
@@ -223,6 +223,7 @@
     "smilehip_plan_get_lifter": (_i64, [_vp, _vp, _i64]),
     "smilehip_batch_f0_pending": (C.c_int, [_vp, _vp]),
     "smilehip_batch_create": (C.c_int, [_vp, _vp, _i32, C.POINTER(_vp)]),
+    "smilehip_batch_create_tiled": (C.c_int, [_vp, _vp, _i32, _i32, C.POINTER(_vp)]),
     "smilehip_batch_destroy": (None, [_vp]),
     "smilehip_batch_total_frames": (_i64, [_vp]),
     "smilehip_batch_frame_offsets": (C.c_int, [_vp, _vp]),
@@ -600,14 +601,14 @@
 
 class Batch:
 
-    def __init__(self, plan, sample_offsets):
+    def __init__(self, plan, sample_offsets, fused_tile_frames=0):
         self.plan = plan
         off = np.ascontiguousarray(sample_offsets, dtype=np.int64)
         assert off.ndim == 1 and len(off) >= 1
         self.n_utt = len(off) - 1
         self.sample_offsets = off
         self._h = _vp()
-        _check(load().smilehip_batch_create(plan._h, off.ctypes.data, self.n_utt, C.byref(self._h)))
+        _check(load().smilehip_batch_create_tiled(plan._h, off.ctypes.data, self.n_utt, fused_tile_frames, C.byref(self._h)))
         self.total_frames = int(load().smilehip_batch_total_frames(self._h))
         self.total_rows = int(load().smilehip_batch_total_rows(self._h))
         self.delta_fused = bool(load().smilehip_batch_delta_fused(self._h))
diff --git a/opensmile_amd/csrc/batch_layout.hpp b/opensmile_amd/csrc/batch_layout.hpp
--- a/opensmile_amd/csrc/batch_layout.hpp
+++ b/opensmile_amd/csrc/batch_layout.hpp
@@ -2,6 +2,7 @@
 #include <algorithm>
 #include <cmath>
 #include <cstdint>
+#include <functional>
 #include <map>
 #include <vector>
 
@@ -22,6 +23,7 @@
   int short_T = 0;
   int jitter_chunk = 0;
   int run_frames_override = 0;
+  int64_t fused_tile_frames = 0;
 };
 
 struct BatchLayout {
@@ -57,28 +59,50 @@
   return T60 >= (compare ? 4 : 1) ? T60 + 1 : 0;
 }
 
+inline int64_t fused_tile_passes(const FTileRec &r) { return r.n_frames / 4 - (r.e1 == r.live_n ? 1 : 0); }
+inline int64_t fused_parts(int64_t T, int64_t L) {
+  const int64_t Q = (T + 3) / 4, most = Q <= 3 ? std::min<int64_t>(Q, 2) : Q - 2;
+  return std::min((T + L - 1) / L, most);
+}
 inline void layout_fused_tiles(const BatchLayoutSpec &s, const int64_t *h_off, int32_t n_utt, BatchLayout &out) {
-  const auto parts_of = [&](int64_t T, int64_t L) { return (T + L - 1) / L; };
-  int64_t bestL = 32;
-  double best = 1e300;
-  std::map<int64_t, int64_t> hist;
-  for (int32_t u = 0; u < n_utt; ++u) {
-    const int64_t T = out.frame_off[u + 1] - out.frame_off[u];
-    if (T > 0) hist[T]++;
-  }
-  for (int64_t L = 32; L <= 2048; L += 4) {
-    int64_t n = 0;
-    for (const auto &h : hist) n += h.second * ((h.first <= s.short_T) ? 1 : parts_of(h.first, L));
-    const double cost = double((n + s.fast_slots - 1) / s.fast_slots) * double(L / 4 + 2);
-    if (cost <= best) { best = cost; bestL = L; }
+  int64_t bestL = s.fused_tile_frames >= 4 ? (s.fused_tile_frames & ~int64_t(3)) : 0;
+  if (bestL == 0) {
+    std::map<int64_t, int64_t> hist;
+    for (int32_t u = 0; u < n_utt; ++u) {
+      const int64_t T = out.frame_off[u + 1] - out.frame_off[u];
+      if (T > 0) hist[T]++;
+    }
+    double best = 1e300;
+    std::map<int64_t, int64_t, std::greater<int64_t>> by_passes;
+    for (int64_t L = 32; L <= 2048; L += 4) {
+      by_passes.clear();
+      for (const auto &h : hist) {
+        const int64_t Q = (h.first + 3) / 4, k = (h.first <= s.short_T) ? 1 : fused_parts(h.first, L), total = Q + 2 * k - 2;
+        by_passes[total / k] += h.second * (k - total % k);
+        if (total % k) by_passes[total / k + 1] += h.second * (total % k);
+      }
+      double cost = 0.0;
+      int64_t at = 0, seen = 0;
+      for (const auto &b : by_passes) {
+        seen += b.second;
+        if (at < seen) {
+          const int64_t n = (seen - at + s.fast_slots - 1) / s.fast_slots;
+          cost += double(n) * double(b.first);
+          at += n * s.fast_slots;
+        }
+      }
+      if (cost <= best) { best = cost; bestL = L; }
+    }
   }
   for (int32_t u = 0; u < n_utt; ++u) {
     const int64_t T = out.frame_off[u + 1] - out.frame_off[u];
     if (T <= 0) continue;
-    const int64_t parts = (T <= s.short_T) ? 1 : parts_of(T, bestL);
-    const int64_t len = (((T + parts - 1) / parts) + 3) & ~int64_t(3);
-    for (int64_t t0 = 0; t0 < T; t0 += len) {
-      const int64_t t1 = std::min<int64_t>(T, t0 + len), p0 = t0 > 0 ? t0 - 4 : 0;
+    const int64_t Q = (T + 3) / 4, k = (T <= s.short_T) ? 1 : fused_parts(T, bestL), total = Q + 2 * k - 2;
+    int64_t t0 = 0;
+    for (int64_t i = 0; i < k; ++i) {
+      const int64_t passes = total / k + (i < total % k ? 1 : 0);
+      const int64_t halo = (i > 0 ? 1 : 0) + (i + 1 < k ? 1 : 0);
+      const int64_t t1 = i + 1 < k ? t0 + 4 * (passes - halo) : T, p0 = t0 > 0 ? t0 - 4 : 0;
       FTileRec r;
       r.samp0 = h_off[u] + p0 * s.H;
       r.row0 = out.frame_off[u] + p0;
@@ -90,6 +114,7 @@
       r.lo = (int32_t)(-p0);
       r.delta_on = T > s.short_T;
       out.ftiles.push_back(r);
+      t0 = t1;
     }
   }
   std::stable_sort(out.ftiles.begin(), out.ftiles.end(), [](const FTileRec &a, const FTileRec &c) { return a.n_frames > c.n_frames; });
diff --git a/opensmile_amd/csrc/lld_mfcc512.hip b/opensmile_amd/csrc/lld_mfcc512.hip
--- a/opensmile_amd/csrc/lld_mfcc512.hip
+++ b/opensmile_amd/csrc/lld_mfcc512.hip
@@ -53,6 +53,16 @@
   r3 = t1r - t3i; i3 = t1i + t3r;
 }
 
+__device__ __forceinline__ void dft4_no3(float &r0, float &i0, float &r1, float &i1, float &r2, float &i2, float &r3, float &i3) {
+  const float t0r = r0 + r2, t0i = i0 + i2;
+  const float t1r = r0 - r2, t1i = i0 - i2;
+  const float t2r = r1, t2i = i1;
+  r0 = t0r + t2r; i0 = t0i + t2i;
+  r2 = t0r - t2r; i2 = t0i - t2i;
+  r1 = t1r + t2i; i1 = t1i - t2r;
+  r3 = t1r - t2i; i3 = t1i + t2r;
+}
+
 __device__ __forceinline__ void cmul(float &r, float &i, float c, float s) {
   const float nr = fmaf(r, c, -i * s);
   const float ni = fmaf(r, s, i * c);
@@ -71,8 +81,18 @@
   }
 };
 
+#ifdef SMILEHIP_MFCC512_FULL_FIRST_LAYER
+constexpr bool kPrunedFirstLayer = false;
+#else
+constexpr bool kPrunedFirstLayer = true;
+#endif
+template <int NIN = 16>
 __device__ __forceinline__ void dft16_first(float (&re)[16], float (&im)[16], int m0) {
-  dft4(re[m0], im[m0], re[m0 + 4], im[m0 + 4], re[m0 + 8], im[m0 + 8], re[m0 + 12], im[m0 + 12]);
+  static_assert(NIN >= 12 && NIN <= 16, "only the fourth input of a first-layer group can be absent");
+  if (kPrunedFirstLayer && m0 + 12 >= NIN)
+    dft4_no3(re[m0], im[m0], re[m0 + 4], im[m0 + 4], re[m0 + 8], im[m0 + 8], re[m0 + 12], im[m0 + 12]);
+  else
+    dft4(re[m0], im[m0], re[m0 + 4], im[m0 + 4], re[m0 + 8], im[m0 + 8], re[m0 + 12], im[m0 + 12]);
 }
 __device__ __forceinline__ void dft16_twiddles(float (&re)[16], float (&im)[16], const Dft16K &K) {
   cmul_ns(re[1 + 4], im[1 + 4], K.c1, K.ns1, K.s1);
@@ -97,9 +117,10 @@
 #pragma unroll
   for (int k = 0; k < 16; ++k) { re[k] = tr[k]; im[k] = ti[k]; }
 }
+template <int NIN = 16>
 __device__ __forceinline__ void dft16(float (&re)[16], float (&im)[16], const Dft16K &K) {
 #pragma unroll
-  for (int m0 = 0; m0 < 4; ++m0) dft16_first(re, im, m0);
+  for (int m0 = 0; m0 < 4; ++m0) dft16_first<NIN>(re, im, m0);
   dft16_twiddles(re, im, K);
 #pragma unroll
   for (int q = 0; q < 4; ++q) dft16_last(re, im, q);
@@ -148,6 +169,16 @@
 constexpr bool kMirrorAtUse = false;
 #else
 constexpr bool kMirrorAtUse = kMirrorOperand;
+#endif
+#ifdef SMILEHIP_MFCC512_FULL_DEAD_PASSES
+constexpr bool kSkipDeadPasses = false;
+#else
+constexpr bool kSkipDeadPasses = true;
+#endif
+#ifdef SMILEHIP_MFCC512_MELW_EARLY
+constexpr bool kMelwEarly = true;
+#else
+constexpr bool kMelwEarly = false;
 #endif
 template <int MP, bool ALIGNED, bool PREEMPH>
 struct FrameRegs {
@@ -349,252 +380,272 @@
   for (;;) {
     const bool live = tp + g < (DELTA ? cur_live : cur_n);
     PHASE(0);
-    if constexpr (!DELTA) {
-      if (pend_row != nullptr && pend_live) {
-        uint32_t oo = out_off;
-        asm volatile("" : "+v"(oo));
-        *reinterpret_cast<float *>(pend_row + oo) = pend_val;
-      }
-    }
-    float st_dn = 0.0f, st_ddn = 0.0f, st_drow = 0.0f;
-    bool st_plain = false;
-    if constexpr (DELTA) delta_fast(pend_val, d_cur, st_dn, st_ddn, st_drow, st_plain);
-    float re[16], im[16];
-    {
-      float tprev = 0.0f;
-      (void)tprev;
-#pragma unroll
-      for (int m = 0; m < 16; ++m) {
-        if (m < MP) {
-          float a, b;
-          if constexpr (ALIGNED && !kB16Samples) {
-            a = (float)(int16_t)(R.v[m] & 0xffffu);
-            b = (float)(int16_t)(R.v[m] >> 16);
+    const bool dead = DELTA && kSkipDeadPasses && MP < 16 && !PLP && tp >= cur_live;
+    if (dead) {
+      float dn, ddn, drow;
+      delta_exact(pend_val, d_cur, b_tp, b_lo, b_live, dn, ddn, drow);
+      const int fdd = b_tp - 4 + g;
+      if (pend_row != nullptr && j < P.n_mfcc && fdd >= b_e0 && fdd < b_e1) {
+        *reinterpret_cast<float *>(pend_row + out_off) = s_prev;
+        if (b_don) {
+          *reinterpret_cast<float *>(pend_row + out_off_d) = drow;
+          *reinterpret_cast<float *>(pend_row + out_off_dd) = ddn;
+        }
+      }
+      s_prev = pend_val;
+      d_cur = dn;
+    } else {
+      if constexpr (!DELTA) {
+        if (pend_row != nullptr && pend_live) {
+          uint32_t oo = out_off;
+          asm volatile("" : "+v"(oo));
+          *reinterpret_cast<float *>(pend_row + oo) = pend_val;
+        }
+      }
+      float st_dn = 0.0f, st_ddn = 0.0f, st_drow = 0.0f;
+      bool st_plain = false;
+      if constexpr (DELTA) delta_fast(pend_val, d_cur, st_dn, st_ddn, st_drow, st_plain);
+      float re[16], im[16];
+      {
+        float tprev = 0.0f;
+        (void)tprev;
+#pragma unroll
+        for (int m = 0; m < 16; ++m) {
+          if (m < MP) {
+            float a, b;
+            if constexpr (ALIGNED && !kB16Samples) {
+              a = (float)(int16_t)(R.v[m] & 0xffffu);
+              b = (float)(int16_t)(R.v[m] >> 16);
+            } else {
+              a = (float)(int32_t)R.v[2 * m];
+              b = (float)(int32_t)R.v[2 * m + 1];
+            }
+            float ya = a, yb = b;
+            if (PREEMPH) {
+              float pa;
+              if constexpr (kPredLoads) {
+                pa = (float)(int32_t)R.p[m];
+              } else {
+                const float t = dpp_f<0x121>(b);
+                pa = (j == 0) ? tprev : t;
+                tprev = t;
+              }
+#ifndef SMILEHIP_MFCC512_PREEMPH_TWO_ROUNDINGS
+              yb = fmaf(nkpre, a, b);
+              ya = fmaf(nkpre, pa, a);
+#else
+              yb = b + nkpre * a;
+              ya = a + nkpre * pa;
+#endif
+              if (PAD0 ? (m == 0 && j == 0) : (m == m0 && j == j0)) ya = P.one_minus_k * a;
+            }
+            const float2 w = s_win[m * 16 + j];
+            re[m] = ya * w.x;
+            im[m] = yb * w.y;
           } else {
-            a = (float)(int32_t)R.v[2 * m];
-            b = (float)(int32_t)R.v[2 * m + 1];
+            re[m] = 0.0f; im[m] = 0.0f;
           }
-          float ya = a, yb = b;
-          if (PREEMPH) {
-            float pa;
-            if constexpr (kPredLoads) {
-              pa = (float)(int32_t)R.p[m];
-            } else {
-              const float t = dpp_f<0x121>(b);
-              pa = (j == 0) ? tprev : t;
-              tprev = t;
-            }
-#ifndef SMILEHIP_MFCC512_PREEMPH_TWO_ROUNDINGS
-            yb = fmaf(nkpre, a, b);
-            ya = fmaf(nkpre, pa, a);
-#else
-            yb = b + nkpre * a;
-            ya = a + nkpre * pa;
-#endif
-            if (PAD0 ? (m == 0 && j == 0) : (m == m0 && j == j0)) ya = P.one_minus_k * a;
+        }
+      }
+      PHASE(1);
+      if constexpr (DELTA) {
+        const bool clamped = !(b_tp - 6 >= b_lo && b_tp + 3 <= b_live - 1);
+        if (clamped || __builtin_amdgcn_ballot_w64(st_plain && j < P.n_mfcc) != 0) delta_exact(pend_val, d_cur, b_tp, b_lo, b_live, st_dn, st_ddn, st_drow);
+        const int fdd = b_tp - 4 + g;
+        const bool row_live = pend_row != nullptr && j < P.n_mfcc && fdd >= b_e0 && fdd < b_e1;
+        if (row_live) {
+          uint32_t oo = out_off;
+          asm volatile("" : "+v"(oo));
+          *reinterpret_cast<float *>(pend_row + oo) = s_prev;
+        }
+        if (row_live && b_don) {
+          uint32_t oo = out_off_d;
+          asm volatile("" : "+v"(oo));
+          *reinterpret_cast<float *>(pend_row + oo) = st_drow;
+          oo = out_off_dd;
+          asm volatile("" : "+v"(oo));
+          *reinterpret_cast<float *>(pend_row + oo) = st_ddn;
+        }
+        s_prev = pend_val;
+        d_cur = st_dn;
+      }
+
+      float2 *tbw = reinterpret_cast<float2 *>(wbase) + g * 16 + j;
+      const float2 *tbr = reinterpret_cast<const float2 *>(wbase) + g * 16 + j * kTB2Row;
+      if constexpr (kWritesEarly) {
+        float2 w[4], wn[4];
+#pragma unroll
+        for (int p = 1; p < 4; ++p) w[p] = s_tw256[(4 * p) * 16 + j];
+        w[0] = make_float2(1.0f, 0.0f);
+#pragma unroll
+        for (int m0 = 0; m0 < 4; ++m0) dft16_first<MP>(re, im, m0);
+        dft16_twiddles(re, im, dk);
+#pragma unroll
+        for (int q = 0; q < 4; ++q) {
+          if (q < 3) {
+#pragma unroll
+            for (int p = 0; p < 4; ++p) wn[p] = s_tw256[(q + 1 + 4 * p) * 16 + j];
           }
-          const float2 w = s_win[m * 16 + j];
-          re[m] = ya * w.x;
-          im[m] = yb * w.y;
-        } else {
-          re[m] = 0.0f; im[m] = 0.0f;
-        }
-      }
-    }
-    PHASE(1);
-    if constexpr (DELTA) {
-      const bool clamped = !(b_tp - 6 >= b_lo && b_tp + 3 <= b_live - 1);
-      if (clamped || __builtin_amdgcn_ballot_w64(st_plain && j < P.n_mfcc) != 0) delta_exact(pend_val, d_cur, b_tp, b_lo, b_live, st_dn, st_ddn, st_drow);
-      const int fdd = b_tp - 4 + g;
-      const bool row_live = pend_row != nullptr && j < P.n_mfcc && fdd >= b_e0 && fdd < b_e1;
-      if (row_live) {
-        uint32_t oo = out_off;
-        asm volatile("" : "+v"(oo));
-        *reinterpret_cast<float *>(pend_row + oo) = s_prev;
-      }
-      if (row_live && b_don) {
-        uint32_t oo = out_off_d;
-        asm volatile("" : "+v"(oo));
-        *reinterpret_cast<float *>(pend_row + oo) = st_drow;
-        oo = out_off_dd;
-        asm volatile("" : "+v"(oo));
-        *reinterpret_cast<float *>(pend_row + oo) = st_ddn;
-      }
-      s_prev = pend_val;
-      d_cur = st_dn;
-    }
-
-    float2 *tbw = reinterpret_cast<float2 *>(wbase) + g * 16 + j;
-    const float2 *tbr = reinterpret_cast<const float2 *>(wbase) + g * 16 + j * kTB2Row;
-    if constexpr (kWritesEarly) {
-      float2 w[4], wn[4];
-#pragma unroll
-      for (int p = 1; p < 4; ++p) w[p] = s_tw256[(4 * p) * 16 + j];
-      w[0] = make_float2(1.0f, 0.0f);
-#pragma unroll
-      for (int m0 = 0; m0 < 4; ++m0) dft16_first(re, im, m0);
-      dft16_twiddles(re, im, dk);
-#pragma unroll
-      for (int q = 0; q < 4; ++q) {
-        if (q < 3) {
-#pragma unroll
-          for (int p = 0; p < 4; ++p) wn[p] = s_tw256[(q + 1 + 4 * p) * 16 + j];
-        }
-        dft16_last(re, im, q);
-#pragma unroll
-        for (int p = 0; p < 4; ++p) {
-          const int k1 = q + 4 * p;
-          if (k1 > 0) cmul(re[4 * q + p], im[4 * q + p], w[p].x, w[p].y);
-          tbw[k1 * kTB2Row] = make_float2(re[4 * q + p], im[4 * q + p]);
-        }
-#pragma unroll
-        for (int p = 0; p < 4; ++p) w[p] = wn[p];
-      }
-    } else {
+          dft16_last(re, im, q);
+#pragma unroll
+          for (int p = 0; p < 4; ++p) {
+            const int k1 = q + 4 * p;
+            if (k1 > 0) cmul(re[4 * q + p], im[4 * q + p], w[p].x, w[p].y);
+            tbw[k1 * kTB2Row] = make_float2(re[4 * q + p], im[4 * q + p]);
+          }
+#pragma unroll
+          for (int p = 0; p < 4; ++p) w[p] = wn[p];
+        }
+      } else {
+        dft16<MP>(re, im, dk);
+#pragma unroll
+        for (int k1 = 1; k1 < 16; ++k1) {
+          const float2 w = s_tw256[k1 * 16 + j];
+          cmul(re[k1], im[k1], w.x, w.y);
+        }
+#pragma unroll
+        for (int k1 = 0; k1 < 16; ++k1) tbw[k1 * kTB2Row] = make_float2(re[k1], im[k1]);
+      }
+      PHASE(3);
+      {
+        wave_lds_fence();
+#pragma unroll
+        for (int i = 0; i < 16; ++i) {
+          const int jj = kReadsInDftOrder ? (i >> 2) + 4 * (i & 3) : i;
+          typedef const volatile __attribute__((address_space(3))) unsigned long long *LdsU64;
+          const unsigned long long v = ((LdsU64)tbr)[jj];
+          re[jj] = __int_as_float((int)(uint32_t)v); im[jj] = __int_as_float((int)(uint32_t)(v >> 32));
+        }
+        wave_lds_fence();
+      }
+      PHASE(4);
+#ifndef SMILEHIP_DEBUG_SKIP_DFT2
       dft16(re, im, dk);
-#pragma unroll
-      for (int k1 = 1; k1 < 16; ++k1) {
-        const float2 w = s_tw256[k1 * 16 + j];
-        cmul(re[k1], im[k1], w.x, w.y);
-      }
-#pragma unroll
-      for (int k1 = 0; k1 < 16; ++k1) tbw[k1 * kTB2Row] = make_float2(re[k1], im[k1]);
-    }
-    PHASE(3);
-    {
+#endif
+      PHASE(5);
+
+      float zr[8], zi[8];
+#ifdef SMILEHIP_MFCC512_BPERMUTE_PARTNER
+      {
+        const int paddr = 4 * ((lane & 48) | ((16 - j) & 15));
+#pragma unroll
+        for (int q = 0; q < 8; ++q) {
+          float c = __int_as_float(__builtin_amdgcn_ds_bpermute(paddr, __float_as_int(re[15 - q])));
+          float d = __int_as_float(__builtin_amdgcn_ds_bpermute(paddr, __float_as_int(im[15 - q])));
+          if (q > 0) { c = (j == 0) ? re[16 - q] : c; d = (j == 0) ? im[16 - q] : d; }
+          zr[q] = c; zi[q] = d;
+        }
+      }
+#else
+#pragma unroll
+      for (int q = 0; q < 8; ++q) {
+        const float pr = q > 0 ? dpp_f<0x12f>(re[(16 - q) & 15]) : re[15];
+        const float pi = q > 0 ? dpp_f<0x12f>(im[(16 - q) & 15]) : im[15];
+        const float tr = __int_as_float(__builtin_amdgcn_update_dpp(__float_as_int(pr), __float_as_int(re[15 - q]), 0x101, 0xf, 0xf, false));
+        const float ti = __int_as_float(__builtin_amdgcn_update_dpp(__float_as_int(pi), __float_as_int(im[15 - q]), 0x101, 0xf, 0xf, false));
+        zr[q] = kMirrorOperand ? tr : dpp_f<0x140>(tr);
+        zi[q] = kMirrorOperand ? ti : dpp_f<0x140>(ti);
+      }
+#endif
+      float2 tw5[8];
+#pragma unroll
+      for (int q = 0; q < 8; ++q) tw5[q] = s_tw512[j + 16 * q];
+#pragma unroll
+      for (int q = 0; q < 8; ++q) {
+        const float2 w = tw5[q];
+        const float a = re[q], b = im[q];
+        const float c = kMirrorAtUse ? dpp_f<0x140>(zr[q]) : zr[q], d = kMirrorAtUse ? dpp_f<0x140>(zi[q]) : zi[q];
+        const float sr = a + c, si = b - d, dr = a - c, di = b + d;
+        const float ur = fmaf(w.x, dr, -w.y * di);
+        const float ui = fmaf(w.x, di, w.y * dr);
+        const float xr = sr + ui, xi = si - ur;
+        const float yr = sr - ui, yi = si + ur;
+        float pk = fmaf(xi, xi, xr * xr);
+        float pm = fmaf(yi, yi, yr * yr);
+        if (q == 0 && j == 0) {
+          const float v0 = 2.0f * (a + b), v1 = 2.0f * (a - b);
+          pk = v0 * v0; pm = v1 * v1;
+        }
+        if (!USE_POWER) { pk = sqrtf(pk); pm = sqrtf(pm); }
+        pb_k[(2 * kOctetFloats) * q] = pk;
+        pb_m[-(2 * kOctetFloats) * q] = pm;
+      }
+      if (j == 0) {
+        const float a = re[8], b = im[8];
+        const float s = 4.0f * fmaf(b, b, a * a);
+        s_pb[pb_pos(128)] = USE_POWER ? s : sqrtf(s);
+      } else if (j < 8) {
+        s_pb[pb_pos(256) + j] = 0.0f;
+      }
       wave_lds_fence();
-#pragma unroll
-      for (int i = 0; i < 16; ++i) {
-        const int jj = kReadsInDftOrder ? (i >> 2) + 4 * (i & 3) : i;
-        typedef const volatile __attribute__((address_space(3))) unsigned long long *LdsU64;
-        const unsigned long long v = ((LdsU64)tbr)[jj];
-        re[jj] = __int_as_float((int)(uint32_t)v); im[jj] = __int_as_float((int)(uint32_t)(v >> 32));
-      }
-      wave_lds_fence();
-    }
-    PHASE(4);
-#ifndef SMILEHIP_DEBUG_SKIP_DFT2
-    dft16(re, im, dk);
-#endif
-    PHASE(5);
-
-    float zr[8], zi[8];
-#ifdef SMILEHIP_MFCC512_BPERMUTE_PARTNER
-    {
-      const int paddr = 4 * ((lane & 48) | ((16 - j) & 15));
-#pragma unroll
-      for (int q = 0; q < 8; ++q) {
-        float c = __int_as_float(__builtin_amdgcn_ds_bpermute(paddr, __float_as_int(re[15 - q])));
-        float d = __int_as_float(__builtin_amdgcn_ds_bpermute(paddr, __float_as_int(im[15 - q])));
-        if (q > 0) { c = (j == 0) ? re[16 - q] : c; d = (j == 0) ? im[16 - q] : d; }
-        zr[q] = c; zi[q] = d;
-      }
-    }
-#else
-#pragma unroll
-    for (int q = 0; q < 8; ++q) {
-      const float pr = q > 0 ? dpp_f<0x12f>(re[(16 - q) & 15]) : re[15];
-      const float pi = q > 0 ? dpp_f<0x12f>(im[(16 - q) & 15]) : im[15];
-      const float tr = __int_as_float(__builtin_amdgcn_update_dpp(__float_as_int(pr), __float_as_int(re[15 - q]), 0x101, 0xf, 0xf, false));
-      const float ti = __int_as_float(__builtin_amdgcn_update_dpp(__float_as_int(pi), __float_as_int(im[15 - q]), 0x101, 0xf, 0xf, false));
-      zr[q] = kMirrorOperand ? tr : dpp_f<0x140>(tr);
-      zi[q] = kMirrorOperand ? ti : dpp_f<0x140>(ti);
-    }
-#endif
-    float2 tw5[8];
-#pragma unroll
-    for (int q = 0; q < 8; ++q) tw5[q] = s_tw512[j + 16 * q];
-#pragma unroll
-    for (int q = 0; q < 8; ++q) {
-      const float2 w = tw5[q];
-      const float a = re[q], b = im[q];
-      const float c = kMirrorAtUse ? dpp_f<0x140>(zr[q]) : zr[q], d = kMirrorAtUse ? dpp_f<0x140>(zi[q]) : zi[q];
-      const float sr = a + c, si = b - d, dr = a - c, di = b + d;
-      const float ur = fmaf(w.x, dr, -w.y * di);
-      const float ui = fmaf(w.x, di, w.y * dr);
-      const float xr = sr + ui, xi = si - ur;
-      const float yr = sr - ui, yi = si + ur;
-      float pk = fmaf(xi, xi, xr * xr);
-      float pm = fmaf(yi, yi, yr * yr);
-      if (q == 0 && j == 0) {
-        const float v0 = 2.0f * (a + b), v1 = 2.0f * (a - b);
-        pk = v0 * v0; pm = v1 * v1;
-      }
-      if (!USE_POWER) { pk = sqrtf(pk); pm = sqrtf(pm); }
-      pb_k[(2 * kOctetFloats) * q] = pk;
-      pb_m[-(2 * kOctetFloats) * q] = pm;
-    }
-    if (j == 0) {
-      const float a = re[8], b = im[8];
-      const float s = 4.0f * fmaf(b, b, a * a);
-      s_pb[pb_pos(128)] = USE_POWER ? s : sqrtf(s);
-    } else if (j < 8) {
-      s_pb[pb_pos(256) + j] = 0.0f;
-    }
-    wave_lds_fence();
-
-    PHASE(6);
+
+      PHASE(6);
+    }
     int ntp = tp + 4;
     const bool advance = ntp >= cur_n;
     const bool more = !advance || has_next;
     if (advance) ntp = 0;
+    float4 mw0 = make_float4(0.f, 0.f, 0.f, 0.f), mw1 = mw0;
+    if constexpr (kMelwEarly) { mw0 = s_melw0[j]; mw1 = s_melw1[j]; }
     if (more)
       pcm_prefetch<MP, ALIGNED, PREEMPH>(P.pcm, P.pcm_total, (advance ? nxt_samp0 : cur_samp0) + (int64_t)ntp * P.H - P.pad_left, P.H, lane, R);
 
     PHASE(7);
-    {
-      float a0 = 0.0f, a1 = 0.0f;
-#pragma unroll
-      for (int i = 0; i < UC; ++i) {
-        const float4 *pp = reinterpret_cast<const float4 *>(reinterpret_cast<const unsigned char *>(s_pb) + mo[i]);
-        const float4 p0 = pp[0], p1 = pp[1];
-        const float4 w0 = s_melw0[i * 16 + j], w1 = s_melw1[i * 16 + j];
-        float acc = p0.x * w0.x;
-        acc = fmaf(p0.y, w0.y, acc); acc = fmaf(p0.z, w0.z, acc); acc = fmaf(p0.w, w0.w, acc);
-        acc = fmaf(p1.x, w1.x, acc); acc = fmaf(p1.y, w1.y, acc); acc = fmaf(p1.z, w1.z, acc); acc = fmaf(p1.w, w1.w, acc);
-        a0 = fmaf(acc, uf0[i], a0);
-        a1 = fmaf(acc, uf1[i], a1);
-      }
-      PHASE(8);
-#pragma unroll
-      for (int h = 0; h < 2; ++h) {
-        const int b = h ? band1 : band0;
-        const float acc = h ? a1 : a0;
-        if (b != 0xff) {
-          if (PLP) {
-            float v = acc * F.mel_scale;
-            v = v < P.melfloor ? P.melfloor : v;
-            s_lmel[b] = __expf(P.plp_compression * __logf(v * s_plp[b]));
-          } else {
-            s_lmel[b] = log_mel_fast(acc * F.mel_scale, P.melfloor, P.log_floor);
+    if (!dead) {
+      {
+        float a0 = 0.0f, a1 = 0.0f;
+#pragma unroll
+        for (int i = 0; i < UC; ++i) {
+          const float4 *pp = reinterpret_cast<const float4 *>(reinterpret_cast<const unsigned char *>(s_pb) + mo[i]);
+          const float4 p0 = pp[0], p1 = pp[1];
+          const float4 w0 = (kMelwEarly && i == 0) ? mw0 : s_melw0[i * 16 + j], w1 = (kMelwEarly && i == 0) ? mw1 : s_melw1[i * 16 + j];
+          float acc = p0.x * w0.x;
+          acc = fmaf(p0.y, w0.y, acc); acc = fmaf(p0.z, w0.z, acc); acc = fmaf(p0.w, w0.w, acc);
+          acc = fmaf(p1.x, w1.x, acc); acc = fmaf(p1.y, w1.y, acc); acc = fmaf(p1.z, w1.z, acc); acc = fmaf(p1.w, w1.w, acc);
+          a0 = fmaf(acc, uf0[i], a0);
+          a1 = fmaf(acc, uf1[i], a1);
+        }
+        PHASE(8);
+#pragma unroll
+        for (int h = 0; h < 2; ++h) {
+          const int b = h ? band1 : band0;
+          const float acc = h ? a1 : a0;
+          if (b != 0xff) {
+            if (PLP) {
+              float v = acc * F.mel_scale;
+              v = v < P.melfloor ? P.melfloor : v;
+              s_lmel[b] = __expf(P.plp_compression * __logf(v * s_plp[b]));
+            } else {
+              s_lmel[b] = log_mel_fast(acc * F.mel_scale, P.melfloor, P.log_floor);
+            }
           }
         }
-      }
-      if (j + 16 >= P.n_bands) s_lmel[j + 16] = 0.0f;
-      if (j >= P.n_bands) s_lmel[j] = 0.0f;
-    }
-    wave_lds_fence();
-
-    PHASE(9);
-    if (PLP) {
-      float *s_acf = s_lmel + 32;
-      if (j <= P.plp_order) s_acf[j] = plp_acf_lag(s_lmel, s_dct + j * 28, P.n_bands);
+        if (j + 16 >= P.n_bands) s_lmel[j + 16] = 0.0f;
+        if (j >= P.n_bands) s_lmel[j] = 0.0f;
+      }
       wave_lds_fence();
-      if (j == 0) plp_cc_serial(s_acf, P.plp_order, s_plp + 32, s_cep);
-      wave_lds_fence();
-      if (j < P.n_mfcc) pend_val = s_cep[j];
-    } else
-    if (j < P.n_mfcc) {
-      const float4 *row_c = reinterpret_cast<const float4 *>(s_dct + j * 28);
-      const float4 *lm = reinterpret_cast<const float4 *>(s_lmel);
-      float acc = 0.0f, dgain = 0.0f;
-#pragma unroll
-      for (int q = 0; q < 7; ++q) {
-        const float4 l = lm[q], c = row_c[q];
-        acc = fmaf(l.x, c.x, acc); acc = fmaf(l.y, c.y, acc); acc = fmaf(l.z, c.z, acc);
-        if (q < 6) acc = fmaf(l.w, c.w, acc); else dgain = c.w;
-      }
-      pend_val = acc * dgain;
+
+      PHASE(9);
+      if (PLP) {
+        float *s_acf = s_lmel + 32;
+        if (j <= P.plp_order) s_acf[j] = plp_acf_lag(s_lmel, s_dct + j * 28, P.n_bands);
+        wave_lds_fence();
+        if (j == 0) plp_cc_serial(s_acf, P.plp_order, s_plp + 32, s_cep);
+        wave_lds_fence();
+        if (j < P.n_mfcc) pend_val = s_cep[j];
+      } else
+      if (j < P.n_mfcc) {
+        const float4 *row_c = reinterpret_cast<const float4 *>(s_dct + j * 28);
+        const float4 *lm = reinterpret_cast<const float4 *>(s_lmel);
+        float acc = 0.0f, dgain = 0.0f;
+#pragma unroll
+        for (int q = 0; q < 7; ++q) {
+          const float4 l = lm[q], c = row_c[q];
+          acc = fmaf(l.x, c.x, acc); acc = fmaf(l.y, c.y, acc); acc = fmaf(l.z, c.z, acc);
+          if (q < 6) acc = fmaf(l.w, c.w, acc); else dgain = c.w;
+        }
+        pend_val = acc * dgain;
+      }
     }
     pend_live = live && j < P.n_mfcc;
     pend_row = reinterpret_cast<unsigned char *>(P.out + (cur_row0 + tp - (DELTA ? 4 : 0)) * P.ld_out);
diff --git a/opensmile_amd/csrc/smilehip_batch.cpp b/opensmile_amd/csrc/smilehip_batch.cpp
--- a/opensmile_amd/csrc/smilehip_batch.cpp
+++ b/opensmile_amd/csrc/smilehip_batch.cpp
@@ -113,7 +113,14 @@
 }
 
 extern "C" int smilehip_batch_create(smilehip_plan *plan, const int64_t *h_off, int32_t n_utt, smilehip_batch **out) {
+  return smilehip_batch_create_tiled(plan, h_off, n_utt, 0, out);
+}
+
+extern "C" int smilehip_batch_create_tiled(smilehip_plan *plan, const int64_t *h_off, int32_t n_utt, int32_t fused_tile_frames,
+                                           smilehip_batch **out) {
   if (!plan || !out || n_utt < 0 || (n_utt > 0 && !h_off)) return fail(SMILEHIP_ERR_INVALID, "smilehip_batch_create: bad argument");
+  if (fused_tile_frames != 0 && (fused_tile_frames < 4 || fused_tile_frames > 2048 || (fused_tile_frames & 3)))
+    return fail(SMILEHIP_ERR_INVALID, "smilehip_batch_create_tiled: the tile length is 0 or a multiple of 4 in 4 .. 2048, not %d", fused_tile_frames);
   *out = nullptr;
   if (!plan->ctx) return fail(SMILEHIP_ERR_NO_DEVICE, "host-only plan: no device attached (tables only)");
   if (plan->stage_mask != SMILEHIP_STAGE_ALL) return fail(SMILEHIP_ERR_INVALID, "single-component plan cannot run the fused chain");
@@ -122,7 +129,9 @@
   std::unique_ptr<smilehip_batch> b(new (std::nothrow) smilehip_batch());
   if (!b) return fail(SMILEHIP_ERR_NOMEM, "out of host memory");
   BatchLayout L;
-  if (const int bad = batch_layout(layout_spec(plan), h_off, n_utt, L))
+  BatchLayoutSpec spec = layout_spec(plan);
+  spec.fused_tile_frames = fused_tile_frames;
+  if (const int bad = batch_layout(spec, h_off, n_utt, L))
     return fail(SMILEHIP_ERR_INVALID, "sample offsets must be non-decreasing (utterance %d)", bad - 1);
   b->plan = plan;
   b->n_utt = n_utt;
```

Result: no change. 2.880 billion (median of 6 runs) (+0.6%).
